# pgvector/pgvector

Measured on AMD Instinct MI355X. Metric: QPS @ recall@10 (IVFFlat, 1M x 1536d), higher is better.
Workload: dtype f32

## Files before the change

pgvector_amd/csrc/kernels_query.hip:

```cpp
#include "pgv_device.h"
#include "pgv_select.h"

#include <type_traits>

namespace pgv {

namespace {

constexpr int kQThreads = kSelThreads;
constexpr int kQWaves = kQThreads / kWave;
constexpr int kMaxBatchLists = 256;
constexpr int kHeadCap = 1024;

template <typename T, int METRIC, int NCH> struct WholeRows {
    Raw16 q[NCH];
    __device__ __forceinline__ void load_query(const char *qp, int lane) {
#pragma unroll
        for (int c = 0; c < NCH; c++) q[c] = load16(qp + ((size_t)c * kWave + lane) * sizeof(Raw16));
    }
    __device__ __forceinline__ float pair(const char *a, const char *b, int lane) const {
        Raw16 ra[NCH], rb[NCH];
#pragma unroll
        for (int c = 0; c < NCH; c++) ra[c] = load16(a + ((size_t)c * kWave + lane) * sizeof(Raw16));
#pragma unroll
        for (int c = 0; c < NCH; c++) rb[c] = load16(b + ((size_t)c * kWave + lane) * sizeof(Raw16));
        float sa = 0.f, sb = 0.f;
#pragma unroll
        for (int c = 0; c < NCH; c++) sa = accum_slice<T, METRIC>(sa, ra[c], q[c]);
#pragma unroll
        for (int c = 0; c < NCH; c++) sb = accum_slice<T, METRIC>(sb, rb[c], q[c]);
        return finish<METRIC>(wave_sum2(sa, sb));
    }
};

template <typename T, int METRIC>
__device__ __forceinline__ float group_distance(const char *row, const char *qp, int nvec, int lane_in, int lg) {
    const int lpr = 1 << lg;
    float acc0 = 0.f, acc1 = 0.f;
    int v = lane_in;
    for (; v + lpr < nvec; v += 2 * lpr) {
        const Raw16 a0 = load16(row + (size_t)v * sizeof(Raw16));
        const Raw16 a1 = load16(row + (size_t)(v + lpr) * sizeof(Raw16));
        acc0 = accum_slice<T, METRIC>(acc0, a0, load16(qp + (size_t)v * sizeof(Raw16)));
        acc1 = accum_slice<T, METRIC>(acc1, a1, load16(qp + (size_t)(v + lpr) * sizeof(Raw16)));
    }
    if (v < nvec) acc0 = accum_slice<T, METRIC>(acc0, load16(row + (size_t)v * sizeof(Raw16)), load16(qp + (size_t)v * sizeof(Raw16)));
    return finish<METRIC>(group_sum_to_last(acc0 + acc1, lg));
}

__device__ __forceinline__ float group_distance_dot(const char *row, const char *qp, int nvec, int lane_in, int lg, float *dot) {
    const int lpr = 1 << lg;
    float acc0 = 0.f, acc1 = 0.f, dot0 = 0.f, dot1 = 0.f;
    int v = lane_in;
    for (; v + lpr < nvec; v += 2 * lpr) {
        const Raw16 a0 = load16(row + (size_t)v * sizeof(Raw16));
        const Raw16 a1 = load16(row + (size_t)(v + lpr) * sizeof(Raw16));
        const Raw16 q0 = load16(qp + (size_t)v * sizeof(Raw16));
        const Raw16 q1 = load16(qp + (size_t)(v + lpr) * sizeof(Raw16));
        acc0 = accum_slice<float, 0>(acc0, a0, q0);
        acc1 = accum_slice<float, 0>(acc1, a1, q1);
        dot0 = accum_slice<float, 1>(dot0, a0, q0);
        dot1 = accum_slice<float, 1>(dot1, a1, q1);
    }
    if (v < nvec) {
        const Raw16 a0 = load16(row + (size_t)v * sizeof(Raw16)), q0 = load16(qp + (size_t)v * sizeof(Raw16));
        acc0 = accum_slice<float, 0>(acc0, a0, q0);
        dot0 = accum_slice<float, 1>(dot0, a0, q0);
    }
    *dot = group_sum_to_last(dot0 + dot1, lg);
    return finish<0>(group_sum_to_last(acc0 + acc1, lg));
}

template <typename RowPtr>
__device__ __forceinline__ void score_rows_dot(RowPtr row_ptr, int64_t first, int64_t end, const char *qp, int nvec, int lg,
                                               float *out, float *out_dot) {
    const int lane = threadIdx.x & (kWave - 1);
    const int wave = threadIdx.x >> 6;
    const int rpw = kWave >> lg;
    const int g = lane >> lg, lane_in = lane & ((1 << lg) - 1);
    for (int64_t j0 = first + (int64_t)wave * rpw; j0 < end; j0 += (int64_t)kQWaves * rpw) {
        const int64_t j = j0 + g;
        const bool valid = j < end;
        float dot;
        const float d = group_distance_dot(row_ptr(valid ? j : end - 1), qp, nvec, lane_in, lg, &dot);
        if (valid && lane_in == (1 << lg) - 1) {
            out[j] = d;
            out_dot[j] = dot;
        }
    }
}

__device__ __forceinline__ void fill_pair_terms(const char *vectors, size_t row_bytes, const char *qrow, int ld,
                                                const int32_t *slots_i32, const int64_t *slots_i64, int k,
                                                float *__restrict__ pair_t) {
    const int lane = threadIdx.x & (kWave - 1);
    for (int i = threadIdx.x >> 6; i < k; i += kQWaves) {
        const int64_t slot = slots_i32 ? (int64_t)__hip_atomic_load(slots_i32 + i, __ATOMIC_RELAXED, __HIP_MEMORY_SCOPE_AGENT)
                                       : __hip_atomic_load(slots_i64 + i, __ATOMIC_RELAXED, __HIP_MEMORY_SCOPE_AGENT);
        float a = 0.f;
        if (slot >= 0) {
            const float *x = reinterpret_cast<const float *>(qrow);
            const float *c = reinterpret_cast<const float *>(vectors + (size_t)slot * row_bytes);
            for (int e = lane; e < ld; e += kWave) a = fmaf(x[e], c[e], a);
            for (int o = 32; o > 0; o >>= 1) a += __shfl_xor(a, o);
        }
        if (lane == 0) pair_t[i] = -2.f * a;
    }
}

template <typename T, int METRIC, int NCH, typename RowPtr>
__device__ __forceinline__ void score_rows(RowPtr row_ptr, int64_t first, int64_t end, const char *qp, int nvec, int lg,
                                           float *out) {
    const int lane = threadIdx.x & (kWave - 1);
    const int wave = threadIdx.x >> 6;
    if constexpr (NCH > 0) {
        WholeRows<T, METRIC, NCH> w;
        w.load_query(qp, lane);
        for (int64_t j = first + 2 * wave; j < end; j += 2 * kQWaves) {
            const bool two = j + 1 < end;
            const float d = w.pair(row_ptr(j), row_ptr(two ? j + 1 : j), lane);
            if (lane == 0 || (lane == 1 && two)) out[j + lane] = d;
        }
    } else {
        const int rpw = kWave >> lg;
        const int g = lane >> lg, lane_in = lane & ((1 << lg) - 1);
        for (int64_t j0 = first + (int64_t)wave * rpw; j0 < end; j0 += (int64_t)kQWaves * rpw) {
            const int64_t j = j0 + g;
            const bool valid = j < end;
            const float d = group_distance<T, METRIC>(row_ptr(valid ? j : end - 1), qp, nvec, lane_in, lg);
            if (valid && lane_in == (1 << lg) - 1) out[j] = d;
        }
    }
}

template <typename T, int METRIC, int NCH>
__global__ __launch_bounds__(kQThreads) void query_rank_kernel(const char *__restrict__ centers, int nlists, int nvec,
                                                               int lg, const char *__restrict__ qp,
                                                               float *__restrict__ cdist, int per) {
    const size_t row_bytes = (size_t)nvec * sizeof(Raw16);
    for (int64_t first = (int64_t)blockIdx.x * per; first < nlists; first += (int64_t)gridDim.x * per) {
        const int64_t end = first + per < nlists ? first + per : nlists;
        score_rows<T, METRIC, NCH>([&](int64_t j) { return centers + (size_t)j * row_bytes; }, first, end, qp, nvec, lg,
                                   cdist);
    }
}

__global__ __launch_bounds__(kQThreads) void query_lists_kernel(const float *__restrict__ cdist, int nlists,
                                                                int max_probes, int kp, int32_t *__restrict__ out_lists) {
    extern __shared__ __attribute__((aligned(16))) char smem[];
    unsigned long long *ent = reinterpret_cast<unsigned long long *>(smem);
    SelShared *s = reinterpret_cast<SelShared *>(smem + (size_t)kHeadCap * 8);
    block_topk_auto(cdist, nlists, max_probes, kp, kHeadCap, ent, s);
    for (int i = threadIdx.x; i < max_probes; i += kQThreads) out_lists[i] = (int32_t)(unsigned)(ent[i] & 0xffffffffu);
}

struct QueryHead {
    long long total;
    int count;
    unsigned seq;
};

struct BatchMap {
    int64_t offs[kMaxBatchLists + 1];
    int64_t lbeg[kMaxBatchLists];
    __device__ void build(const int32_t *probe_lists, int nprobes, const int64_t *list_off) {
        if ((int)threadIdx.x < nprobes) {
            const int l = probe_lists[threadIdx.x];
            lbeg[threadIdx.x] = list_off[l];
            offs[threadIdx.x + 1] = list_off[l + 1] - list_off[l];
        }
        __syncthreads();
        if (threadIdx.x == 0) {
            offs[0] = 0;
            for (int p = 0; p < nprobes; p++) offs[p + 1] += offs[p];
        }
        __syncthreads();
    }
    __device__ __forceinline__ int64_t slot_of(int64_t j, int nprobes) const {
        int lo = 0, hi = nprobes - 1;
        while (lo < hi) {
            const int mid = (lo + hi + 1) >> 1;
            if (offs[mid] <= j)
                lo = mid;
            else
                hi = mid - 1;
        }
        return lbeg[lo] + (j - offs[lo]);
    }
};

template <typename T, int METRIC, int NCH>
__global__ __launch_bounds__(kQThreads) void query_scan_kernel(
    const char *__restrict__ vectors, const int64_t *__restrict__ list_off, const int32_t *__restrict__ probe_lists,
    int nprobes, int nvec, int lg, const char *__restrict__ qp, float *__restrict__ seg, int per) {
    __shared__ BatchMap map;
    const size_t row_bytes = (size_t)nvec * sizeof(Raw16);
    map.build(probe_lists, nprobes, list_off);
    const int64_t m = map.offs[nprobes];
    for (int64_t first = (int64_t)blockIdx.x * per; first < m; first += (int64_t)gridDim.x * per) {
        const int64_t end = first + per < m ? first + per : m;
        if (qp) {
            score_rows<T, METRIC, NCH>([&](int64_t j) { return vectors + (size_t)map.slot_of(j, nprobes) * row_bytes; },
                                       first, end, qp, nvec, lg, seg);
        } else {
            for (int64_t j = first + threadIdx.x; j < end; j += kQThreads) seg[j] = 0.f;
        }
    }
}

__global__ __launch_bounds__(kQThreads) void query_head_kernel(
    const float *__restrict__ seg, const int64_t *__restrict__ list_off, const uint64_t *__restrict__ tids,
    const int32_t *__restrict__ probe_lists, int nprobes, int skip, int count, int kp, QueryHead *__restrict__ hdr,
    float *__restrict__ head_dist, int64_t *__restrict__ head_slot, uint64_t *__restrict__ head_tid, unsigned seq) {
    extern __shared__ __attribute__((aligned(16))) char smem[];
    __shared__ BatchMap map;
    map.build(probe_lists, nprobes, list_off);
    const int64_t m = map.offs[nprobes];
    unsigned long long *ent = reinterpret_cast<unsigned long long *>(smem);
    SelShared *s = reinterpret_cast<SelShared *>(smem + (size_t)kHeadCap * 8);
    const int k = skip + count;
    block_topk_auto(seg, m, k, kp, kHeadCap, ent, s);
    const int have = (int)(m < k ? m : k) - skip;
    for (int i = threadIdx.x; i < have; i += kQThreads) {
        const unsigned long long e = ent[skip + i];
        const int64_t slot = map.slot_of((int64_t)(unsigned)(e & 0xffffffffu), nprobes);
        head_dist[i] = key_to_float((unsigned)(e >> 32));
        head_slot[i] = slot;
        head_tid[i] = tids ? tids[slot] : ~0ull;
    }
    asm volatile("s_waitcnt vmcnt(0)" ::: "memory");
    __syncthreads();
    if (threadIdx.x == 0) {
        hdr->total = m;
        hdr->count = have > 0 ? have : 0;
        __hip_atomic_store(&hdr->seq, seq, __ATOMIC_RELEASE, __HIP_MEMORY_SCOPE_SYSTEM);
    }
}

__global__ __launch_bounds__(1024) void query_stage_kernel(const Raw16 *__restrict__ src, Raw16 *__restrict__ dst, int nvec) {
    for (int i = threadIdx.x; i < nvec; i += 1024) dst[i] = src[i];
}

__global__ void query_iota_kernel(int32_t *__restrict__ out, int n) {
    const int i = blockIdx.x * blockDim.x + threadIdx.x;
    if (i < n) out[i] = i;
}

template <typename T, int METRIC, int NCH>
__global__ __launch_bounds__(kQThreads) void mq_rank_kernel(const char *__restrict__ centers, int nlists, int nvec, int lg,
                                                            const char *__restrict__ queries, float *__restrict__ cdist,
                                                            int64_t cd_stride, int per) {
    const size_t row_bytes = (size_t)nvec * sizeof(Raw16);
    const char *qp = queries + (size_t)blockIdx.y * row_bytes;
    float *cd = cdist + (size_t)blockIdx.y * cd_stride;
    for (int64_t first = (int64_t)blockIdx.x * per; first < nlists; first += (int64_t)gridDim.x * per) {
        const int64_t end = first + per < nlists ? first + per : nlists;
        score_rows<T, METRIC, NCH>([&](int64_t j) { return centers + (size_t)j * row_bytes; }, first, end, qp, nvec, lg, cd);
    }
}

__global__ __launch_bounds__(kQThreads) void mq_lists_kernel(const float *__restrict__ cdist, int64_t cd_stride, int nlists,
                                                             int max_probes, int kp, int32_t *__restrict__ out_lists,
                                                             float *__restrict__ out_dist) {
    extern __shared__ __attribute__((aligned(16))) char smem[];
    unsigned long long *ent = reinterpret_cast<unsigned long long *>(smem);
    SelShared *s = reinterpret_cast<SelShared *>(smem + (size_t)kHeadCap * 8);
    const int q = blockIdx.x;
    block_topk_auto(cdist + (size_t)q * cd_stride, nlists, max_probes, kp, kHeadCap, ent, s);
    for (int i = threadIdx.x; i < max_probes; i += kQThreads) {
        out_lists[(size_t)q * max_probes + i] = (int32_t)(unsigned)(ent[i] & 0xffffffffu);
        if (out_dist) out_dist[(size_t)q * max_probes + i] = key_to_float((unsigned)(ent[i] >> 32));
    }
}

template <typename T, int METRIC, int NCH>
__global__ __launch_bounds__(kQThreads) void mq_scan_kernel(
    const char *__restrict__ vectors, const int64_t *__restrict__ list_off, const int32_t *__restrict__ probe_lists,
    int nprobes, int nvec, int lg, const char *__restrict__ queries, float *__restrict__ seg, int64_t seg_stride, int per) {
    __shared__ BatchMap map;
    const size_t row_bytes = (size_t)nvec * sizeof(Raw16);
    const int q = blockIdx.y;
    map.build(probe_lists + (size_t)q * nprobes, nprobes, list_off);
    const int64_t m = map.offs[nprobes];
    const char *qp = queries + (size_t)q * row_bytes;
    float *sg = seg + (size_t)q * seg_stride;
    for (int64_t first = (int64_t)blockIdx.x * per; first < m; first += (int64_t)gridDim.x * per) {
        const int64_t end = first + per < m ? first + per : m;
        score_rows<T, METRIC, NCH>([&](int64_t j) { return vectors + (size_t)map.slot_of(j, nprobes) * row_bytes; },
                                   first, end, qp, nvec, lg, sg);
    }
}

__global__ __launch_bounds__(kQThreads) void mq_head_kernel(
    const float *__restrict__ seg, int64_t seg_stride, const int64_t *__restrict__ list_off,
    const uint64_t *__restrict__ tids, const int32_t *__restrict__ probe_lists, int nprobes, int k, int kp,
    float *__restrict__ out_dist, int64_t *__restrict__ out_slot, uint64_t *__restrict__ out_tid,
    double *__restrict__ stats) {
    extern __shared__ __attribute__((aligned(16))) char smem[];
    __shared__ BatchMap map;
    const int q = blockIdx.x;
    map.build(probe_lists + (size_t)q * nprobes, nprobes, list_off);
    const int64_t m = map.offs[nprobes];
    unsigned long long *ent = reinterpret_cast<unsigned long long *>(smem);
    SelShared *s = reinterpret_cast<SelShared *>(smem + (size_t)kHeadCap * 8);
    block_topk_auto(seg + (size_t)q * seg_stride, m, k, kp, kHeadCap, ent, s);
    const int have = (int)(m < k ? m : k);
    for (int i = threadIdx.x; i < k; i += kQThreads) {
        const size_t o = (size_t)q * k + i;
        if (i < have) {
            const unsigned long long e = ent[i];
            const int64_t slot = map.slot_of((int64_t)(unsigned)(e & 0xffffffffu), nprobes);
            out_dist[o] = key_to_float((unsigned)(e >> 32));
            if (out_slot) out_slot[o] = slot;
            if (out_tid) out_tid[o] = tids ? tids[slot] : ~0ull;
        } else {
            out_dist[o] = INFINITY;
            if (out_slot) out_slot[o] = -1;
            if (out_tid) out_tid[o] = ~0ull;
        }
    }
    if (stats && threadIdx.x == 0) {
        atomicAdd(&stats[0], (double)m);
        atomicAdd(&stats[1], (double)m);
        atomicAdd(&stats[5], (double)m);
    }
}

constexpr int kRecheckCap = 256;

template <typename T, bool DOT = false>
__global__ __launch_bounds__(kQThreads) void batch_recheck_kernel(
    const char *__restrict__ vectors, const uint64_t *__restrict__ tids, int nvec, int lg,
    const char *__restrict__ queries, int kprime, int k, const float *__restrict__ approx_val,
    const int64_t *__restrict__ cand_pos, const int64_t *__restrict__ cand_slot,
    const int64_t *__restrict__ list_off, const int32_t *__restrict__ probe_lists,
    const int64_t *__restrict__ probe_off, int probes,
    const int64_t *__restrict__ seg_start, int64_t fixed_len,
    const unsigned *__restrict__ row_norm_max, ScanBound bound, const float *__restrict__ eps_add, int nq,
    float *__restrict__ out_dist, int64_t *__restrict__ out_slot, uint64_t *__restrict__ out_tid,
    int32_t *__restrict__ out_i32, int32_t *__restrict__ flags, float *__restrict__ pair_t, PlanEmit emit) {
    static_assert(!DOT || std::is_same<T, float>::value, "pair terms: fp32 rows");
    __shared__ float exact[kRecheckCap];
    __shared__ float dots[DOT ? kRecheckCap : 1];
    __shared__ __attribute__((aligned(16))) unsigned long long ent[kRecheckCap];
    const int q = blockIdx.x;
    const size_t row_bytes = (size_t)nvec * sizeof(Raw16);
    const int64_t m = seg_start ? seg_start[q + 1] - seg_start[q] : fixed_len;
    const int ncand = (int)(m < kprime ? m : (int64_t)kprime);
    const int kk = ncand < k ? ncand : k;
    const float *av = approx_val + (size_t)q * kprime;
    __shared__ float qn_part[kQWaves];
    {
        const char *qrow = queries + (size_t)q * row_bytes;
        float a = 0.f;
        for (int v = threadIdx.x; v < nvec; v += kQThreads) {
            const Raw16 x = load16(qrow + (size_t)v * sizeof(Raw16));
            a = accum_slice<T, 1>(a, x, x);
        }
        for (int m2 = 32; m2 > 0; m2 >>= 1) a += __shfl_xor(a, m2);
        if ((threadIdx.x & (kWave - 1)) == 0) qn_part[threadIdx.x >> 6] = a;
    }
    __syncthreads();
    float qn = 0.f;
    for (int w = 0; w < kQWaves; w++) qn += qn_part[w];
    const float rn = __uint_as_float(*row_norm_max);
    const float cross = 2.f * sqrtf(qn * rn);
    const float eps = 1.001f * (bound.g_sq * (qn + rn + cross) + bound.g_dot * cross + bound.g_norm * rn +
                                (eps_add ? eps_add[q] : 0.f));
    unsigned band = 0u;
    if (kk > 0) {
        const float edge = av[kk - 1] + 2.f * eps;
        band = float_to_key(edge + bound.g_ref * fabsf(edge + qn));
    }
    const int cnt = __syncthreads_count((int)threadIdx.x < ncand && float_to_key(av[threadIdx.x]) <= band);
    __shared__ int64_t slots[kRecheckCap];
    if ((int)threadIdx.x < cnt) {
        const int64_t p = cand_pos[(size_t)q * kprime + threadIdx.x];
        int64_t slot = p;
        if (cand_slot) {
            slot = cand_slot[(size_t)q * kprime + threadIdx.x];
        } else {
            const int64_t *off = probe_off + (size_t)q * probes;
            int lo = 0, hi = probes - 1;
            while (lo < hi) {
                const int mid = (lo + hi + 1) >> 1;
                if (off[mid] <= p)
                    lo = mid;
                else
                    hi = mid - 1;
            }
            slot = list_off[probe_lists[(size_t)q * probes + lo]] + (p - off[lo]);
        }
        slots[threadIdx.x] = slot;
    }
    __syncthreads();
    if constexpr (DOT)
        score_rows_dot([&](int64_t j) { return vectors + (size_t)slots[j] * row_bytes; }, 0, cnt,
                       queries + (size_t)q * row_bytes, nvec, lg, exact, dots);
    else
        score_rows<T, 0, 0>([&](int64_t j) { return vectors + (size_t)slots[j] * row_bytes; }, 0, cnt,
                            queries + (size_t)q * row_bytes, nvec, lg, exact);
    __syncthreads();
    if ((int)threadIdx.x < kRecheckCap)
        ent[threadIdx.x] = (int)threadIdx.x < cnt
                               ? ((unsigned long long)float_to_key(exact[threadIdx.x]) << 32) |
                                     (unsigned)cand_pos[(size_t)q * kprime + threadIdx.x]
                               : ~0ull;
    __syncthreads();
    const unsigned long long mine = ent[threadIdx.x];
    const int64_t my_slot = (int)threadIdx.x < cnt ? slots[threadIdx.x] : -1;
    int rank = 0;
    {
        const ulonglong2 *e2 = reinterpret_cast<const ulonglong2 *>(ent);
        const int n2 = (cnt + 1) / 2;
#pragma unroll 8
        for (int j = 0; j < n2; j++) {
            const ulonglong2 o = e2[j];
            rank += o.x < mine ? 1 : 0;
            rank += o.y < mine ? 1 : 0;
        }
    }
    if ((int)threadIdx.x < cnt && rank < k) {
        const size_t o = (size_t)q * k + rank;
        out_dist[o] = key_to_float((unsigned)(mine >> 32));
        if (out_slot) out_slot[o] = my_slot;
        if (out_i32) out_i32[o] = (int32_t)my_slot;
        if (out_tid) out_tid[o] = tids ? tids[my_slot] : ~0ull;
        if constexpr (DOT) pair_t[o] = -2.f * dots[threadIdx.x];
    }
    if ((int)threadIdx.x >= kk && (int)threadIdx.x < k) {
        const size_t o = (size_t)q * k + threadIdx.x;
        out_dist[o] = INFINITY;
        if (out_slot) out_slot[o] = -1;
        if (out_i32) out_i32[o] = -1;
        if (out_tid) out_tid[o] = ~0ull;
        if constexpr (DOT) pair_t[o] = 0.f;
    }
    if constexpr (DOT) {
        if (emit.cnt) {
            __syncthreads();
            if ((int)threadIdx.x < cnt && rank < k) {
                atomicAdd(&emit.cnt[my_slot], 1);
                slots[rank] = emit.list_off[my_slot + 1] - emit.list_off[my_slot];
            }
            if ((int)threadIdx.x >= kk && (int)threadIdx.x < k) slots[threadIdx.x] = 0;
            __syncthreads();
            if ((int)threadIdx.x < k) {
                int64_t run = 0;
                for (int i = 0; i < (int)threadIdx.x; i++) run += slots[i];
                emit.probe_off[(size_t)q * k + threadIdx.x] = run;
                if ((int)threadIdx.x == k - 1) emit.seg_len[q] = run + slots[threadIdx.x];
            }
        }
    }
    if (threadIdx.x == 0) {
        const int32_t flag = (m > ncand && cnt == ncand) ? 1 : 0;
        flags[q] = flag;
        if (flag) flags[nq + 1 + atomicAdd(&flags[nq], 1)] = q;
    }
}

constexpr int kWide = kRecheckCap;

template <typename T>
__global__ __launch_bounds__(kQThreads) void batch_fix_kernel(
    const char *__restrict__ vectors, const int64_t *__restrict__ list_off, const uint64_t *__restrict__ tids, int nvec,
    int lg, const char *__restrict__ queries, const int32_t *__restrict__ probe_lists,
    const int64_t *__restrict__ probe_off, int probes, const int64_t *__restrict__ seg_start, int64_t fixed_len,
    const int32_t *__restrict__ flags, int nq, float *__restrict__ seg_vals, int k, int kp, int cap,
    const unsigned *__restrict__ row_norm_max, ScanBound bound, const float *__restrict__ eps_add, int widen,
    float *__restrict__ out_dist, int64_t *__restrict__ out_slot, uint64_t *__restrict__ out_tid,
    int32_t *__restrict__ out_i32, double *__restrict__ stats, float *__restrict__ pair_t, PlanEmit emit) {
    extern __shared__ __attribute__((aligned(16))) char smem[];
    unsigned long long *ent = reinterpret_cast<unsigned long long *>(smem);
    SelShared *sel = reinterpret_cast<SelShared *>(smem + (size_t)cap * 8);
    __shared__ float exact[kWide];
    __shared__ int64_t slots[kWide];
    __shared__ float qn_part[kQWaves];
    const int nflag = flags[nq];
    const size_t row_bytes = (size_t)nvec * sizeof(Raw16);
    for (int f = blockIdx.x; f < nflag; f += gridDim.x) {
        const int q = flags[nq + 1 + f];
        const int64_t base = probe_lists ? seg_start[q] : (int64_t)q * fixed_len;
        const int64_t m = probe_lists ? seg_start[q + 1] - base : fixed_len;
        const int64_t *off = probe_off + (size_t)q * probes;
        const int32_t *pl = probe_lists + (size_t)q * probes;
        auto slot_of = [&](int64_t j) -> int64_t {
            if (!probe_lists) return j;
            int lo = 0, hi = probes - 1;
            while (lo < hi) {
                const int mid = (lo + hi + 1) >> 1;
                if (off[mid] <= j)
                    lo = mid;
                else
                    hi = mid - 1;
            }
            return list_off[pl[lo]] + (j - off[lo]);
        };
        float *v = seg_vals + base;
        const char *qrow = queries + (size_t)q * row_bytes;
        auto pair_terms = [&]() {
            if constexpr (std::is_same<T, float>::value) {
                if (pair_t) {
                    __threadfence();
                    __syncthreads();
                    fill_pair_terms(vectors, row_bytes, qrow, nvec * 4, out_i32 ? out_i32 + (size_t)q * k : nullptr,
                                    out_slot ? out_slot + (size_t)q * k : nullptr, k, pair_t + (size_t)q * k);
                    if (emit.cnt) {
                        if ((int)threadIdx.x < k) {
                            const int l = __hip_atomic_load(out_i32 + (size_t)q * k + threadIdx.x, __ATOMIC_RELAXED,
                                                            __HIP_MEMORY_SCOPE_AGENT);
                            if (l >= 0) atomicAdd(&emit.cnt[l], 1);
                            slots[threadIdx.x] = l >= 0 ? emit.list_off[l + 1] - emit.list_off[l] : 0;
                        }
                        __syncthreads();
                        if ((int)threadIdx.x < k) {
                            int64_t run = 0;
                            for (int i = 0; i < (int)threadIdx.x; i++) run += slots[i];
                            emit.probe_off[(size_t)q * k + threadIdx.x] = run;
                            if ((int)threadIdx.x == k - 1) emit.seg_len[q] = run + slots[threadIdx.x];
                        }
                    }
                }
            }
        };
        if constexpr (std::is_same<T, float>::value) {
            if (pair_t && emit.cnt) {
                if ((int)threadIdx.x < k) {
                    const int l = out_i32[(size_t)q * k + threadIdx.x];
                    if (l >= 0) atomicSub(&emit.cnt[l], 1);
                }
                __syncthreads();
            }
        }
        bool settled = false;
        if (widen && k <= kWide / 2) {
            const int nw = (int)(m < kWide ? m : (int64_t)kWide);
            block_topk([v](int64_t i) { return v[i]; }, m, nw, kWide, cap, ent, sel);
            {
                float a = 0.f;
                for (int x = threadIdx.x; x < nvec; x += kQThreads) {
                    const Raw16 e = load16(qrow + (size_t)x * sizeof(Raw16));
                    a = accum_slice<T, 1>(a, e, e);
                }
                for (int m2 = 32; m2 > 0; m2 >>= 1) a += __shfl_xor(a, m2);
                if ((threadIdx.x & (kWave - 1)) == 0) qn_part[threadIdx.x >> 6] = a;
            }
            __syncthreads();
            float qn = 0.f;
            for (int w = 0; w < kQWaves; w++) qn += qn_part[w];
            const float rn = __uint_as_float(*row_norm_max);
            const float cross = 2.f * sqrtf(qn * rn);
            const float eps = 1.001f * (bound.g_sq * (qn + rn + cross) + bound.g_dot * cross + bound.g_norm * rn +
                                        (eps_add ? eps_add[q] : 0.f));
            const int kk = nw < k ? nw : k;
            unsigned band = 0u;
            if (kk > 0) {
                const float edge = key_to_float((unsigned)(ent[kk - 1] >> 32)) + 2.f * eps;
                band = float_to_key(edge + bound.g_ref * fabsf(edge + qn));
            }
            const int cnt = __syncthreads_count((int)threadIdx.x < nw && (unsigned)(ent[threadIdx.x] >> 32) <= band);
            settled = !(m > nw && cnt == nw);
            if (settled) {
                const unsigned my_pos = (int)threadIdx.x < cnt ? (unsigned)(ent[threadIdx.x] & 0xffffffffu) : 0u;
                if ((int)threadIdx.x < cnt) slots[threadIdx.x] = slot_of((int64_t)my_pos);
                __syncthreads();
                score_rows<T, 0, 0>([&](int64_t j) { return vectors + (size_t)slots[j] * row_bytes; }, 0, cnt, qrow, nvec, lg,
                                    exact);
                __syncthreads();
                if ((int)threadIdx.x < kWide)
                    ent[threadIdx.x] = (int)threadIdx.x < cnt
                                           ? ((unsigned long long)float_to_key(exact[threadIdx.x]) << 32) | my_pos
                                           : ~0ull;
                __syncthreads();
                const unsigned long long mine = ent[threadIdx.x];
                int rank = 0;
                for (int j = 0; j < cnt; j++) rank += ent[j] < mine ? 1 : 0;
                const int have = (int)(m < k ? m : (int64_t)k);
                if ((int)threadIdx.x < cnt && rank < k) {
                    const size_t o = (size_t)q * k + rank;
                    const int64_t slot = slots[threadIdx.x];
                    out_dist[o] = key_to_float((unsigned)(mine >> 32));
                    if (out_slot) out_slot[o] = slot;
                    if (out_i32) out_i32[o] = (int32_t)slot;
                    if (out_tid) out_tid[o] = tids ? tids[slot] : ~0ull;
                }
                if ((int)threadIdx.x >= have && (int)threadIdx.x < k) {
                    const size_t o = (size_t)q * k + threadIdx.x;
                    out_dist[o] = INFINITY;
                    if (out_slot) out_slot[o] = -1;
                    if (out_i32) out_i32[o] = -1;
                    if (out_tid) out_tid[o] = ~0ull;
                }
                if (stats && threadIdx.x == 0) atomicAdd(&stats[7], 1.0);
                pair_terms();
            }
            __syncthreads();
        }
        if (settled) continue;
        if (stats && threadIdx.x == 0) atomicAdd(&stats[6], 1.0);
        score_rows<T, 0, 0>([&](int64_t j) { return vectors + (size_t)slot_of(j) * row_bytes; }, 0, m, qrow, nvec, lg, v);
        __threadfence();
        __syncthreads();
        block_topk([v](int64_t i) { return __hip_atomic_load(v + i, __ATOMIC_RELAXED, __HIP_MEMORY_SCOPE_AGENT); }, m, k, kp,
                   cap, ent, sel);
        for (int i = threadIdx.x; i < k; i += kQThreads) {
            const unsigned long long e = ent[i];
            const bool have = e != ~0ull && (int64_t)i < (m < k ? m : (int64_t)k);
            const int64_t slot = have ? slot_of((int64_t)(unsigned)(e & 0xffffffffu)) : -1;
            out_dist[(size_t)q * k + i] = have ? key_to_float((unsigned)(e >> 32)) : INFINITY;
            if (out_slot) out_slot[(size_t)q * k + i] = slot;
            if (out_i32) out_i32[(size_t)q * k + i] = (int32_t)slot;
            if (out_tid) out_tid[(size_t)q * k + i] = (have && tids) ? tids[slot] : ~0ull;
        }
        pair_terms();
        __syncthreads();
    }
}

constexpr size_t kQueryLds = (size_t)kHeadCap * 8 + sizeof(SelShared);

void run_geometry(pgv_ctx *ctx, const RowGeom &g, int64_t nrows, int *per, int *grid) {
    const bool whole = g.lpr_log2 == 6 && g.nvec % kWave == 0;
    const int step = kQWaves * (whole ? 2 : (kWave >> g.lpr_log2));
    int64_t runs = (nrows + step - 1) / step;
    const int64_t cap = (int64_t)ctx->num_cus * 8;
    *per = step;
    *grid = (int)(runs < 1 ? 1 : (runs > cap ? cap : runs));
}

int pow2_at_least(int k) {
    int kp = 2;
    while (kp < k) kp <<= 1;
    return kp;
}

template <typename T, int METRIC, typename F> int dispatch_nch(const RowGeom &g, F f) {
    if (g.lpr_log2 == 6 && g.nvec % kWave == 0) {
        switch (g.nvec / kWave) {
            case 1: return f(std::integral_constant<int, 1>());
            case 2: return f(std::integral_constant<int, 2>());
            case 3: return f(std::integral_constant<int, 3>());
            case 4: return f(std::integral_constant<int, 4>());
            case 6: return f(std::integral_constant<int, 6>());
        }
    }
    return f(std::integral_constant<int, 0>());
}

}

int query_max_batch_lists() { return kMaxBatchLists; }
int query_head_cap() { return kHeadCap; }
size_t query_head_bytes(int head) { return sizeof(QueryHead) + (size_t)head * (4 + 8 + 8) + 64; }

int launch_query_stage(pgv_ctx *ctx, const void *src_pinned, void *dst_dev, int nvec) {
    hipLaunchKernelGGL(query_stage_kernel, dim3(1), dim3(1024), 0, ctx->stream, static_cast<const Raw16 *>(src_pinned),
                       static_cast<Raw16 *>(dst_dev), nvec);
    PGV_HIP(hipGetLastError());
    return PGV_OK;
}

int launch_query_iota(pgv_ctx *ctx, int32_t *out, int n) {
    hipLaunchKernelGGL(query_iota_kernel, dim3((n + 255) / 256), dim3(256), 0, ctx->stream, out, n);
    PGV_HIP(hipGetLastError());
    return PGV_OK;
}

int launch_one_query_rows(pgv_ctx *ctx, const RowsView &v, const void *q_dev, float *out) {
    if (v.n <= 0) return PGV_OK;
    if (v.bits()) PGV_FAIL(PGV_ERR_ARG, "one query over rows: fp32 / fp16 rows only");
    const RowGeom &g = v.geom;
    const void *rows = v.rows;
    const int n = (int)v.n;
    int per, grid;
    run_geometry(ctx, g, n, &per, &grid);
    return dispatch_metric(v.metric, v.dtype(), [&](auto *tp, auto mc) {
        using T = std::remove_pointer_t<decltype(tp)>;
        constexpr int M = decltype(mc)::value;
        return dispatch_nch<T, M>(g, [&](auto nc) {
            constexpr int NCH = decltype(nc)::value;
            hipLaunchKernelGGL((query_rank_kernel<T, M, NCH>), dim3(grid), dim3(kQThreads), 0, ctx->stream,
                               static_cast<const char *>(rows), n, g.nvec, g.lpr_log2, static_cast<const char *>(q_dev),
                               out, per);
            PGV_HIP(hipGetLastError());
            return PGV_OK;
        });
    });
}

int launch_query_rank(pgv_ctx *ctx, const pgv_index *ix, const void *q_dev, float *cdist, int max_probes,
                      int32_t *out_lists) {
    const RowGeom &g = ix->geom;
    int per, grid;
    run_geometry(ctx, g, ix->nlists, &per, &grid);
    const int kp = pow2_at_least(max_probes);
    PGV_TRY(dispatch_metric(ix->metric, ix->dtype, [&](auto *tp, auto mc) {
        using T = std::remove_pointer_t<decltype(tp)>;
        constexpr int M = decltype(mc)::value;
        return dispatch_nch<T, M>(g, [&](auto nc) {
            constexpr int NCH = decltype(nc)::value;
            hipLaunchKernelGGL((query_rank_kernel<T, M, NCH>), dim3(grid), dim3(kQThreads), 0, ctx->stream,
                               static_cast<const char *>(ix->centers), ix->nlists, g.nvec, g.lpr_log2,
                               static_cast<const char *>(q_dev), cdist, per);
            PGV_HIP(hipGetLastError());
            return PGV_OK;
        });
    }));
    hipLaunchKernelGGL(query_lists_kernel, dim3(1), dim3(kQThreads), kQueryLds, ctx->stream, cdist, ix->nlists,
                       max_probes, kp, out_lists);
    PGV_HIP(hipGetLastError());
    return PGV_OK;
}

int launch_query_scan(pgv_ctx *ctx, const pgv_index *ix, const void *q_dev, const int32_t *probe_lists, int nprobes,
                      int64_t rows_bound, float *seg) {
    const RowGeom &g = ix->geom;
    int per, grid;
    run_geometry(ctx, g, rows_bound, &per, &grid);
    return dispatch_metric(ix->metric, ix->dtype, [&](auto *tp, auto mc) {
        using T = std::remove_pointer_t<decltype(tp)>;
        constexpr int M = decltype(mc)::value;
        return dispatch_nch<T, M>(g, [&](auto nc) {
            constexpr int NCH = decltype(nc)::value;
            hipLaunchKernelGGL((query_scan_kernel<T, M, NCH>), dim3(grid), dim3(kQThreads), 0, ctx->stream,
                               static_cast<const char *>(ix->vectors), ix->list_offsets, probe_lists, nprobes, g.nvec,
                               g.lpr_log2, static_cast<const char *>(q_dev), seg, per);
            PGV_HIP(hipGetLastError());
            return PGV_OK;
        });
    });
}

int launch_query_head(pgv_ctx *ctx, const pgv_index *ix, const float *seg, const int32_t *probe_lists, int nprobes,
                      int skip, int count, void *head_rec, unsigned seq) {
    const int kp = pow2_at_least(skip + count);
    QueryHead *hdr = static_cast<QueryHead *>(head_rec);
    char *base = static_cast<char *>(head_rec) + 64;
    int64_t *h_slot = reinterpret_cast<int64_t *>(base);
    uint64_t *h_tid = reinterpret_cast<uint64_t *>(base + (size_t)count * 8);
    float *h_dist = reinterpret_cast<float *>(base + (size_t)count * 16);
    hipLaunchKernelGGL(query_head_kernel, dim3(1), dim3(kQThreads), kQueryLds, ctx->stream, seg, ix->list_offsets,
                       ix->tids, probe_lists, nprobes, skip, count, kp, hdr, h_dist, h_slot, h_tid, seq);
    PGV_HIP(hipGetLastError());
    return PGV_OK;
}

int launch_multi_rank(pgv_ctx *ctx, const pgv_index *ix, const void *q_dev, int nq, float *cdist, int64_t cd_stride,
                      int max_probes, int32_t *out_lists, float *out_dist) {
    const RowGeom &g = ix->geom;
    int per, grid;
    run_geometry(ctx, g, ix->nlists, &per, &grid);
    const int kp = pow2_at_least(max_probes);
    PGV_TRY(dispatch_metric(ix->metric, ix->dtype, [&](auto *tp, auto mc) {
        using T = std::remove_pointer_t<decltype(tp)>;
        constexpr int M = decltype(mc)::value;
        return dispatch_nch<T, M>(g, [&](auto nc) {
            constexpr int NCH = decltype(nc)::value;
            hipLaunchKernelGGL((mq_rank_kernel<T, M, NCH>), dim3(grid, nq), dim3(kQThreads), 0, ctx->stream,
                               static_cast<const char *>(ix->centers), ix->nlists, g.nvec, g.lpr_log2,
                               static_cast<const char *>(q_dev), cdist, cd_stride, per);
            PGV_HIP(hipGetLastError());
            return PGV_OK;
        });
    }));
    hipLaunchKernelGGL(mq_lists_kernel, dim3(nq), dim3(kQThreads), kQueryLds, ctx->stream, cdist, cd_stride, ix->nlists,
                       max_probes, kp, out_lists, out_dist);
    PGV_HIP(hipGetLastError());
    return PGV_OK;
}

int launch_multi_scan(pgv_ctx *ctx, const pgv_index *ix, const void *q_dev, int nq, const int32_t *probe_lists, int nprobes,
                      int64_t rows_bound, float *seg, int64_t seg_stride, int k, float *out_dist, int64_t *out_slot,
                      uint64_t *out_tid) {
    const RowGeom &g = ix->geom;
    int per, grid;
    run_geometry(ctx, g, rows_bound, &per, &grid);
    const int cap = (ctx->num_cus * 8 + nq - 1) / nq;
    if (grid > cap) grid = cap < 1 ? 1 : cap;
    PGV_TRY(dispatch_metric(ix->metric, ix->dtype, [&](auto *tp, auto mc) {
        using T = std::remove_pointer_t<decltype(tp)>;
        constexpr int M = decltype(mc)::value;
        return dispatch_nch<T, M>(g, [&](auto nc) {
            constexpr int NCH = decltype(nc)::value;
            hipLaunchKernelGGL((mq_scan_kernel<T, M, NCH>), dim3(grid, nq), dim3(kQThreads), 0, ctx->stream,
                               static_cast<const char *>(ix->vectors), ix->list_offsets, probe_lists, nprobes, g.nvec,
                               g.lpr_log2, static_cast<const char *>(q_dev), seg, seg_stride, per);
            PGV_HIP(hipGetLastError());
            return PGV_OK;
        });
    }));
    double *stats = (ctx->profiling && ctx->stats_dev.p) ? ctx->stats_dev.as<double>() : nullptr;
    hipLaunchKernelGGL(mq_head_kernel, dim3(nq), dim3(kQThreads), kQueryLds, ctx->stream, seg, seg_stride, ix->list_offsets,
                       ix->tids, probe_lists, nprobes, k, pow2_at_least(k), out_dist, out_slot, out_tid, stats);
    PGV_HIP(hipGetLastError());
    return PGV_OK;
}

namespace {
struct ApproxScratch {
    float *cand_val = nullptr;
    int64_t *cand_pos = nullptr;
    int32_t *flags = nullptr;
    int carve(DBuf &buf, int nq, int kprime) {
        const size_t nk = (size_t)nq * kprime;
        const size_t a1 = (sizeof(float) * nk + 15) & ~(size_t)15, a2 = a1 + sizeof(int64_t) * nk;
        PGV_TRY(buf.ensure(a2 + sizeof(int32_t) * (2 * (size_t)nq + 1)));
        cand_val = buf.as<float>();
        cand_pos = reinterpret_cast<int64_t *>(buf.as<char>() + a1);
        flags = reinterpret_cast<int32_t *>(buf.as<char>() + a2);
        return PGV_OK;
    }
};
}

int launch_exact_tail(pgv_ctx *ctx, const ExactTail &t, DBuf &scratch) {
    if (t.nq <= 0) return PGV_OK;
    const ExactRows &xr = t.rows;
    const bool dense = t.dense();
    if (dense ? (t.fixed_len <= 0 || t.probe_off || t.seg_start || t.probes != 0)
              : (t.fixed_len != 0 || !t.probe_off || !t.seg_start || t.probes < 1))
        PGV_FAIL(PGV_ERR_ARG, "exact tail: a list plan or one dense run");
    if (t.kprime > kRecheckCap || t.k > t.kprime)
        PGV_FAIL(PGV_ERR_ARG, "exact tail: k' = %d outside k..%d", t.kprime, kRecheckCap);
    if (t.pair_t && xr.dtype != PGV_F32) PGV_FAIL(PGV_ERR_ARG, "exact tail: pair terms are for fp32 rows");
    static_assert(kWide >= kRecheckCap, "k <= k' <= kWide: batch_fix_kernel's emit");
    if (t.emit.cnt && !(dense && t.pair_t && t.out_i32 && t.emit.probe_off && t.emit.seg_len && t.emit.list_off))
        PGV_FAIL(PGV_ERR_ARG, "exact tail: the plan is counted where the pair terms are written");
    ApproxScratch sc;
    PGV_TRY(sc.carve(scratch, t.nq, t.kprime));
    const int64_t *cand_slot = dense ? sc.cand_pos : nullptr;
    const int64_t *seg_start = dense ? nullptr : t.seg_start;
    const int64_t fixed_len = dense ? t.fixed_len : 0;
    PGV_TRY(launch_topk_segments(ctx, t.approx, seg_start, t.nq, fixed_len, t.kprime, sc.cand_val, sc.cand_pos,
                                 sc.flags + t.nq, t.emit.cnt, t.emit.cnt ? 2 * (int)fixed_len : 0,
                                 dense ? 0 : t.seg_bound));
#define PGV_RECHECK(T, DOT)                                                                                          \
    hipLaunchKernelGGL((batch_recheck_kernel<T, DOT>), dim3(t.nq), dim3(kQThreads), 0, ctx->stream,                   \
                       static_cast<const char *>(xr.vectors), xr.tids, xr.geom.nvec, xr.geom.lpr_log2,                \
                       static_cast<const char *>(t.queries), t.kprime, t.k, sc.cand_val, sc.cand_pos, cand_slot,      \
                       xr.list_offsets, t.probe_lists, t.probe_off, t.probes, seg_start, fixed_len, xr.norm_max,      \
                       t.bound, t.eps_add, t.nq, t.out_dist, t.out_slot, t.out_tid, t.out_i32, sc.flags, t.pair_t,    \
                       t.emit)
    if (t.pair_t)
        PGV_RECHECK(float, true);
    else if (xr.dtype == PGV_F32)
        PGV_RECHECK(float, false);
    else
        PGV_RECHECK(__half, false);
#undef PGV_RECHECK
    PGV_HIP(hipGetLastError());
    double *stats = (ctx->profiling && ctx->stats_dev.p) ? ctx->stats_dev.as<double>() : nullptr;
    int kp = 2;
    while (kp < t.k) kp <<= 1;
    const int cap = kp > kFastCap ? kp : kFastCap;
    const size_t lds = (size_t)cap * 8 + sizeof(SelShared);
    const int grid = t.nq < ctx->num_cus ? t.nq : ctx->num_cus;
#define PGV_FIX(T)                                                                                                    \
    hipLaunchKernelGGL(batch_fix_kernel<T>, dim3(grid), dim3(kQThreads), lds, ctx->stream,                            \
                       static_cast<const char *>(xr.vectors), xr.list_offsets, xr.tids, xr.geom.nvec,                 \
                       xr.geom.lpr_log2, static_cast<const char *>(t.queries), t.probe_lists, t.probe_off, t.probes,  \
                       seg_start, fixed_len, sc.flags, t.nq, t.approx, t.k, kp, cap, xr.norm_max, t.bound, t.eps_add, \
                       ctx->no_widen ? 0 : 1, t.out_dist, t.out_slot, t.out_tid, t.out_i32, stats, t.pair_t, t.emit)
    if (xr.dtype == PGV_F32)
        PGV_FIX(float);
    else
        PGV_FIX(__half);
#undef PGV_FIX
    PGV_HIP(hipGetLastError());
    return PGV_OK;
}

}
```

pgvector_amd/csrc/kernels_shadow.hip:

```cpp
#include "pgv_device.h"

#include <cfloat>

namespace pgv {

namespace {

__device__ __forceinline__ int list_of_row(const int64_t *__restrict__ list_off, int nlists, int64_t r) {
    int lo = 0, hi = nlists - 1;
    while (lo < hi) {
        const int mid = (lo + hi + 1) >> 1;
        if (list_off[mid] <= r)
            lo = mid;
        else
            hi = mid - 1;
    }
    return lo;
}

__device__ __forceinline__ int scale_for(float m) {
    if (!(m > 0.f) || !isfinite(m)) return 0;
    int e;
    (void)frexpf(m, &e);
    return e - 14;
}

__global__ __launch_bounds__(256) void shadow_absmax_kernel(const float *__restrict__ rows, const float *__restrict__ centers,
                                                            const int64_t *__restrict__ list_off, int nlists, int64_t n,
                                                            int ld, unsigned *__restrict__ max_bits) {
    const int64_t r = (int64_t)blockIdx.x * 4 + (threadIdx.x >> 6);
    if (r >= n) return;
    const int lane = threadIdx.x & (kWave - 1);
    const float *x = rows + (size_t)r * ld;
    const float *c = centers ? centers + (size_t)list_of_row(list_off, nlists, r) * ld : nullptr;
    float m = 0.f;
    for (int i = lane; i < ld; i += kWave) {
        const float d = fabsf(c ? x[i] - c[i] : x[i]);
        m = (d > m || d != d) ? d : m;
    }
    for (int o = 32; o > 0; o >>= 1) {
        const float v = __shfl_xor(m, o);
        m = (v > m || v != v) ? v : m;
    }
    if (lane == 0 && __float_as_uint(m) > __hip_atomic_load(max_bits, __ATOMIC_RELAXED, __HIP_MEMORY_SCOPE_AGENT))
        atomicMax(max_bits, __float_as_uint(m));
}

__global__ __launch_bounds__(256) void shadow_build_kernel(const float *__restrict__ rows, const float *__restrict__ centers,
                                                           const int64_t *__restrict__ list_off, int nlists, int64_t n,
                                                           int ld, int ld16, const unsigned *__restrict__ max_bits,
                                                           __half *__restrict__ shadow,
                                                           unsigned long long *__restrict__ ep_bits) {
    const int64_t r = (int64_t)blockIdx.x * 4 + (threadIdx.x >> 6);
    if (r >= n) return;
    const int lane = threadIdx.x & (kWave - 1);
    const int s = scale_for(__uint_as_float(*max_bits));
    const float *x = rows + (size_t)r * ld;
    const float *c = centers ? centers + (size_t)list_of_row(list_off, nlists, r) * ld : nullptr;
    __half *h = shadow + (size_t)r * ld16;
    const double up = ldexp(1.0, s);
    double e2 = 0.0, p2 = 0.0;
    for (int i = lane; i < ld16; i += kWave) {
        __half v = __float2half(0.f);
        if (i < ld) {
            const float ci = c ? c[i] : 0.f;
            v = __float2half(ldexpf(x[i] - ci, -s));
            const double back = (double)__half2float(v) * up;
            const double d = ((double)x[i] - (double)ci) - back;
            e2 = fma(d, d, e2);
            p2 = fma(back, back, p2);
        }
        h[i] = v;
    }
    for (int o = 32; o > 0; o >>= 1) {
        e2 += __shfl_xor(e2, o);
        p2 += __shfl_xor(p2, o);
    }
    if (lane == 0) {
        const unsigned long long eb = (unsigned long long)__double_as_longlong(e2 != e2 ? INFINITY : e2),
                                 pb = (unsigned long long)__double_as_longlong(p2 != p2 ? INFINITY : p2);
        if (eb > __hip_atomic_load(&ep_bits[0], __ATOMIC_RELAXED, __HIP_MEMORY_SCOPE_AGENT)) atomicMax(&ep_bits[0], eb);
        if (pb > __hip_atomic_load(&ep_bits[1], __ATOMIC_RELAXED, __HIP_MEMORY_SCOPE_AGENT)) atomicMax(&ep_bits[1], pb);
    }
}

constexpr int kCastChunks = 4;

struct CastChunk {
    float4 a, b;
};

__device__ __forceinline__ float absmax_keep_nan(float m, float v) {
    const float a = fabsf(v);
    return (a > m || a != a) ? a : m;
}

__device__ __forceinline__ CastChunk cast_chunk_load(const float *__restrict__ x, int c, int ld) {
    CastChunk r;
    const float4 zero = make_float4(0.f, 0.f, 0.f, 0.f);
    r.a = 8 * c < ld ? *reinterpret_cast<const float4 *>(x + 8 * c) : zero;
    r.b = 8 * c + 4 < ld ? *reinterpret_cast<const float4 *>(x + 8 * c + 4) : zero;
    return r;
}

__device__ __forceinline__ float cast_chunk_max(const CastChunk &r, float m) {
    m = absmax_keep_nan(m, r.a.x);
    m = absmax_keep_nan(m, r.a.y);
    m = absmax_keep_nan(m, r.a.z);
    m = absmax_keep_nan(m, r.a.w);
    m = absmax_keep_nan(m, r.b.x);
    m = absmax_keep_nan(m, r.b.y);
    m = absmax_keep_nan(m, r.b.z);
    m = absmax_keep_nan(m, r.b.w);
    return m;
}

__device__ __forceinline__ void cast_chunk_store(const CastChunk &r, int c, int ld, int sq, double up, __half *__restrict__ h,
                                                 double (&qq)[4], double (&dd)[4], double (&hh)[4]) {
    const float xs[8] = {r.a.x, r.a.y, r.a.z, r.a.w, r.b.x, r.b.y, r.b.z, r.b.w};
    union {
        __half v[8];
        uint4 w;
    } out;
#pragma unroll
    for (int e = 0; e < 8; e++) {
        __half v = __float2half(0.f);
        if (8 * c + e < ld) {
            v = __float2half(ldexpf(xs[e], -sq));
            const double back = (double)__half2float(v) * up, xi = (double)xs[e];
            qq[e & 3] = fma(xi, xi, qq[e & 3]);
            dd[e & 3] = fma(xi - back, xi - back, dd[e & 3]);
            hh[e & 3] = fma(back, back, hh[e & 3]);
        }
        out.v[e] = v;
    }
    *reinterpret_cast<uint4 *>(h + 8 * c) = out.w;
}

__global__ __launch_bounds__(256) void shadow_query_kernel(const float *__restrict__ queries, int nq, int ld, int ld16,
                                                           ShadowTerms st, RankShadowTerms rt,
                                                           const float *__restrict__ center_norm_max,
                                                           const float *__restrict__ row_norm_max,
                                                           __half *__restrict__ qcast, float *__restrict__ qscale,
                                                           float *__restrict__ qeps, float *__restrict__ cscale,
                                                           float *__restrict__ ceps) {
    const int q = (int)(blockIdx.x * 4 + (threadIdx.x >> 6));
    if (q >= nq) return;
    const int lane = threadIdx.x & (kWave - 1);
    const float *x = queries + (size_t)q * ld;
    __half *h = qcast + (size_t)q * ld16;
    const int nchunks = ld16 / 8;
    const bool in_regs = nchunks <= kWave * kCastChunks;
    CastChunk reg[kCastChunks];
    float m = 0.f;
    if (in_regs) {
#pragma unroll
        for (int j = 0; j < kCastChunks; j++) {
            const int c = lane + j * kWave;
            reg[j] = cast_chunk_load(x, c < nchunks ? c : nchunks, ld);
        }
#pragma unroll
        for (int j = 0; j < kCastChunks; j++) m = cast_chunk_max(reg[j], m);
    } else {
        for (int c = lane; c < nchunks; c += kWave) m = cast_chunk_max(cast_chunk_load(x, c, ld), m);
    }
    for (int o = 32; o > 0; o >>= 1) {
        const float v = __shfl_xor(m, o);
        m = (v > m || v != v) ? v : m;
    }
    const int sq = scale_for(m);
    const double up = ldexp(1.0, sq);
    double qq4[4] = {0.0, 0.0, 0.0, 0.0}, dd4[4] = {0.0, 0.0, 0.0, 0.0}, hh4[4] = {0.0, 0.0, 0.0, 0.0};
    if (in_regs) {
#pragma unroll
        for (int j = 0; j < kCastChunks; j++) {
            const int c = lane + j * kWave;
            if (c < nchunks) cast_chunk_store(reg[j], c, ld, sq, up, h, qq4, dd4, hh4);
        }
    } else {
        for (int c = lane; c < nchunks; c += kWave) cast_chunk_store(cast_chunk_load(x, c, ld), c, ld, sq, up, h, qq4, dd4, hh4);
    }
    double qq = (qq4[0] + qq4[1]) + (qq4[2] + qq4[3]);
    double dd = (dd4[0] + dd4[1]) + (dd4[2] + dd4[3]);
    double hh = (hh4[0] + hh4[1]) + (hh4[2] + hh4[3]);
    for (int o = 32; o > 0; o >>= 1) {
        qq += __shfl_xor(qq, o);
        dd += __shfl_xor(dd, o);
        hh += __shfl_xor(hh, o);
    }
    const double u = 5.9604644775390625e-8;
    if (lane == 0 && ceps) {
        const int e = 1 + rt.s + sq;
        const double qn = sqrt(qq), dq = sqrt(dd), qh = sqrt(hh);
        const double cn = (double)*center_norm_max * (1.0 + rt.g_cn);
        double eps = 2.0 * (qn * rt.E + dq * rt.P)
                     + rt.g_dot * 2.0 * qh * rt.P
                     + 4.0 * u * (cn + 2.0 * qh * rt.P * (1.0 + rt.g_dot));
        eps = eps * (1.0 + 1.0 / 1048576.0) + 4.0 * (double)FLT_MIN;
        if (e < -125 || e > 125 || !(eps < 1e30)) eps = INFINITY;
        cscale[q] = ldexpf(1.f, e < -125 ? 0 : (e > 125 ? 0 : e));
        ceps[q] = (float)eps;
    }
    if (lane == 0 && qeps) {
        const int e = 1 + st.s + sq;
        const double qn = sqrt(qq), dq = sqrt(dd), qh = sqrt(hh);
        const double cmax = sqrt((double)*center_norm_max * (1.0 + st.g_cn)), rn = (double)*row_norm_max * (1.0 + st.g_cn);
        const double tmax = 2.0 * qn * cmax;
        double eps = 2.0 * (qn * st.E + dq * st.P)
                     + st.g_dot * 2.0 * qh * st.P
                     + st.g_pair * tmax
                     + 4.0 * u * (rn + tmax * (1.0 + st.g_pair) + 2.0 * qh * st.P * (1.0 + st.g_dot));
        eps = eps * (1.0 + 1.0 / 1048576.0) + 4.0 * (double)FLT_MIN;
        if (e < -125 || e > 125 || !(eps < 1e30)) eps = INFINITY;
        qscale[q] = ldexpf(1.f, e < -125 ? 0 : (e > 125 ? 0 : e));
        qeps[q] = (float)eps;
    }
}

__global__ __launch_bounds__(256) void shadow_pair_kernel(const float *__restrict__ queries, const float *__restrict__ centers,
                                                          const int64_t *__restrict__ pair_start, int nlists, int64_t npairs,
                                                          int ld, ScanPair *__restrict__ pairs) {
    const int64_t pos = (int64_t)blockIdx.x * 4 + (threadIdx.x >> 6);
    if (pos >= npairs) return;
    const int lane = threadIdx.x & (kWave - 1);
    int lo = 0, hi = nlists - 1;
    while (lo < hi) {
        const int mid = (lo + hi + 1) >> 1;
        if (pair_start[mid] <= pos)
            lo = mid;
        else
            hi = mid - 1;
    }
    const int q = pairs[pos].query;
    const float *x = queries + (size_t)q * ld;
    const float *c = centers + (size_t)lo * ld;
    float a = 0.f;
    for (int i = lane; i < ld; i += kWave) a = fmaf(x[i], c[i], a);
    for (int o = 32; o > 0; o >>= 1) a += __shfl_xor(a, o);
    if (lane == 0) pairs[pos].pad = (int32_t)__float_as_uint(-2.f * a);
}

}

int launch_shadow_build(pgv_ctx *ctx, const RowGeom &g32, const RowGeom &g16, const void *rows, const void *centers,
                        const int64_t *list_off, int nlists, int64_t n, void *shadow, void *words) {
    if (n <= 0) return PGV_OK;
    PGV_HIP(hipMemsetAsync(words, 0, 24, ctx->stream));
    unsigned *max_bits = static_cast<unsigned *>(words);
    unsigned long long *ep = reinterpret_cast<unsigned long long *>(static_cast<char *>(words) + 8);
    const dim3 grid((unsigned)((n + 3) / 4));
    hipLaunchKernelGGL(shadow_absmax_kernel, grid, dim3(256), 0, ctx->stream, static_cast<const float *>(rows),
                       static_cast<const float *>(centers), list_off, nlists, n, g32.ld, max_bits);
    hipLaunchKernelGGL(shadow_build_kernel, grid, dim3(256), 0, ctx->stream, static_cast<const float *>(rows),
                       static_cast<const float *>(centers), list_off, nlists, n, g32.ld, g16.ld, max_bits, static_cast<__half *>(shadow), ep);
    PGV_HIP(hipGetLastError());
    return PGV_OK;
}

int shadow_scale_of(float max_abs) {
    if (!(max_abs > 0.f) || !std::isfinite(max_abs)) return 0;
    int e;
    (void)std::frexp(max_abs, &e);
    return e - 14;
}

int launch_shadow_query(pgv_ctx *ctx, const RowGeom &g32, const RowGeom &g16, const void *queries, int nq,
                        const ShadowTerms &st, const RankShadowTerms &rt, const float *center_norm_max,
                        const float *row_norm_max, void *qcast, float *qscale, float *qeps, float *cscale, float *ceps) {
    if (nq <= 0) return PGV_OK;
    hipLaunchKernelGGL(shadow_query_kernel, dim3((unsigned)((nq + 3) / 4)), dim3(256), 0, ctx->stream,
                       static_cast<const float *>(queries), nq, g32.ld, g16.ld, st, rt, center_norm_max, row_norm_max,
                       static_cast<__half *>(qcast), qscale, qeps, cscale, ceps);
    PGV_HIP(hipGetLastError());
    return PGV_OK;
}

int launch_shadow_pairs(pgv_ctx *ctx, const RowGeom &g32, const void *queries, const void *centers,
                        const int64_t *pair_start, int nlists, int64_t npairs, ScanPair *pairs) {
    if (npairs <= 0) return PGV_OK;
    hipLaunchKernelGGL(shadow_pair_kernel, dim3((unsigned)((npairs + 3) / 4)), dim3(256), 0, ctx->stream,
                       static_cast<const float *>(queries), static_cast<const float *>(centers), pair_start, nlists, npairs,
                       g32.ld, pairs);
    PGV_HIP(hipGetLastError());
    return PGV_OK;
}

}
```

pgvector_amd/csrc/pgv_abi_ivf.hip:

```cpp
#include "pgv_abi_common.h"

extern "C" {


namespace {
struct IndexLayout {
    size_t centers, vectors, offsets, tids, row_norms, center_norms, bytes;
    bool has_tids, has_norms;
};
IndexLayout index_layout(int nlists, int64_t n, size_t row_bytes, bool has_tids, bool l2) {
    auto up = [](size_t v) { return (v + 255) & ~(size_t)255; };
    IndexLayout L{};
    size_t at = 0;
    L.centers = at; at = up(at + (size_t)nlists * row_bytes);
    L.vectors = at; at = up(at + (size_t)(n > 0 ? n : 1) * row_bytes);
    L.offsets = at; at = up(at + sizeof(int64_t) * ((size_t)nlists + 1));
    L.has_tids = has_tids;
    L.tids = at; if (has_tids) at = up(at + sizeof(uint64_t) * (size_t)n);
    L.has_norms = l2;
    L.row_norms = at; if (l2 && n > 0) at = up(at + sizeof(float) * ((size_t)n + 1));
    L.center_norms = at; if (l2) at = up(at + sizeof(float) * ((size_t)nlists + 1));
    L.bytes = at;
    return L;
}
void index_carve(pgv_index *ix, const IndexLayout &L) {
    char *b = static_cast<char *>(ix->arena);
    ix->centers = b + L.centers;
    ix->vectors = b + L.vectors;
    ix->list_offsets = reinterpret_cast<int64_t *>(b + L.offsets);
    ix->tids = L.has_tids ? reinterpret_cast<uint64_t *>(b + L.tids) : nullptr;
    ix->row_norms = L.has_norms && ix->nrows > 0 ? reinterpret_cast<float *>(b + L.row_norms) : nullptr;
    ix->center_norms = L.has_norms ? reinterpret_cast<float *>(b + L.center_norms) : nullptr;
}
void index_host_tables(pgv_index *ix) {
    const int nlists = ix->nlists;
    std::vector<int64_t> lens((size_t)nlists);
    int64_t maxlen = 0;
    for (int l = 0; l < nlists; l++) {
        lens[l] = ix->h_offsets[l + 1] - ix->h_offsets[l];
        if (lens[l] > maxlen) maxlen = lens[l];
    }
    ix->max_list_len = maxlen;
    std::sort(lens.begin(), lens.end(), [](int64_t a, int64_t b) { return a > b; });
    ix->len_prefix.assign((size_t)nlists + 1, 0);
    for (int l = 0; l < nlists; l++) ix->len_prefix[l + 1] = ix->len_prefix[l] + lens[l];
}
}

extern "C++" {
namespace {

int shadow_env() {
    const char *e = getenv("PGV_SCAN_SHADOW");
    return e ? atoi(e) : -1;
}

int rank_shadow_env() {
    const char *e = getenv("PGV_RANK_SHADOW");
    return e ? atoi(e) : 1;
}

int shadow_create(pgv_ctx *ctx, pgv_index *ix) {
    const int env = shadow_env();
    if (env == 0 || ix->metric != PGV_L2SQ || ix->dtype != PGV_F32 || ix->nrows <= 0 || !ix->row_norms || !ix->center_norms)
        return PGV_OK;
    if (env < 0 && !rows_stream_past_caches(ivf_rows(ix))) return PGV_OK;
    const RowGeom g16 = row_geom(ix->dim, PGV_F16);
    const size_t bytes = ((size_t)ix->nrows * g16.ld * sizeof(uint16_t) + 255) & ~(size_t)255;
    const size_t cbytes = ((size_t)ix->nlists * g16.ld * sizeof(uint16_t) + 255) & ~(size_t)255;
    void *sh = nullptr;
    if (hipMalloc(&sh, bytes + 256 + cbytes) != hipSuccess) {
        (void)hipGetLastError();
        return PGV_OK;
    }
    void *words = static_cast<char *>(sh) + bytes;
    void *csh = static_cast<char *>(sh) + bytes + 256;
    int rc = launch_shadow_build(ctx, ix->geom, g16, ix->vectors, ix->centers, ix->list_offsets, ix->nlists, ix->nrows, sh,
                                 words);
    if (rc == PGV_OK)
        rc = launch_shadow_build(ctx, ix->geom, g16, ix->centers, nullptr, nullptr, 0, ix->nlists, csh,
                                 static_cast<char *>(words) + 32);
    unsigned char h[56];
    if (rc == PGV_OK && (hipStreamSynchronize(ctx->stream) != hipSuccess ||
                         hipMemcpy(h, words, sizeof(h), hipMemcpyDeviceToHost) != hipSuccess)) {
        set_error("shadow build failed: %s", hipGetErrorString(hipGetLastError()));
        rc = PGV_ERR_DEVICE;
    }
    if (rc != PGV_OK) {
        (void)hipFree(sh);
        return rc;
    }
    float max_abs;
    double e2, p2;
    memcpy(&max_abs, h, 4);
    memcpy(&e2, h + 8, 8);
    memcpy(&p2, h + 16, 8);
    const double P = std::sqrt(p2), E = std::sqrt(e2);
    if (!std::isfinite(E) || !std::isfinite(P) || !std::isfinite(max_abs)) {
        (void)hipFree(sh);
        return PGV_OK;
    }
    ix->shadow = sh;
    ix->shadow_geom = g16;
    ix->shadow_s = shadow_scale_of(max_abs);
    ix->shadow_E = (E + 1e-12 * (P + E)) * (1.0 + 1e-9);
    ix->shadow_P = P * (1.0 + 1e-9);
    float cmax_abs;
    double ce2, cp2;
    memcpy(&cmax_abs, h + 32, 4);
    memcpy(&ce2, h + 40, 8);
    memcpy(&cp2, h + 48, 8);
    const double Pc = std::sqrt(cp2), Ec = std::sqrt(ce2);
    if (std::isfinite(Ec) && std::isfinite(Pc) && std::isfinite(cmax_abs)) {
        ix->cshadow = csh;
        ix->cshadow_s = shadow_scale_of(cmax_abs);
        ix->cshadow_E = (Ec + 1e-12 * (Pc + Ec)) * (1.0 + 1e-9);
        ix->cshadow_P = Pc * (1.0 + 1e-9);
    }
    return PGV_OK;
}

struct ShadowBatch {
    void *qcast = nullptr;
    float *qscale = nullptr, *qeps = nullptr;
    float *cscale = nullptr, *ceps = nullptr;
    float *pair_t = nullptr;
    bool scan_follows = false;
    bool cast_for_scan = false;
    bool pairs_done = false;
};

int shadow_batch_cast(pgv_index *ix, const void *q_dev, int nq, int probes, bool for_rank, bool for_scan, ShadowBatch *sb) {
    pgv_ctx *ctx = ix->ctx;
    const RowGeom &g16 = ix->shadow_geom;
    const size_t qb = ((size_t)nq * g16.ld * sizeof(uint16_t) + 255) & ~(size_t)255;
    PGV_TRY(ctx->sh_q.ensure(qb + sizeof(float) * (size_t)nq * (4 + (size_t)probes)));
    sb->qcast = ctx->sh_q.p;
    sb->qscale = reinterpret_cast<float *>(ctx->sh_q.as<char>() + qb);
    sb->qeps = sb->qscale + nq;
    sb->cscale = sb->qeps + nq;
    sb->ceps = sb->cscale + nq;
    sb->pair_t = sb->ceps + nq;
    constexpr double u = 5.9604644775390625e-8;
    ShadowTerms st{};
    st.s = ix->shadow_s;
    st.E = ix->shadow_E;
    st.P = ix->shadow_P;
    st.g_dot = gamma_n(shadow_chain_length(g16) + 4.0, u);
    st.g_pair = gamma_n((double)pair_chain_length(ix->geom), u);
    st.g_cn = shadow_band(ix->geom.ld, 0.f, u).g_norm;
    RankShadowTerms rt{};
    rt.s = ix->cshadow_s;
    rt.E = ix->cshadow_E;
    rt.P = ix->cshadow_P;
    rt.g_dot = st.g_dot;
    rt.g_cn = st.g_cn;
    PGV_TRY(launch_shadow_query(ctx, ix->geom, g16, q_dev, nq, st, rt, ix->center_norms + ix->nlists,
                                ix->row_norms + ix->nrows, sb->qcast, for_scan ? sb->qscale : nullptr,
                                for_scan ? sb->qeps : nullptr, for_rank ? sb->cscale : nullptr,
                                for_rank ? sb->ceps : nullptr));
    sb->cast_for_scan = for_scan;
    return PGV_OK;
}

struct IndexElem {
    pgv_metric metric;
    pgv_dtype dtype;
    int dim, nbits;
    static IndexElem bits(int nbits) { return {PGV_L1, PGV_F32, nbits, nbits}; }
    size_t tight_bytes() const { return nbits > 0 ? (size_t)(nbits + 7) / 8 : (size_t)dim * elem_size(dtype); }
};

template <typename Fill>
int index_create(pgv_ctx *ctx, const IndexElem &el, int nlists, const std::vector<int64_t> &off, bool has_tids, Fill fill,
                 pgv_index **out) {
    const pgv_metric metric = el.metric;
    const int nbits = el.nbits;
    const int64_t n = off[nlists];
    pgv_index *ix = new (std::nothrow) pgv_index();
    if (!ix) PGV_FAIL(PGV_ERR_NOMEM, "out of host memory");
    ix->ctx = ctx;
    ix->refs = new (std::nothrow) int(1);
    if (!ix->refs) {
        delete ix;
        PGV_FAIL(PGV_ERR_NOMEM, "out of host memory");
    }
    ix->metric = metric;
    ix->dtype = el.dtype;
    ix->dim = el.dim;
    ix->nlists = nlists;
    ix->nrows = n;
    ix->nbits = nbits;
    ix->geom = nbits > 0 ? bit_row_geom(nbits) : row_geom(el.dim, el.dtype);
    ix->h_offsets = off;
    index_host_tables(ix);

    auto fail = [&](int rc) {
        pgv_index_free(ix);
        return rc;
    };
    IndexLayout lay = index_layout(nlists, n, ivf_rows(ix).row_bytes(), has_tids && n > 0, metric == PGV_L2SQ && nbits == 0);
    if (malloc_exportable(&ix->arena, lay.bytes) != hipSuccess) {
        (void)hipGetLastError();
        set_error("hipMalloc(%zu) for the index mirror failed", lay.bytes);
        return fail(PGV_ERR_NOMEM);
    }
    ix->arena_bytes = lay.bytes;
    index_carve(ix, lay);
    int rc;
    if ((rc = fill(ix)) != PGV_OK) return fail(rc);
    if (hipMemcpyAsync(ix->list_offsets, ix->h_offsets.data(), sizeof(int64_t) * off.size(),
                       hipMemcpyHostToDevice, ctx->stream) != hipSuccess)
        return fail((set_error("copy of list_offsets failed"), PGV_ERR_DEVICE));
    if (ix->row_norms) {
        if (hipMemsetAsync(ix->row_norms + n, 0, sizeof(float), ctx->stream) != hipSuccess)
            return fail((set_error("memset of row_norms failed"), PGV_ERR_DEVICE));
        if ((rc = launch_row_norms(ctx, ivf_rows(ix), ix->row_norms, reinterpret_cast<unsigned *>(ix->row_norms + n))) != PGV_OK)
            return fail(rc);
    }
    if (ix->center_norms) {
        if (hipMemsetAsync(ix->center_norms + nlists, 0, sizeof(float), ctx->stream) != hipSuccess)
            return fail((set_error("memset of center_norms failed"), PGV_ERR_DEVICE));
        if ((rc = launch_row_norms(ctx, ivf_centers(ix), ix->center_norms,
                                   reinterpret_cast<unsigned *>(ix->center_norms + nlists))) != PGV_OK)
            return fail(rc);
    }
    if (nbits == 0 && (rc = shadow_create(ctx, ix)) != PGV_OK) return fail(rc);
    if (hipStreamSynchronize(ctx->stream) != hipSuccess)
        return fail((set_error("index upload failed: %s", hipGetErrorString(hipGetLastError())), PGV_ERR_DEVICE));
    *out = ix;
    return PGV_OK;
}

int index_upload(pgv_ctx *ctx, const IndexElem &el, int nlists, const void *centers, const int64_t *list_offsets,
                 const void *rows, const char *rows_name, const uint64_t *tids, pgv_index **out) {
    if (nlists < 1 || nlists > 32768) PGV_FAIL(PGV_ERR_ARG, "lists %d outside 1..32768", nlists);
    if (!centers || !list_offsets) PGV_FAIL(PGV_ERR_ARG, "centers/list_offsets is NULL");
    PGV_HIP(hipSetDevice(ctx->device));
    std::vector<int64_t> off((size_t)nlists + 1);
    if (is_device_ptr(list_offsets)) {
        PGV_HIP(hipMemcpy(off.data(), list_offsets, sizeof(int64_t) * off.size(), hipMemcpyDeviceToHost));
    } else {
        memcpy(off.data(), list_offsets, sizeof(int64_t) * off.size());
    }
    if (off[0] != 0) PGV_FAIL(PGV_ERR_ARG, "list_offsets[0] must be 0");
    for (int l = 0; l < nlists; l++)
        if (off[l + 1] < off[l]) PGV_FAIL(PGV_ERR_ARG, "list_offsets not ascending at list %d", l);
    const int64_t n = off[nlists];
    if (n > 0 && !rows) PGV_FAIL(PGV_ERR_ARG, "%s is NULL", rows_name);
    return index_create(ctx, el, nlists, off, tids != nullptr, [&](pgv_index *ix) -> int {
        const size_t padded = ivf_rows(ix).row_bytes();
        PGV_TRY(put_padded_rows(ctx->stream, ix->centers, padded, centers, el.tight_bytes(), nlists));
        PGV_TRY(put_padded_rows(ctx->stream, ix->vectors, padded, rows, el.tight_bytes(), n));
        if (ix->tids)
            PGV_HIP(hipMemcpyAsync(ix->tids, tids, sizeof(uint64_t) * (size_t)n,
                                   is_device_ptr(tids) ? hipMemcpyDeviceToDevice : hipMemcpyHostToDevice, ctx->stream));
        return PGV_OK;
    }, out);
}

}
}

int pgv_index_upload(pgv_ctx *ctx, pgv_metric metric, pgv_dtype dtype, int dim, int nlists,
                     const void *centers, const int64_t *list_offsets, const void *vectors,
                     const uint64_t *tids, pgv_index **out) {
    if (!ctx || !out) PGV_FAIL(PGV_ERR_ARG, "pgv_index_upload: ctx/out is NULL");
    *out = nullptr;
    PGV_TRY(check_common(dtype, dim));
    PGV_TRY(check_metric(metric));
    return index_upload(ctx, IndexElem{metric, dtype, dim, 0}, nlists, centers, list_offsets, vectors, "vectors", tids, out);
}

int pgv_index_upload_bits(pgv_ctx *ctx, int nbits, int nlists, const void *centers, const int64_t *list_offsets,
                          const void *rows, const uint64_t *tids, pgv_index **out) {
    if (!ctx || !out) PGV_FAIL(PGV_ERR_ARG, "pgv_index_upload_bits: ctx/out is NULL");
    *out = nullptr;
    if (nbits < 1 || nbits > kIvfMaxBits) PGV_FAIL(PGV_ERR_DIMS, "bit length %d outside 1..%d", nbits, kIvfMaxBits);
    return index_upload(ctx, IndexElem::bits(nbits), nlists, centers, list_offsets, rows, "rows", tids, out);
}

int pgv_index_nbits(const pgv_index *ix) { return ix ? ix->nbits : -1; }

#define PGV_NO_BIT_INDEX(ix, who)                                                                                 \
    do {                                                                                                          \
        if ((ix)->nbits > 0) PGV_FAIL(PGV_ERR_ARG, "%s: not served on a bit index (pgv_index_upload_bits)", who); \
    } while (0)

static int stage_queries(pgv_index *ix, const void *queries, int nq, const void **q_dev) {
    if (ix->nbits > 0)
        return stage_rows(ix->ctx, queries, nq, (size_t)(ix->nbits + 7) / 8, (size_t)bit_query_bytes(ix->nbits), ix->ctx->q_stage,
                          q_dev);
    return stage_rows(ix->ctx, queries, nq, ix->dim, ix->dtype, ix->geom, ix->ctx->q_stage, q_dev);
}

struct pgv_builder {
    pgv_ctx *ctx = nullptr;
    pgv_metric metric = PGV_L2SQ;
    pgv_dtype dtype = PGV_F32;
    int dim = 0, nlists = 0;
    RowGeom geom{};
    DBuf centers;
    DBuf rows;
    DBuf tids;
    DBuf lists;
    int64_t n = 0, cap = 0;
    int64_t assigned = 0;
    bool has_tids = true;
    bool deferred = false;
    hipStream_t copy_stream = nullptr;
    hipStream_t stream() const { return deferred ? copy_stream : ctx->stream; }
    RowsView view() const { return {rows.p, n, geom, row_kind(dtype), metric}; }
    size_t row_bytes() const { return view().row_bytes(); }
    int put(hipStream_t to, void *dst, const void *src, int64_t cnt) const {
        return put_padded_rows(to, dst, row_bytes(), src, (size_t)dim * elem_size(dtype), cnt);
    }
};

static int builder_reserve(pgv_builder *b, int64_t want) {
    if (want <= b->cap) return PGV_OK;
    int64_t cap = b->cap ? b->cap + b->cap / 2 : want;
    if (cap < want) cap = want;
    const size_t row_bytes = b->row_bytes();
    DBuf rows, tids, lists;
    PGV_TRY(rows.ensure(row_bytes * (size_t)cap));
    int rc = tids.ensure(sizeof(uint64_t) * (size_t)cap);
    if (rc == PGV_OK) rc = lists.ensure(sizeof(int32_t) * (size_t)cap);
    if (rc == PGV_OK && b->n > 0) {
        hipError_t e = hipMemcpyAsync(rows.p, b->rows.p, row_bytes * (size_t)b->n, hipMemcpyDeviceToDevice, b->stream());
        if (e == hipSuccess) e = hipMemcpyAsync(tids.p, b->tids.p, sizeof(uint64_t) * (size_t)b->n, hipMemcpyDeviceToDevice, b->stream());
        if (e == hipSuccess) e = hipMemcpyAsync(lists.p, b->lists.p, sizeof(int32_t) * (size_t)b->n, hipMemcpyDeviceToDevice, b->stream());
        if (e == hipSuccess) e = hipStreamSynchronize(b->stream());
        if (e != hipSuccess) {
            set_error("growing the builder failed: %s", hipGetErrorString(e));
            rc = PGV_ERR_DEVICE;
        }
    }
    if (rc != PGV_OK) {
        rows.release();
        tids.release();
        lists.release();
        return rc;
    }
    b->rows.release();
    b->tids.release();
    b->lists.release();
    b->rows = rows;
    b->tids = tids;
    b->lists = lists;
    b->cap = cap;
    return PGV_OK;
}

static int builder_assign_pending(pgv_builder *b) {
    if (b->assigned >= b->n) return PGV_OK;
    PGV_TRY(launch_argmin(b->ctx, b->metric, b->dtype, b->geom, b->rows.as<char>() + (size_t)b->assigned * b->row_bytes(),
                          b->n - b->assigned, b->centers.p, b->nlists, b->lists.as<int32_t>() + b->assigned, nullptr));
    b->assigned = b->n;
    return PGV_OK;
}

int pgv_builder_begin(pgv_ctx *ctx, pgv_metric metric, pgv_dtype dtype, int dim, int nlists, const void *centers,
                      int64_t expected_rows, pgv_builder **out) {
    if (!ctx || !out) PGV_FAIL(PGV_ERR_ARG, "pgv_builder_begin: ctx/out is NULL");
    *out = nullptr;
    PGV_TRY(check_common(dtype, dim));
    PGV_TRY(check_metric(metric));
    if (nlists < 1 || nlists > 32768) PGV_FAIL(PGV_ERR_ARG, "lists %d outside 1..32768", nlists);
    if (expected_rows < 0) PGV_FAIL(PGV_ERR_ARG, "expected_rows < 0");
    PGV_HIP(hipSetDevice(ctx->device));
    pgv_builder *b = new (std::nothrow) pgv_builder();
    if (!b) PGV_FAIL(PGV_ERR_NOMEM, "out of host memory");
    b->ctx = ctx;
    b->metric = metric;
    b->dtype = dtype;
    b->dim = dim;
    b->nlists = nlists;
    b->geom = row_geom(dim, dtype);
    int rc = b->centers.ensure(b->row_bytes() * (size_t)nlists);
    if (rc == PGV_OK && centers) {
        rc = b->put(ctx->stream, b->centers.p, centers, nlists);
        if (rc == PGV_OK && hipStreamSynchronize(ctx->stream) != hipSuccess) rc = PGV_ERR_DEVICE;
    } else if (rc == PGV_OK) {
        b->deferred = true;
        if (hipStreamCreateWithFlags(&b->copy_stream, hipStreamNonBlocking) != hipSuccess) {
            set_error("pgv_builder_begin: no stream for the upload");
            rc = PGV_ERR_DEVICE;
        }
    }
    if (rc == PGV_OK && expected_rows > 0) rc = builder_reserve(b, expected_rows);
    if (rc != PGV_OK) {
        pgv_builder_free(b);
        return rc;
    }
    *out = b;
    return PGV_OK;
}

void pgv_builder_free(pgv_builder *b) {
    if (!b) return;
    if (b->copy_stream) {
        (void)hipStreamSynchronize(b->copy_stream);
        (void)hipStreamDestroy(b->copy_stream);
    }
    if (b->ctx) (void)hipStreamSynchronize(b->ctx->stream);
    b->centers.release();
    b->rows.release();
    b->tids.release();
    b->lists.release();
    delete b;
}

int64_t pgv_builder_rows(const pgv_builder *b) { return b ? b->n : -1; }

int pgv_builder_add(pgv_builder *b, const void *rows, const uint64_t *tids, int64_t n) {
    if (!b) PGV_FAIL(PGV_ERR_ARG, "pgv_builder_add: builder is NULL");
    if (n < 0) PGV_FAIL(PGV_ERR_ARG, "n < 0");
    if (n == 0) return PGV_OK;
    if (!rows) PGV_FAIL(PGV_ERR_ARG, "rows is NULL");
    if (b->n + n > 0xffffffffll) PGV_FAIL(PGV_ERR_ARG, "pgv_builder_add: more than 2^32 rows");
    if (b->n > 0 && (tids != nullptr) != b->has_tids) PGV_FAIL(PGV_ERR_ARG, "pgv_builder_add: tids given for some batches only");
    pgv_ctx *ctx = b->ctx;
    PGV_HIP(hipSetDevice(ctx->device));
    PGV_TRY(builder_reserve(b, b->n + n));
    b->has_tids = tids != nullptr;
    hipStream_t stream = b->stream();
    PGV_TRY(b->put(stream, b->rows.as<char>() + (size_t)b->n * b->row_bytes(), rows, n));
    if (tids)
        PGV_HIP(hipMemcpyAsync(b->tids.as<uint64_t>() + b->n, tids, sizeof(uint64_t) * (size_t)n,
                               is_device_ptr(tids) ? hipMemcpyDeviceToDevice : hipMemcpyHostToDevice, stream));
    b->n += n;
    if (!b->deferred) PGV_TRY(builder_assign_pending(b));
    if (b->deferred || !is_device_ptr(rows) || (tids && !is_device_ptr(tids))) PGV_HIP(hipStreamSynchronize(stream));
    return PGV_OK;
}

int pgv_builder_set_centers(pgv_builder *b, const void *centers) {
    if (!b || !centers) PGV_FAIL(PGV_ERR_ARG, "pgv_builder_set_centers: builder/centers is NULL");
    if (!b->deferred) PGV_FAIL(PGV_ERR_STATE, "pgv_builder_set_centers: the builder has its centers");
    pgv_ctx *ctx = b->ctx;
    PGV_HIP(hipSetDevice(ctx->device));
    PGV_HIP(hipStreamSynchronize(b->copy_stream));
    b->deferred = false;
    PGV_TRY(b->put(ctx->stream, b->centers.p, centers, b->nlists));
    PGV_HIP(hipStreamSynchronize(ctx->stream));
    return PGV_OK;
}

int pgv_builder_finish(pgv_builder *b, pgv_index **out_index, int64_t *out_offsets, int32_t *out_lists) {
    if (!b || !out_index) PGV_FAIL(PGV_ERR_ARG, "pgv_builder_finish: builder/out_index is NULL");
    *out_index = nullptr;
    pgv_ctx *ctx = b->ctx;
    PGV_HIP(hipSetDevice(ctx->device));
    if (b->deferred) PGV_FAIL(PGV_ERR_STATE, "pgv_builder_finish: no centers (pgv_builder_set_centers)");
    PGV_TRY(builder_assign_pending(b));
    const int64_t n = b->n;
    const int nlists = b->nlists;
    int list_bits = 1;
    while ((1 << list_bits) < nlists) list_bits++;
    const size_t sort_bytes = n > 0 ? build_sort_scratch_bytes(n, 32 + list_bits) : 0;
    const size_t kb = sizeof(unsigned long long) * (size_t)(n > 0 ? n : 1), cb = sizeof(unsigned long long) * (size_t)nlists,
                 ob = sizeof(int64_t) * ((size_t)nlists + 1);
    auto up = [](size_t x) { return (x + 255) & ~(size_t)255; };
    const size_t o_sorted = up(kb), o_counts = o_sorted + up(kb), o_off = o_counts + up(cb), o_bad = o_off + up(ob),
                 o_sort = o_bad + 256;
    DBuf scratch;
    PGV_TRY(scratch.ensure(o_sort + sort_bytes + 256));
    char *sp = scratch.as<char>();
    auto *keys_tmp = reinterpret_cast<unsigned long long *>(sp);
    auto *keys_sorted = reinterpret_cast<unsigned long long *>(sp + o_sorted);
    auto *counts = reinterpret_cast<unsigned long long *>(sp + o_counts);
    auto *offsets_dev = reinterpret_cast<int64_t *>(sp + o_off);
    int *bad = reinterpret_cast<int *>(sp + o_bad);
    int rc = launch_build_order(ctx, b->lists.as<int32_t>(), n, nlists, keys_tmp, keys_sorted, counts, offsets_dev, bad,
                                sp + o_sort, sort_bytes);
    std::vector<int64_t> off((size_t)nlists + 1);
    int bad_h = 0;
    if (rc == PGV_OK) {
        hipError_t e = hipMemcpyAsync(off.data(), offsets_dev, ob, hipMemcpyDeviceToHost, ctx->stream);
        if (e == hipSuccess) e = hipMemcpyAsync(&bad_h, bad, sizeof(int), hipMemcpyDeviceToHost, ctx->stream);
        if (e == hipSuccess && out_lists && n > 0)
            e = hipMemcpyAsync(out_lists, b->lists.p, sizeof(int32_t) * (size_t)n,
                               is_device_ptr(out_lists) ? hipMemcpyDeviceToDevice : hipMemcpyDeviceToHost, ctx->stream);
        if (e == hipSuccess) e = hipStreamSynchronize(ctx->stream);
        if (e != hipSuccess) {
            set_error("pgv_builder_finish: %s", hipGetErrorString(e));
            rc = PGV_ERR_DEVICE;
        }
    }
    if (rc == PGV_OK && (bad_h || off[nlists] != n)) {
        set_error("pgv_builder_finish: assignment produced a list id outside 0..%d", nlists - 1);
        rc = PGV_ERR_STATE;
    }
    if (rc == PGV_OK)
        rc = index_create(ctx, IndexElem{b->metric, b->dtype, b->dim, 0}, nlists, off, true, [&](pgv_index *ix) -> int {
            PGV_HIP(hipMemcpyAsync(ix->centers, b->centers.p, b->row_bytes() * (size_t)nlists, hipMemcpyDeviceToDevice,
                                   ctx->stream));
            return launch_build_gather(ctx, b->rows.p, keys_sorted, n, b->geom.nvec, ix->vectors,
                                       b->has_tids ? b->tids.as<uint64_t>() : nullptr, ix->tids);
        }, out_index);
    scratch.release();
    if (rc != PGV_OK) return rc;
    if (out_offsets) memcpy(out_offsets, off.data(), ob);
    b->rows.release();
    b->tids.release();
    b->lists.release();
    b->n = b->cap = b->assigned = 0;
    return PGV_OK;
}

int pgv_index_drain(pgv_index *ix, int64_t chunk_rows, pgv_rows_sink sink, void *arg) {
    if (!ix || !sink) PGV_FAIL(PGV_ERR_ARG, "pgv_index_drain: index/sink is NULL");
    PGV_NO_BIT_INDEX(ix, "pgv_index_drain");
    pgv_ctx *ctx = ix->ctx;
    PGV_HIP(hipSetDevice(ctx->device));
    const int64_t n = ix->nrows;
    if (n == 0) return PGV_OK;
    const size_t tight = (size_t)ix->dim * elem_size(ix->dtype), padded = ivf_rows(ix).row_bytes();
    if (chunk_rows <= 0) chunk_rows = (int64_t)std::max<size_t>(1, ((size_t)64 << 20) / tight);
    if (chunk_rows > n) chunk_rows = n;
    void *buf[2] = {nullptr, nullptr};
    hipEvent_t ev[2] = {nullptr, nullptr};
    const size_t piece = tight * (size_t)chunk_rows + sizeof(uint64_t) * (size_t)chunk_rows;
    int rc = PGV_OK;
    for (int i = 0; i < 2 && rc == PGV_OK; i++) {
        if (hipHostMalloc(&buf[i], piece, hipHostMallocDefault) != hipSuccess) rc = PGV_ERR_NOMEM;
        if (rc == PGV_OK && hipEventCreateWithFlags(&ev[i], hipEventDisableTiming) != hipSuccess) rc = PGV_ERR_DEVICE;
    }
    auto issue = [&](int64_t c, int slot) -> int {
        const int64_t r0 = c * chunk_rows, cnt = std::min(chunk_rows, n - r0);
        char *dst = static_cast<char *>(buf[slot]);
        const char *src = static_cast<const char *>(ix->vectors) + (size_t)r0 * padded;
        if (padded == tight)
            PGV_HIP(hipMemcpyAsync(dst, src, tight * (size_t)cnt, hipMemcpyDeviceToHost, ctx->stream));
        else
            PGV_HIP(hipMemcpy2DAsync(dst, tight, src, padded, tight, (size_t)cnt, hipMemcpyDeviceToHost, ctx->stream));
        if (ix->tids)
            PGV_HIP(hipMemcpyAsync(dst + tight * (size_t)chunk_rows, ix->tids + r0, sizeof(uint64_t) * (size_t)cnt,
                                   hipMemcpyDeviceToHost, ctx->stream));
        PGV_HIP(hipEventRecord(ev[slot], ctx->stream));
        return PGV_OK;
    };
    const int64_t nchunks = (n + chunk_rows - 1) / chunk_rows;
    if (rc == PGV_OK) rc = issue(0, 0);
    for (int64_t c = 0; c < nchunks && rc == PGV_OK; c++) {
        const int slot = (int)(c & 1);
        if (c + 1 < nchunks) rc = issue(c + 1, slot ^ 1);
        if (rc != PGV_OK) break;
        if (hipEventSynchronize(ev[slot]) != hipSuccess) {
            set_error("pgv_index_drain: copy failed");
            rc = PGV_ERR_DEVICE;
            break;
        }
        const int64_t r0 = c * chunk_rows, cnt = std::min(chunk_rows, n - r0);
        const char *p = static_cast<const char *>(buf[slot]);
        const int src = sink(arg, r0, cnt, p, ix->tids ? reinterpret_cast<const uint64_t *>(p + tight * (size_t)chunk_rows) : nullptr);
        if (src != 0) {
            set_error("pgv_index_drain: the sink returned %d", src);
            rc = PGV_ERR_STATE;
        }
    }
    (void)hipStreamSynchronize(ctx->stream);
    for (int i = 0; i < 2; i++) {
        if (ev[i]) (void)hipEventDestroy(ev[i]);
        if (buf[i]) (void)hipHostFree(buf[i]);
    }
    if (rc == PGV_ERR_NOMEM) set_error("pgv_index_drain: pinned buffers (2 x %zu bytes) could not be allocated", piece);
    return rc;
}

static void index_drop_lanes(pgv_index *ix);

int pgv_index_set_overlap(pgv_index *ix, int lanes) {
    if (!ix) PGV_FAIL(PGV_ERR_ARG, "pgv_index_set_overlap: index is NULL");
    PGV_NO_BIT_INDEX(ix, "pgv_index_set_overlap");
    if (lanes < 1 || lanes > 4) PGV_FAIL(PGV_ERR_ARG, "pgv_index_set_overlap: lanes %d outside 1..4", lanes);
    PGV_HIP(hipSetDevice(ix->ctx->device));
    PGV_TRY(pgv_ctx_sync(ix->ctx));
    index_drop_lanes(ix);
    if (lanes == 1) return PGV_OK;
    PGV_HIP(hipEventCreateWithFlags(&ix->lane_event, hipEventDisableTiming));
    PGV_HIP(hipEventCreateWithFlags(&ix->lane_scan_done, hipEventDisableTiming));
    for (int i = 0; i < lanes; i++) {
        pgv_ctx *lc = nullptr;
        pgv_index *v = nullptr;
        int rc = pgv_ctx_create(ix->ctx->device, nullptr, &lc);
        if (rc == PGV_OK) rc = pgv_index_share(ix, lc, &v);
        if (rc != PGV_OK) {
            if (lc) pgv_ctx_destroy(lc);
            index_drop_lanes(ix);
            return rc;
        }
        lc->no_mfma_scan = ix->ctx->no_mfma_scan;
        lc->bound_mode = ix->ctx->bound_mode;
        lc->assign_bound_mode = ix->ctx->assign_bound_mode;
        if (ix->ctx->profiling) (void)pgv_ctx_set_profiling(lc, 1);
        lc->scan_gate = ix->lane_scan_done;
        ix->lanes.push_back(v);
        ix->ctx->children.push_back(lc);
    }
    return PGV_OK;
}

int pgv_index_share(pgv_index *ix, pgv_ctx *ctx, pgv_index **out) {
    if (!ix || !ctx || !out) PGV_FAIL(PGV_ERR_ARG, "pgv_index_share: index/ctx/out is NULL");
    *out = nullptr;
    if (ctx->device != ix->ctx->device)
        PGV_FAIL(PGV_ERR_ARG, "pgv_index_share: the index lives on device %d, the context on %d", ix->ctx->device, ctx->device);
    pgv_index *v = new (std::nothrow) pgv_index(*ix);
    if (!v) PGV_FAIL(PGV_ERR_NOMEM, "out of host memory");
    v->ctx = ctx;
    v->lanes.clear();
    v->lane_next = 0;
    v->lane_event = nullptr;
    v->lane_scan_done = nullptr;
    __atomic_add_fetch(ix->refs, 1, __ATOMIC_RELAXED);
    *out = v;
    return PGV_OK;
}

struct IndexHandleWire {
    uint64_t magic;
    uint32_t abi, pid;
    int32_t device, metric, dtype, dim, nlists, has_tids;
    int64_t nrows;
    uint64_t arena_bytes;
    hipIpcMemHandle_t mem;
};
static_assert(sizeof(IndexHandleWire) <= PGV_INDEX_HANDLE_BYTES, "pgv_index_handle too small");
static constexpr uint64_t kIndexHandleMagic = 0x7067765f69786831ull;

int pgv_index_export(pgv_index *ix, pgv_index_handle *out) {
    if (!ix || !out) PGV_FAIL(PGV_ERR_ARG, "pgv_index_export: index/out is NULL");
    PGV_NO_BIT_INDEX(ix, "pgv_index_export");
    if (!ix->arena) PGV_FAIL(PGV_ERR_STATE, "pgv_index_export: the index has no device arrays");
    if (ix->imported) PGV_FAIL(PGV_ERR_STATE, "pgv_index_export: export from the process that uploaded the index");
    PGV_HIP(hipSetDevice(ix->ctx->device));
    IndexHandleWire w;
    memset(&w, 0, sizeof(w));
    w.magic = kIndexHandleMagic;
    w.abi = PGV_ABI_VERSION;
    w.pid = (uint32_t)getpid();
    w.device = ix->ctx->device;
    w.metric = ix->metric;
    w.dtype = ix->dtype;
    w.dim = ix->dim;
    w.nlists = ix->nlists;
    w.has_tids = ix->tids != nullptr;
    w.nrows = ix->nrows;
    w.arena_bytes = ix->arena_bytes;
    hipError_t e = hipIpcGetMemHandle(&w.mem, ix->arena);
    if (e != hipSuccess) {
        (void)hipGetLastError();
        PGV_FAIL(PGV_ERR_DEVICE,
                 "hipIpcGetMemHandle failed: %s (the driver here shares memory by dmabuf: HSA_ENABLE_IPC_MODE_LEGACY=0 "
                 "must be in the environment of every process)", hipGetErrorString(e));
    }
    memset(out, 0, sizeof(*out));
    memcpy(out->bytes, &w, sizeof(w));
    return PGV_OK;
}

int pgv_index_import(pgv_ctx *ctx, const pgv_index_handle *handle, pgv_index **out) {
    if (!ctx || !handle || !out) PGV_FAIL(PGV_ERR_ARG, "pgv_index_import: ctx/handle/out is NULL");
    *out = nullptr;
    IndexHandleWire w;
    memcpy(&w, handle->bytes, sizeof(w));
    if (w.magic != kIndexHandleMagic || w.abi != PGV_ABI_VERSION)
        PGV_FAIL(PGV_ERR_ARG, "pgv_index_import: not a handle of this library version");
    if (w.pid == (uint32_t)getpid())
        PGV_FAIL(PGV_ERR_STATE, "pgv_index_import: the handle was exported by this process (use pgv_index_share)");
    if (w.device != ctx->device)
        PGV_FAIL(PGV_ERR_ARG, "pgv_index_import: the index lives on device %d, the context on %d", w.device, ctx->device);
    PGV_TRY(check_common((pgv_dtype)w.dtype, w.dim));
    PGV_TRY(check_metric((pgv_metric)w.metric));
    if (w.nlists < 1 || w.nlists > 32768 || w.nrows < 0) PGV_FAIL(PGV_ERR_ARG, "pgv_index_import: corrupt handle");
    PGV_HIP(hipSetDevice(ctx->device));
    pgv_index *ix = new (std::nothrow) pgv_index();
    if (!ix) PGV_FAIL(PGV_ERR_NOMEM, "out of host memory");
    ix->refs = new (std::nothrow) int(1);
    if (!ix->refs) {
        delete ix;
        PGV_FAIL(PGV_ERR_NOMEM, "out of host memory");
    }
    ix->ctx = ctx;
    ix->metric = (pgv_metric)w.metric;
    ix->dtype = (pgv_dtype)w.dtype;
    ix->dim = w.dim;
    ix->nlists = w.nlists;
    ix->nrows = w.nrows;
    ix->geom = row_geom(w.dim, ix->dtype);
    ix->imported = true;
    IndexLayout lay = index_layout(w.nlists, w.nrows, ivf_rows(ix).row_bytes(), w.has_tids != 0, ix->metric == PGV_L2SQ);
    if (lay.bytes != w.arena_bytes) {
        pgv_index_free(ix);
        PGV_FAIL(PGV_ERR_ARG, "pgv_index_import: handle describes %llu bytes, this library lays the mirror out in %zu",
                 (unsigned long long)w.arena_bytes, lay.bytes);
    }
    hipError_t e = hipIpcOpenMemHandle(&ix->arena, w.mem, hipIpcMemLazyEnablePeerAccess);
    if (e != hipSuccess) {
        (void)hipGetLastError();
        ix->arena = nullptr;
        pgv_index_free(ix);
        PGV_FAIL(PGV_ERR_DEVICE, "hipIpcOpenMemHandle failed: %s (is the exporting process alive, and "
                 "HSA_ENABLE_IPC_MODE_LEGACY=0 set in both?)", hipGetErrorString(e));
    }
    ix->arena_bytes = lay.bytes;
    index_carve(ix, lay);
    ix->h_offsets.assign((size_t)w.nlists + 1, 0);
    if (hipMemcpy(ix->h_offsets.data(), ix->list_offsets, sizeof(int64_t) * ix->h_offsets.size(),
                  hipMemcpyDeviceToHost) != hipSuccess) {
        set_error("pgv_index_import: reading list_offsets failed: %s", hipGetErrorString(hipGetLastError()));
        pgv_index_free(ix);
        return PGV_ERR_DEVICE;
    }
    if (ix->h_offsets[0] != 0 || ix->h_offsets[w.nlists] != w.nrows) {
        pgv_index_free(ix);
        PGV_FAIL(PGV_ERR_DATA, "pgv_index_import: the shared mirror does not match its handle");
    }
    index_host_tables(ix);
    *out = ix;
    return PGV_OK;
}

static void index_drop_lanes(pgv_index *ix) {
    for (pgv_index *v : ix->lanes) {
        pgv_ctx *lc = v->ctx;
        if (ix->ctx) {
            auto &ch = ix->ctx->children;
            ch.erase(std::remove(ch.begin(), ch.end(), lc), ch.end());
        }
        pgv_index_free(v);
        pgv_ctx_destroy(lc);
    }
    ix->lanes.clear();
    if (ix->lane_event) (void)hipEventDestroy(ix->lane_event);
    ix->lane_event = nullptr;
    if (ix->lane_scan_done) (void)hipEventDestroy(ix->lane_scan_done);
    ix->lane_scan_done = nullptr;
}

void pgv_index_free(pgv_index *ix) {
    if (!ix) return;
    if (!ix->lanes.empty()) index_drop_lanes(ix);
    if (ix->ctx) (void)hipStreamSynchronize(ix->ctx->stream);
    if (ix->refs && __atomic_sub_fetch(ix->refs, 1, __ATOMIC_ACQ_REL) > 0) {
        delete ix;
        return;
    }
    if (ix->arena) {
        if (ix->imported)
            (void)hipIpcCloseMemHandle(ix->arena);
        else
            (void)hipFree(ix->arena);
    }
    if (ix->shadow) (void)hipFree(ix->shadow);
    delete ix->refs;
    delete ix;
}

int pgv_index_tids(pgv_index *ix, const int64_t *slots, int64_t n, uint64_t *out) {
    if (!ix || !out || (n > 0 && !slots)) PGV_FAIL(PGV_ERR_ARG, "pgv_index_tids: index/slots/out is NULL");
    if (!ix->tids) PGV_FAIL(PGV_ERR_STATE, "pgv_index_tids: the index was uploaded without tids");
    if (is_device_ptr(slots) || is_device_ptr(out)) PGV_FAIL(PGV_ERR_ARG, "pgv_index_tids: host arrays only");
    PGV_HIP(hipSetDevice(ix->ctx->device));
    int64_t i = 0;
    while (i < n) {
        if (slots[i] < 0 || slots[i] >= ix->nrows) PGV_FAIL(PGV_ERR_ARG, "pgv_index_tids: slot %lld out of range", (long long)slots[i]);
        int64_t j = i + 1;
        while (j < n && slots[j] == slots[j - 1] + 1) j++;
        if (slots[j - 1] >= ix->nrows) PGV_FAIL(PGV_ERR_ARG, "pgv_index_tids: slot %lld out of range", (long long)slots[j - 1]);
        PGV_HIP(hipMemcpyAsync(out + i, ix->tids + slots[i], sizeof(uint64_t) * (size_t)(j - i), hipMemcpyDeviceToHost,
                               ix->ctx->stream));
        i = j;
    }
    PGV_HIP(hipStreamSynchronize(ix->ctx->stream));
    return PGV_OK;
}

int64_t pgv_index_rows(const pgv_index *ix) { return ix ? ix->nrows : -1; }
int pgv_index_lists(const pgv_index *ix) { return ix ? ix->nlists : -1; }

static int rank_lists_impl(pgv_index *ix, const void *q_dev, int nq, int maxprobes,
                           int32_t *out_lists_dev, float *out_dist_dev, ShadowBatch *sb) {
    pgv_ctx *ctx = ix->ctx;
    PGV_TRY(ctx->dist_mat.ensure(sizeof(float) * (size_t)nq * ix->nlists));
    float *mat = ctx->dist_mat.as<float>();
    PGV_TRY(ctx->sel_a.ensure(sizeof(int64_t) * (size_t)nq * maxprobes));
    float *dist = out_dist_dev;
    if (!dist) {
        PGV_TRY(ctx->sel_b.ensure(sizeof(float) * (size_t)nq * maxprobes));
        dist = ctx->sel_b.as<float>();
    }
    int64_t *pos = ctx->sel_a.as<int64_t>();
    if (ix->nbits > 0) {
        ScanTimer timer{ctx};
        PGV_TRY(timer.begin((double)ix->nlists * nq, (double)ix->nlists * ((nq + 31) / 32), true));
        PGV_TRY(launch_hamming_tiles(ctx, ivf_centers(ix), q_dev, bit_query_bytes(ix->nbits), nq, mat));
        PGV_TRY(timer.end());
        PGV_TRY(launch_topk_segments(ctx, mat, nullptr, nq, ix->nlists, maxprobes, dist, pos));
        return launch_cast_pos_to_i32(ctx, pos, (int64_t)nq * maxprobes, out_lists_dev);
    }
    if (nq <= 24 && maxprobes <= query_head_cap()) {
        const int64_t cd_stride = ((int64_t)ix->nlists + 7) / 4 * 4;
        PGV_TRY(ctx->dist_mat.ensure(sizeof(float) * (size_t)nq * cd_stride));
        return launch_multi_rank(ctx, ix, q_dev, nq, ctx->dist_mat.as<float>(), cd_stride, maxprobes, out_lists_dev,
                                 out_dist_dev);
    }
    int cand = maxprobes + 16 < ix->nlists ? maxprobes + 16 : ix->nlists;
    const int rank_env = rank_shadow_env();
    const bool rank_sh = ix->metric == PGV_L2SQ && ix->cshadow && ix->dtype == PGV_F32 && rank_env != 0 && shadow_env() != 0;
    if (rank_sh && maxprobes + 54 <= 256) cand = maxprobes + 54 < ix->nlists ? maxprobes + 54 : ix->nlists;
    const bool mfma = nq >= 128 && ix->nlists >= 64 && !ctx->no_mfma_scan &&
                      (ix->metric == PGV_NEG_IP || (ix->metric == PGV_L2SQ && ix->center_norms && cand <= 256));
    if (mfma && ix->metric == PGV_L2SQ) {
        ShadowBatch own;
        if (!sb) sb = &own;
        const bool scan_follows = sb->scan_follows;
        if (rank_sh) {
            PGV_TRY(shadow_batch_cast(ix, q_dev, nq, maxprobes, true, scan_follows, sb));
            PGV_TRY(dense_scan(ctx, ivf_shadow_centers(ix), sb->qcast, nq, ix->nlists, mat, true, ix->center_norms, nullptr,
                               sb->cscale));
        } else {
            PGV_TRY(dense_scan(ctx, ivf_centers(ix), q_dev, nq, ix->nlists, mat, true, ix->center_norms, nullptr));
        }
        ExactTail tail;
        tail.pair_t = (rank_sh && rank_env == 1 && scan_follows) ? sb->pair_t : nullptr;
        PlanBuffers pbuf;
        if (tail.pair_t) {
            PGV_TRY(plan_batch_reserve(ctx, ix->nlists, nq, maxprobes, &pbuf));
            tail.emit = {pbuf.cnt, pbuf.probe_off, pbuf.seg_len, ix->list_offsets};
        }
        tail.rows = {ix->centers, nullptr, nullptr, ix->geom, ix->dtype,
                     reinterpret_cast<const unsigned *>(ix->center_norms + ix->nlists)};
        tail.queries = q_dev;
        tail.nq = nq;
        tail.kprime = cand;
        tail.k = maxprobes;
        tail.approx = mat;
        tail.fixed_len = ix->nlists;
        tail.bound = scan_bound_chain(ctx, ix->geom.ld, scan_chain_length(ix->geom, ix->dtype, false));
        if (rank_sh) tail.bound = shadow_band(ix->geom.ld, tail.bound.g_ref);
        tail.eps_add = rank_sh ? sb->ceps : nullptr;
        tail.out_dist = dist;
        tail.out_i32 = out_lists_dev;
        PGV_TRY(launch_exact_tail(ctx, tail, ctx->ms_b));
        sb->pairs_done = tail.pair_t != nullptr;
        return PGV_OK;
    } else {
        PGV_TRY(dense_scan(ctx, ivf_centers(ix), q_dev, nq, ix->nlists, mat, mfma, nullptr, nullptr));
        PGV_TRY(launch_topk_segments(ctx, mat, nullptr, nq, ix->nlists, maxprobes, dist, pos));
    }
    PGV_TRY(launch_cast_pos_to_i32(ctx, pos, (int64_t)nq * maxprobes, out_lists_dev));
    return PGV_OK;
}

int rank_lists_dev(pgv_index *ix, const void *q_dev, int nq, int maxprobes, int32_t *out_lists_dev, float *out_dist_dev) {
    return rank_lists_impl(ix, q_dev, nq, maxprobes, out_lists_dev, out_dist_dev, nullptr);
}

int pgv_rank_lists(pgv_index *ix, const void *queries, int nq, int maxprobes, int32_t *out_lists,
                   float *out_dist) {
    if (!ix || !out_lists) PGV_FAIL(PGV_ERR_ARG, "pgv_rank_lists: index/out_lists is NULL");
    if (nq < 0) PGV_FAIL(PGV_ERR_ARG, "nq < 0");
    if (maxprobes < 1 || maxprobes > ix->nlists)
        PGV_FAIL(PGV_ERR_ARG, "maxprobes %d outside 1..lists (%d)", maxprobes, ix->nlists);
    if (nq == 0) return PGV_OK;
    if (!queries) PGV_FAIL(PGV_ERR_ARG, "queries is NULL");
    pgv_ctx *ctx = ix->ctx;
    PGV_HIP(hipSetDevice(ctx->device));
    const void *q_dev;
    PGV_TRY(stage_queries(ix, queries, nq, &q_dev));
    OutArg ol, od;
    PGV_TRY(ol.init(out_lists, sizeof(int32_t) * (size_t)nq * maxprobes, ctx->out_stage));
    PGV_TRY(od.init(out_dist, sizeof(float) * (size_t)nq * maxprobes, ctx->out_stage2));
    PGV_TRY(rank_lists_dev(ix, q_dev, nq, maxprobes, ol.as<int32_t>(), od.as<float>()));
    bool need = false;
    PGV_TRY(ol.finish(ctx, &need));
    PGV_TRY(od.finish(ctx, &need));
    return sync_if(ctx, need);
}

static int scan_turn_begin(pgv_ctx *ctx) {
    if (ctx->scan_gate) PGV_HIP(hipStreamWaitEvent(ctx->stream, ctx->scan_gate, 0));
    return PGV_OK;
}
static int scan_turn_end(pgv_ctx *ctx) {
    if (ctx->scan_gate) PGV_HIP(hipEventRecord(ctx->scan_gate, ctx->stream));
    return PGV_OK;
}

struct ScanPath {
    bool bits = false;
    bool per_query = false;
    bool use_mfma = false;
    bool use_tile = false;
    bool wide = false;
    int qt = 0, rows_per_task = 0;
    bool approx = false;
    bool shadow = false;
};
static ScanPath scan_path(const pgv_index *ix, int nq, int probes, int k) {
    ScanPath p;
    const double share = (double)nq * probes / (double)ix->nlists;
    if (ix->nbits > 0) {
        p.bits = true;
        p.qt = hamming_list_group_size(share);
        p.rows_per_task = hamming_list_rows_per_task();
        return p;
    }
    p.per_query = (share <= 0.4 || nq <= 4) && nq <= 1024 && probes <= query_max_batch_lists() && k <= query_head_cap();
    if (p.per_query) return p;
    p.use_mfma = share > 3.0 && k <= 192 && !ix->ctx->no_mfma_scan &&
                 (ix->metric == PGV_NEG_IP || (ix->metric == PGV_L2SQ && ix->row_norms));
    p.use_tile = !p.use_mfma && tile_scan_supported(ix->geom) && share > 8.0;
    static const int wide_env = [] {
        const char *e = getenv("PGV_SCAN_WIDE");
        return e ? atoi(e) : -1;
    }();
    p.wide = p.use_mfma && (wide_env < 0 ? share > 12.0 : wide_env != 0);
    p.qt = p.use_mfma ? (p.wide ? mfma_scan_queries_per_task_wide() : mfma_scan_queries_per_task())
                      : (p.use_tile ? tile_scan_queries_per_task()
                                    : scan_group_size(ix->geom, ix->dtype, (int)std::ceil(share)));
    constexpr int rpt_tiles = 20;
    p.rows_per_task = p.use_mfma ? mfma_scan_rows_per_task()
                                 : (p.use_tile ? rpt_tiles * tile_scan_tile_rows(ix->geom)
                                               : (p.qt >= 16 ? 256 : (p.qt >= 4 ? 128 : 64)));
    p.approx = p.use_mfma && ix->metric == PGV_L2SQ;
    p.shadow = p.approx && ix->shadow && shadow_env() != 0;
    return p;
}

static int list_scan_step(pgv_index *ix, const ScanPath &path, const ScanWork &work, const void *queries, const float *qscale,
                          double counted, float *out) {
    pgv_ctx *ctx = ix->ctx;
    const RowsView v = path.shadow ? ivf_shadow_rows(ix) : ivf_rows(ix);
    PGV_TRY(scan_turn_begin(ctx));
    ScanTimer timer{ctx};
    PGV_TRY(timer.begin(counted, counted));
    if (path.bits)
        PGV_TRY(launch_hamming_lists(ctx, v, queries, bit_query_bytes(ix->nbits), work, path.qt, out));
    else if (path.use_mfma)
        PGV_TRY(launch_mfma_scan(ctx, v, queries, work, ix->row_norms, nullptr, out, rows_stream_past_caches(v), path.qt,
                                 path.shadow ? qscale : nullptr));
    else if (path.use_tile)
        PGV_TRY(launch_tile_scan(ctx, v, queries, work, out));
    else
        PGV_TRY(launch_scan(ctx, v, queries, work, path.qt, out));
    PGV_TRY(timer.end());
    return scan_turn_end(ctx);
}

static int scan_batch_impl(pgv_index *ix, const void *q_dev, int nq, const int32_t *probe_lists, int probes,
                           int k, float *out_dist, int64_t *out_slot, uint64_t *out_tid, ShadowBatch *sb) {
    pgv_ctx *ctx = ix->ctx;
    const ScanPath path = scan_path(ix, nq, probes, k);
    if (path.per_query) {
        const int64_t bound = ix->len_prefix[probes];
        const int64_t seg_stride = (bound + 7) / 4 * 4;
        PGV_TRY(ctx->plan_d.ensure(sizeof(float) * (size_t)nq * seg_stride));
        OutArg od, os, ot;
        PGV_TRY(od.init(out_dist, sizeof(float) * (size_t)nq * k, ctx->out_stage));
        PGV_TRY(os.init(out_slot, sizeof(int64_t) * (size_t)nq * k, ctx->out_stage2));
        PGV_TRY(ot.init(out_tid, sizeof(uint64_t) * (size_t)nq * k, ctx->sel_b));
        PGV_TRY(scan_turn_begin(ctx));
        ScanTimer timer{ctx};
        PGV_TRY(timer.begin(0.0, 0.0));
        PGV_TRY(launch_multi_scan(ctx, ix, q_dev, nq, probe_lists, probes, bound, ctx->plan_d.as<float>(), seg_stride, k,
                                  od.as<float>(), os.as<int64_t>(), ot.as<uint64_t>()));
        PGV_TRY(timer.end());
        PGV_TRY(scan_turn_end(ctx));
        bool need = false;
        PGV_TRY(od.finish(ctx, &need));
        PGV_TRY(os.finish(ctx, &need));
        PGV_TRY(ot.finish(ctx, &need));
        return sync_if(ctx, need);
    }
    ShadowBatch own;
    if (!sb) sb = &own;
    if (path.shadow && !sb->cast_for_scan) PGV_TRY(shadow_batch_cast(ix, q_dev, nq, probes, false, true, sb));
    const float *pair_t = (path.shadow && sb->pairs_done) ? sb->pair_t : nullptr;
    PlanResult plan;
    PGV_TRY(launch_plan_batch(ctx, ix, probe_lists, nq, probes, path.qt, path.rows_per_task, ctx->profiling, &plan, pair_t,
                              pair_t != nullptr));
    if (path.shadow) {
        if (!pair_t)
            PGV_TRY(launch_shadow_pairs(ctx, ix->geom, q_dev, ix->centers, plan.pair_start, ix->nlists, (int64_t)nq * probes,
                                        plan.pairs));
        ctx->scan_shadow_queries += nq;
    }

    PGV_TRY(ctx->plan_d.ensure(sizeof(float) * (size_t)(plan.out_bound > 0 ? plan.out_bound : 1)));
    float *seg_vals = ctx->plan_d.as<float>();
    if (plan.ntasks_bound > 0)
        PGV_TRY(list_scan_step(ix, path, plan.work(), path.shadow ? sb->qcast : q_dev, sb->qscale, 0.0, seg_vals));

    OutArg od, os, ot;
    PGV_TRY(od.init(out_dist, sizeof(float) * (size_t)nq * k, ctx->out_stage));
    PGV_TRY(os.init(out_slot, sizeof(int64_t) * (size_t)nq * k, ctx->out_stage2));
    PGV_TRY(ot.init(out_tid, sizeof(uint64_t) * (size_t)nq * k, ctx->sel_b));
    PGV_TRY(ctx->sel_a.ensure(sizeof(int64_t) * (size_t)nq * k));
    int64_t *pos = ctx->sel_a.as<int64_t>();
    if (path.approx) {
        ExactTail tail;
        tail.rows = {ix->vectors, ix->tids, ix->list_offsets, ix->geom, ix->dtype,
                     reinterpret_cast<const unsigned *>(ix->row_norms + ix->nrows)};
        tail.queries = q_dev;
        tail.nq = nq;
        tail.kprime = approx_candidates(k);
        tail.k = k;
        tail.approx = seg_vals;
        tail.probe_lists = probe_lists;
        tail.probe_off = plan.probe_off;
        tail.probes = probes;
        tail.seg_start = plan.seg_start;
        tail.seg_bound = ix->len_prefix[probes];
        tail.bound = scan_bound_chain(ctx, ix->geom.ld, scan_chain_length(ix->geom, ix->dtype, path.wide));
        if (path.shadow) tail.bound = shadow_band(ix->geom.ld, tail.bound.g_ref);
        tail.eps_add = path.shadow ? sb->qeps : nullptr;
        tail.out_dist = od.as<float>();
        tail.out_slot = os.as<int64_t>();
        tail.out_tid = ot.as<uint64_t>();
        PGV_TRY(launch_exact_tail(ctx, tail, ctx->ms_a));
    } else {
        PGV_TRY(launch_topk_segments(ctx, seg_vals, plan.seg_start, nq, 0, k, od.as<float>(), pos, nullptr, nullptr, 0,
                                     ix->len_prefix[probes]));
        PGV_TRY(launch_positions_to_slots(ctx, ix, probe_lists, plan.probe_off, nq, probes, k, pos,
                                          os.as<int64_t>(), ot.as<uint64_t>()));
    }
    bool need = false;
    PGV_TRY(od.finish(ctx, &need));
    PGV_TRY(os.finish(ctx, &need));
    PGV_TRY(ot.finish(ctx, &need));
    return sync_if(ctx, need);
}

int scan_batch_dev(pgv_index *ix, const void *q_dev, int nq, const int32_t *probe_lists, int probes, int k, float *out_dist,
                   int64_t *out_slot, uint64_t *out_tid) {
    return scan_batch_impl(ix, q_dev, nq, probe_lists, probes, k, out_dist, out_slot, out_tid, nullptr);
}

int pgv_scan_lists(pgv_index *ix, const void *query, const int32_t *lists, int nlists,
                   float *out_dist, int64_t *out_slot, int64_t capacity, int64_t *out_count) {
    if (!ix || !out_count) PGV_FAIL(PGV_ERR_ARG, "pgv_scan_lists: index/out_count is NULL");
    if (nlists < 0 || (nlists > 0 && !lists)) PGV_FAIL(PGV_ERR_ARG, "bad list array");
    pgv_ctx *ctx = ix->ctx;
    PGV_HIP(hipSetDevice(ctx->device));

    std::vector<int32_t> hl((size_t)nlists);
    if (nlists) {
        if (is_device_ptr(lists))
            PGV_HIP(hipMemcpy(hl.data(), lists, sizeof(int32_t) * (size_t)nlists, hipMemcpyDeviceToHost));
        else
            memcpy(hl.data(), lists, sizeof(int32_t) * (size_t)nlists);
    }
    int64_t m = 0;
    for (int p = 0; p < nlists; p++) {
        if (hl[p] < 0 || hl[p] >= ix->nlists) PGV_FAIL(PGV_ERR_ARG, "list id %d out of range", hl[p]);
        m += ix->h_offsets[hl[p] + 1] - ix->h_offsets[hl[p]];
    }
    *out_count = m;
    if (m > capacity) PGV_FAIL(PGV_ERR_ARG, "output capacity %lld < %lld tuples", (long long)capacity, (long long)m);
    if (m == 0) return PGV_OK;
    if (!out_dist || !out_slot) PGV_FAIL(PGV_ERR_ARG, "out_dist/out_slot is NULL");

    OutArg od, os;
    PGV_TRY(od.init(out_dist, sizeof(float) * (size_t)m, ctx->out_stage));
    PGV_TRY(os.init(out_slot, sizeof(int64_t) * (size_t)m, ctx->out_stage2));

    ScanPath path;
    path.bits = ix->nbits > 0;
    path.qt = path.bits ? hamming_list_group_size(1.0) : 1;
    path.rows_per_task = path.bits ? hamming_list_rows_per_task() : rows_per_task_for(ctx, m, 1);
    const int ch = path.rows_per_task;
    int64_t ntasks = 0;
    for (int p = 0; p < nlists; p++) {
        int64_t len = ix->h_offsets[hl[p] + 1] - ix->h_offsets[hl[p]];
        ntasks += (len + ch - 1) / ch;
    }
    const size_t tb = sizeof(ScanTask) * (size_t)ntasks, pb = sizeof(ScanPair) * (size_t)nlists,
                 ob = sizeof(int64_t) * (size_t)nlists, lb = sizeof(int32_t) * (size_t)nlists;
    PGV_TRY(staging_acquire(ctx));
    PGV_TRY(ctx->h_a.ensure(tb + pb + ob + lb + 16));
    char *hb = ctx->h_a.as<char>();
    ScanTask *ht = reinterpret_cast<ScanTask *>(hb);
    ScanPair *hp = reinterpret_cast<ScanPair *>(hb + tb);
    int64_t *hoff = reinterpret_cast<int64_t *>(hb + tb + pb);
    int32_t *hlist = reinterpret_cast<int32_t *>(hb + tb + pb + ob);
    int *hn = reinterpret_cast<int *>(hb + tb + pb + ob + lb);
    int64_t t = 0, run = 0;
    for (int p = 0; p < nlists; p++) {
        const int64_t beg = ix->h_offsets[hl[p]], len = ix->h_offsets[hl[p] + 1] - beg;
        hp[p].out_rel = run - beg;
        hp[p].query = 0;
        hp[p].pad = 0;
        hoff[p] = run;
        hlist[p] = hl[p];
        for (int64_t c = 0; c * ch < len; c++) {
            ht[t].row0 = beg + c * ch;
            int64_t left = len - c * ch;
            ht[t].nrows = (int)(left < ch ? left : ch);
            ht[t].pair0 = p;
            ht[t].npairs = 1;
            ht[t].pad = 0;
            t++;
        }
        run += len;
    }
    *hn = (int)ntasks;
    const size_t total = tb + pb + ob + lb + 16;
    PGV_TRY(ctx->tasks.ensure(total));
    PGV_HIP(hipMemcpyAsync(ctx->tasks.p, hb, total, hipMemcpyHostToDevice, ctx->stream));
    char *db = ctx->tasks.as<char>();

    PGV_TRY(launch_iota_slots(ctx, ix, reinterpret_cast<int32_t *>(db + tb + pb + ob), nlists,
                              reinterpret_cast<int64_t *>(db + tb + pb), os.as<int64_t>()));
    if (query == nullptr) {
        PGV_HIP(hipMemsetAsync(od.dev, 0, sizeof(float) * (size_t)m, ctx->stream));
    } else {
        const void *q_dev;
        PGV_TRY(stage_queries(ix, query, 1, &q_dev));
        const ScanWork work{reinterpret_cast<ScanTask *>(db), reinterpret_cast<int *>(db + tb + pb + ob + lb), (int)ntasks,
                            reinterpret_cast<ScanPair *>(db + tb)};
        PGV_TRY(list_scan_step(ix, path, work, q_dev, nullptr, (double)m, od.as<float>()));
    }
    bool need = true;
    PGV_TRY(od.finish(ctx, &need));
    PGV_TRY(os.finish(ctx, &need));
    return sync_if(ctx, need);
}

int check_batch_args(pgv_index *ix, const void *queries, int nq, int probes, int k, float *out_dist,
                            uint64_t *out_tid, const char *who) {
    if (!ix) PGV_FAIL(PGV_ERR_ARG, "%s: index is NULL", who);
    if (nq < 0 || k < 1) PGV_FAIL(PGV_ERR_ARG, "bad nq/k");
    if (probes < 1 || probes > ix->nlists)
        PGV_FAIL(PGV_ERR_ARG, "probes %d outside 1..lists (%d)", probes, ix->nlists);
    if (out_tid && !ix->tids) PGV_FAIL(PGV_ERR_STATE, "index was uploaded without tids");
    if (nq > 0 && (!queries || !out_dist)) PGV_FAIL(PGV_ERR_ARG, "queries/out_dist is NULL");
    return PGV_OK;
}

int pgv_search_batch(pgv_index *ix, const void *queries, int nq, int probes, int k, float *out_dist,
                     int64_t *out_slot, uint64_t *out_tid) {
    PGV_TRY(check_batch_args(ix, queries, nq, probes, k, out_dist, out_tid, "pgv_search_batch"));
    if (nq == 0) return PGV_OK;
    if (!ix->lanes.empty()) {
        pgv_index *lane = ix->lanes[ix->lane_next++ % ix->lanes.size()];
        PGV_HIP(hipSetDevice(ix->ctx->device));
        PGV_HIP(hipEventRecord(ix->lane_event, ix->ctx->stream));
        PGV_HIP(hipStreamWaitEvent(lane->ctx->stream, ix->lane_event, 0));
        return pgv_search_batch(lane, queries, nq, probes, k, out_dist, out_slot, out_tid);
    }
    pgv_ctx *ctx = ix->ctx;
    PGV_HIP(hipSetDevice(ctx->device));
    const void *q_dev;
    PGV_TRY(stage_queries(ix, queries, nq, &q_dev));
    PGV_TRY(ctx->idx_stage.ensure(sizeof(int32_t) * (size_t)nq * probes));
    int32_t *probe_lists = ctx->idx_stage.as<int32_t>();
    ShadowBatch sb;
    sb.scan_follows = scan_path(ix, nq, probes, k).shadow;
    PGV_TRY(rank_lists_impl(ix, q_dev, nq, probes, probe_lists, nullptr, &sb));
    return scan_batch_impl(ix, q_dev, nq, probe_lists, probes, k, out_dist, out_slot, out_tid, &sb);
}

int pgv_scan_batch(pgv_index *ix, const void *queries, int nq, const int32_t *probe_lists, int probes, int k,
                   float *out_dist, int64_t *out_slot, uint64_t *out_tid) {
    PGV_TRY(check_batch_args(ix, queries, nq, probes, k, out_dist, out_tid, "pgv_scan_batch"));
    if (nq == 0) return PGV_OK;
    if (!probe_lists) PGV_FAIL(PGV_ERR_ARG, "probe_lists is NULL");
    pgv_ctx *ctx = ix->ctx;
    PGV_HIP(hipSetDevice(ctx->device));
    if (!is_device_ptr(probe_lists)) {
        for (size_t i = 0; i < (size_t)nq * probes; i++)
            if (probe_lists[i] < 0 || probe_lists[i] >= ix->nlists)
                PGV_FAIL(PGV_ERR_ARG, "probe list id %d out of range 0..%d", probe_lists[i], ix->nlists - 1);
    }
    const void *q_dev, *pl_dev;
    PGV_TRY(stage_queries(ix, queries, nq, &q_dev));
    PGV_TRY(stage_flat(ctx, probe_lists, sizeof(int32_t) * (size_t)nq * probes, ctx->idx_stage, &pl_dev));
    return scan_batch_dev(ix, q_dev, nq, static_cast<const int32_t *>(pl_dev), probes, k, out_dist, out_slot,
                          out_tid);
}

int pgv_index_shadow_cast(pgv_index *ix, const void *queries, int nq, void *out_qcast, float *out_qscale, float *out_qeps,
                          float *out_cscale, float *out_ceps) {
    if (!ix || !queries || nq < 1) PGV_FAIL(PGV_ERR_ARG, "pgv_index_shadow_cast: index/queries is NULL or nq < 1");
    PGV_NO_BIT_INDEX(ix, "pgv_index_shadow_cast");
    if (!ix->shadow || !ix->cshadow) PGV_FAIL(PGV_ERR_STATE, "pgv_index_shadow_cast: the index has no fp16 shadow");
    pgv_ctx *ctx = ix->ctx;
    PGV_HIP(hipSetDevice(ctx->device));
    const void *q_dev;
    PGV_TRY(stage_rows(ctx, queries, nq, ix->dim, ix->dtype, ix->geom, ctx->q_stage, &q_dev));
    ShadowBatch sb;
    PGV_TRY(shadow_batch_cast(ix, q_dev, nq, 1, true, true, &sb));
    const struct {
        void *dst;
        const void *src;
        size_t bytes;
    } parts[] = {{out_qcast, sb.qcast, (size_t)nq * ix->shadow_geom.ld * sizeof(uint16_t)},
                 {out_qscale, sb.qscale, sizeof(float) * (size_t)nq},
                 {out_qeps, sb.qeps, sizeof(float) * (size_t)nq},
                 {out_cscale, sb.cscale, sizeof(float) * (size_t)nq},
                 {out_ceps, sb.ceps, sizeof(float) * (size_t)nq}};
    for (const auto &p : parts)
        if (p.dst) PGV_HIP(hipMemcpyAsync(p.dst, p.src, p.bytes, hipMemcpyDefault, ctx->stream));
    PGV_HIP(hipStreamSynchronize(ctx->stream));
    return PGV_OK;
}

namespace {

struct QueryHeadHost {
    long long total;
    int count;
    unsigned seq;
};

static int g_scan_gate_width = -1;
static PgvGate g_scan_gate;
static void scan_gate_enter() {
    if (g_scan_gate_width < 0) {
        const char *e = getenv("PGV_MAX_INFLIGHT_SCANS");
        __atomic_store_n(&g_scan_gate_width, e ? atoi(e) : 16, __ATOMIC_RELAXED);
    }
    g_scan_gate.enter(g_scan_gate_width);
}
static void scan_gate_leave() { g_scan_gate.leave(g_scan_gate_width); }
struct ScanGate {
    ScanGate() { scan_gate_enter(); }
    ~ScanGate() { scan_gate_leave(); }
};

int wait_head(pgv_ctx *ctx, pgv_query *q, unsigned seq) {
    volatile QueryHeadHost *h = static_cast<volatile QueryHeadHost *>(q->head_pinned);
    for (int spin = 0; spin < 200000; spin++) {
        if (__atomic_load_n(&h->seq, __ATOMIC_ACQUIRE) == seq) return PGV_OK;
        __builtin_ia32_pause();
    }
    PGV_HIP(hipStreamSynchronize(ctx->stream));
    if (__atomic_load_n(&h->seq, __ATOMIC_ACQUIRE) != seq) PGV_FAIL(PGV_ERR_DEVICE, "query kernel did not report");
    return PGV_OK;
}

void copy_head(pgv_query *q, int stride, int n, float *out_dist, int64_t *out_slot, uint64_t *out_tid) {
    const char *base = static_cast<const char *>(q->head_pinned) + 64;
    if (out_slot) memcpy(out_slot, base, sizeof(int64_t) * (size_t)n);
    if (out_tid) memcpy(out_tid, base + (size_t)stride * 8, sizeof(uint64_t) * (size_t)n);
    if (out_dist) memcpy(out_dist, base + (size_t)stride * 16, sizeof(float) * (size_t)n);
}

}

static bool query_direct_enabled() {
    static const bool on = [] {
        const char *e = getenv("PGV_QUERY_DIRECT");
        return !(e && e[0] == '0');
    }();
    return on;
}

int pgv_query_begin(pgv_index *ix, pgv_query **out) {
    if (!ix || !out) PGV_FAIL(PGV_ERR_ARG, "pgv_query_begin: index/out is NULL");
    *out = nullptr;
    PGV_NO_BIT_INDEX(ix, "pgv_query_begin");
    pgv_ctx *ctx = ix->ctx;
    PGV_HIP(hipSetDevice(ctx->device));
    pgv_query *q = new (std::nothrow) pgv_query();
    if (!q) PGV_FAIL(PGV_ERR_NOMEM, "out of host memory");
    q->ix = ix;
    const int cap = query_head_cap();
    const size_t state_bytes = sizeof(int32_t) * (size_t)cap + sizeof(float) * ((size_t)ix->nlists + 4);
    const size_t row_bytes = ivf_rows(ix).row_bytes();
    q->head_bytes = query_head_bytes(cap);
    int rc = q->state.ensure(state_bytes);
    if (rc == PGV_OK) rc = q->q_dev.ensure(row_bytes);
    if (rc == PGV_OK && hipHostMalloc(&q->q_pinned, row_bytes, hipHostMallocDefault) != hipSuccess) rc = PGV_ERR_NOMEM;
    if (rc == PGV_OK && hipHostMalloc(&q->head_pinned, q->head_bytes, hipHostMallocDefault) != hipSuccess)
        rc = PGV_ERR_NOMEM;
    if (rc == PGV_OK && hipMemsetAsync(q->state.p, 0, state_bytes, ctx->stream) != hipSuccess) rc = PGV_ERR_DEVICE;
    int large_bar = 0;
    if (rc == PGV_OK && query_direct_enabled() &&
        hipDeviceGetAttribute(&large_bar, hipDeviceAttributeIsLargeBar, ctx->device) == hipSuccess && large_bar) {
        if (hipExtMallocWithFlags(&q->q_direct, row_bytes, hipDeviceMallocFinegrained) != hipSuccess) {
            (void)hipGetLastError();
            q->q_direct = nullptr;
        }
    }
    if (rc != PGV_OK) {
        set_error("pgv_query_begin: allocation failed");
        pgv_query_end(q);
        return rc;
    }
    memset(q->head_pinned, 0, q->head_bytes);
    q->lists = q->state.as<int32_t>();
    q->cdist = reinterpret_cast<float *>(q->lists + cap);
    *out = q;
    return PGV_OK;
}

void pgv_query_end(pgv_query *q) {
    if (!q) return;
    if (q->ix && q->ix->ctx) (void)hipStreamSynchronize(q->ix->ctx->stream);
    q->state.release();
    q->seg.release();
    q->q_dev.release();
    if (q->q_pinned) (void)hipHostFree(q->q_pinned);
    if (q->q_direct) (void)hipFree(q->q_direct);
    if (q->head_pinned) (void)hipHostFree(q->head_pinned);
    delete q;
}

int pgv_query_rank(pgv_query *q, const void *query, int max_probes) {
    if (!q) PGV_FAIL(PGV_ERR_ARG, "pgv_query_rank: q is NULL");
    pgv_index *ix = q->ix;
    pgv_ctx *ctx = ix->ctx;
    if (max_probes < 1 || max_probes > ix->nlists)
        PGV_FAIL(PGV_ERR_ARG, "maxprobes %d outside 1..lists (%d)", max_probes, ix->nlists);
    if (max_probes > query_head_cap())
        PGV_FAIL(PGV_ERR_ARG, "pgv_query_rank handles up to %d probes; use pgv_rank_lists", query_head_cap());
    PGV_HIP(hipSetDevice(ctx->device));
    q->max_probes = max_probes;
    q->is_null = query == nullptr;
    q->cur_n = 0;
    if (q->is_null) return launch_query_iota(ctx, q->lists, max_probes);
    const size_t tight = (size_t)ix->dim * elem_size(ix->dtype), row_bytes = ivf_rows(ix).row_bytes();
    if (is_device_ptr(query)) {
        PGV_HIP(hipMemsetAsync(q->q_dev.p, 0, row_bytes, ctx->stream));
        PGV_HIP(hipMemcpyAsync(q->q_dev.p, query, tight, hipMemcpyDeviceToDevice, ctx->stream));
        q->q_row = q->q_dev.p;
    } else {
        if (q->rank_pending) PGV_HIP(hipStreamSynchronize(ctx->stream));
        void *dst = q->q_direct ? q->q_direct : q->q_pinned;
        memcpy(dst, query, tight);
        if (row_bytes > tight) memset(static_cast<char *>(dst) + tight, 0, row_bytes - tight);
        if (q->q_direct) {
            __builtin_ia32_sfence();
            q->q_row = q->q_direct;
        } else {
            PGV_TRY(launch_query_stage(ctx, q->q_pinned, q->q_dev.p, ix->geom.nvec));
            q->q_row = q->q_dev.p;
        }
    }
    q->rank_pending = true;
    return launch_query_rank(ctx, ix, q->q_row, q->cdist, max_probes, q->lists);
}

int pgv_query_scan(pgv_query *q, int first, int nprobes, int head, float *out_dist, int64_t *out_slot,
                   uint64_t *out_tid, int *out_count, int64_t *out_total) {
    if (!q || !out_count) PGV_FAIL(PGV_ERR_ARG, "pgv_query_scan: q/out_count is NULL");
    pgv_index *ix = q->ix;
    pgv_ctx *ctx = ix->ctx;
    if (q->max_probes <= 0) PGV_FAIL(PGV_ERR_STATE, "pgv_query_scan before pgv_query_rank");
    if (first < 0 || nprobes < 1 || first + nprobes > q->max_probes)
        PGV_FAIL(PGV_ERR_ARG, "lists [%d, %d) outside the %d ranked", first, first + nprobes, q->max_probes);
    if (nprobes > query_max_batch_lists())
        PGV_FAIL(PGV_ERR_ARG, "pgv_query_scan handles up to %d lists per batch; use pgv_scan_lists", query_max_batch_lists());
    if (head < 1 || head > query_head_cap()) PGV_FAIL(PGV_ERR_ARG, "head %d outside 1..%d", head, query_head_cap());
    if (out_tid && !ix->tids) PGV_FAIL(PGV_ERR_STATE, "index was uploaded without tids");
    PGV_HIP(hipSetDevice(ctx->device));
    const int64_t bound = ix->len_prefix[nprobes];
    PGV_TRY(q->seg.ensure(sizeof(float) * (size_t)(bound + 4)));
    const unsigned seq = ++q->seq ? q->seq : ++q->seq;
    ScanGate gate;
    PGV_TRY(launch_query_scan(ctx, ix, q->is_null ? nullptr : q->q_row, q->lists + first, nprobes, bound,
                              q->seg.as<float>()));
    PGV_TRY(launch_query_head(ctx, ix, q->seg.as<float>(), q->lists + first, nprobes, 0, head, q->head_pinned, seq));
    q->cur_first = first;
    q->cur_n = nprobes;
    PGV_TRY(wait_head(ctx, q, seq));
    q->rank_pending = false;
    const QueryHeadHost *h = static_cast<const QueryHeadHost *>(q->head_pinned);
    *out_count = h->count;
    if (out_total) *out_total = h->total;
    copy_head(q, head, h->count, out_dist, out_slot, out_tid);
    return PGV_OK;
}

int pgv_query_more(pgv_query *q, int skip, int count, float *out_dist, int64_t *out_slot, uint64_t *out_tid,
                   int *out_count) {
    if (!q || !out_count) PGV_FAIL(PGV_ERR_ARG, "pgv_query_more: q/out_count is NULL");
    pgv_index *ix = q->ix;
    pgv_ctx *ctx = ix->ctx;
    if (q->cur_n <= 0) PGV_FAIL(PGV_ERR_STATE, "pgv_query_more before pgv_query_scan");
    if (skip < 0 || count < 1 || skip + count > query_head_cap())
        PGV_FAIL(PGV_ERR_ARG, "skip + count = %d exceeds %d; fetch the batch with pgv_scan_lists", skip + count,
                 query_head_cap());
    if (out_tid && !ix->tids) PGV_FAIL(PGV_ERR_STATE, "index was uploaded without tids");
    PGV_HIP(hipSetDevice(ctx->device));
    const unsigned seq = ++q->seq ? q->seq : ++q->seq;
    PGV_TRY(launch_query_head(ctx, ix, q->seg.as<float>(), q->lists + q->cur_first, q->cur_n, skip, count,
                              q->head_pinned, seq));
    PGV_TRY(wait_head(ctx, q, seq));
    const QueryHeadHost *h = static_cast<const QueryHeadHost *>(q->head_pinned);
    *out_count = h->count;
    copy_head(q, count, h->count, out_dist, out_slot, out_tid);
    return PGV_OK;
}

int pgv_query_lists(pgv_query *q, int32_t *out_lists, int n) {
    if (!q || !out_lists) PGV_FAIL(PGV_ERR_ARG, "pgv_query_lists: NULL argument");
    if (n < 0 || n > q->max_probes) PGV_FAIL(PGV_ERR_ARG, "%d lists asked, %d ranked", n, q->max_probes);
    pgv_ctx *ctx = q->ix->ctx;
    PGV_HIP(hipSetDevice(ctx->device));
    PGV_HIP(hipMemcpyAsync(out_lists, q->lists, sizeof(int32_t) * (size_t)n,
                           is_device_ptr(out_lists) ? hipMemcpyDeviceToDevice : hipMemcpyDeviceToHost, ctx->stream));
    PGV_HIP(hipStreamSynchronize(ctx->stream));
    q->rank_pending = false;
    return PGV_OK;
}

}
```

pgvector_amd/csrc/pgv_internal.h:

```cpp
#pragma once

#include <hip/hip_runtime.h>

#include <cstdint>
#include <cstdio>
#include <cstdlib>
#include <cstring>
#include <cmath>
#include <vector>

#include "../../include/pgv_hip.h"

namespace pgv {

void set_error(const char *fmt, ...) __attribute__((format(printf, 1, 2)));

#define PGV_FAIL(code, ...)            \
    do {                               \
        ::pgv::set_error(__VA_ARGS__); \
        return (code);                 \
    } while (0)

#define PGV_HIP(call)                                                                  \
    do {                                                                               \
        hipError_t e__ = (call);                                                       \
        if (e__ != hipSuccess) {                                                       \
            ::pgv::set_error("%s failed: %s (%s:%d)", #call, hipGetErrorString(e__),   \
                             __FILE__, __LINE__);                                      \
            return e__ == hipErrorOutOfMemory ? PGV_ERR_NOMEM : PGV_ERR_DEVICE;        \
        }                                                                              \
    } while (0)

#define PGV_TRY(call)          \
    do {                       \
        int rc__ = (call);     \
        if (rc__ != PGV_OK)    \
            return rc__;       \
    } while (0)

struct DBuf {
    void *p = nullptr;
    size_t cap = 0;
    int ensure(size_t bytes);
    void release();
    template <typename T> T *as() const { return static_cast<T *>(p); }
};

struct HBuf {
    void *p = nullptr;
    size_t cap = 0;
    int ensure(size_t bytes);
    void release();
    template <typename T> T *as() const { return static_cast<T *>(p); }
};

bool is_device_ptr(const void *p);

constexpr int kVecBytes = 16;

constexpr int kHnswMaxBits = 64000;
constexpr int kIvfMaxBits = 64000;

inline int elem_size(pgv_dtype t) { return t == PGV_F32 ? 4 : 2; }
inline int padded_dim(int dim, pgv_dtype t) {
    int per = kVecBytes / elem_size(t);
    return (dim + per - 1) / per * per;
}

struct RowGeom {
    int ld;
    int nvec;
    int lpr_log2;
    int nchunks;
};
RowGeom row_geom(int dim, pgv_dtype t);
RowGeom bit_row_geom(int nbits);

enum class RowKind { F32, F16, Bits };
struct RowsView {
    const void *rows;
    int64_t n;
    RowGeom geom;
    RowKind kind;
    pgv_metric metric;
    bool bits() const { return kind == RowKind::Bits; }
    pgv_dtype dtype() const { return kind == RowKind::F16 ? PGV_F16 : PGV_F32; }
    size_t row_bytes() const { return bits() ? (size_t)geom.ld : (size_t)geom.ld * elem_size(dtype()); }
};
inline RowKind row_kind(pgv_dtype t) { return t == PGV_F16 ? RowKind::F16 : RowKind::F32; }

struct HnswGraph {
    void *mem = nullptr;
    size_t bytes = 0;
    const int32_t *levels = nullptr;
    const int64_t *nbr_start = nullptr;
    int32_t *nbr = nullptr;
    int64_t nbr_total = 0;
    int m = 0;
    int32_t entry = -1;
};

struct ScanTask {
    int64_t row0;
    int32_t nrows;
    int32_t pair0;
    int32_t npairs;
    int32_t pad;
};
struct ScanPair {
    int64_t out_rel;
    int32_t query;
    int32_t pad;
};
struct ScanWork {
    const ScanTask *tasks;
    const int *ntasks_dev;
    int ntasks_bound;
    const ScanPair *pairs;
};

}

struct pgv_ctx {
    int device = 0;
    hipStream_t stream = nullptr;
    bool own_stream = false;
    int num_cus = 256;
    hipEvent_t ev0 = nullptr, ev1 = nullptr;
    pgv::DBuf q_stage, rows_stage, centers_stage, out_stage, out_stage2, idx_stage;
    pgv::DBuf tasks, pairs, counters, plan_a, plan_b, plan_c, plan_d, dist_mat, sel_a, sel_b;
    pgv::DBuf km_a, km_b, km_c, km_d, km_e, km_f, km_g;
    pgv::DBuf ms_b;
    pgv::DBuf dense_plan;
    int64_t dense_plan_rows = -1, dense_plan_stride = -1;
    int dense_plan_nq = -1, dense_plan_kind = -1;
    bool counters_clean = false;
    pgv::DBuf ms_a;
    pgv::DBuf sh_q;
    pgv::DBuf mf_d;
    pgv::DBuf mf_a, mf_b, mf_c, zeros;
    pgv::DBuf stats_dev;
    pgv::HBuf h_a, h_b, h_c;
    hipEvent_t h_a_busy = nullptr;
    bool h_a_pending = false;
    bool profiling = false;
    bool no_mfma_scan = false;
    bool no_widen = false;
    int bound_mode = 1;
    int assign_bound_mode = 1;
    pgv::DBuf xt_norms;
    std::vector<hipEvent_t> ev_pool;
    size_t ev_used = 0;
    double scan_ms = 0.0;
    int64_t scan_launches = 0;
    double scan_pairs = 0.0;
    double scan_rows = 0.0;
    std::vector<char> ev_is_aux;
    double aux_ms = 0.0;
    int64_t aux_launches = 0;
    double aux_pairs = 0.0;
    double scan_shadow_queries = 0.0;
    std::vector<pgv_ctx *> children;
    hipEvent_t scan_gate = nullptr;
};

struct pgv_index {
    pgv_ctx *ctx = nullptr;
    pgv_metric metric = PGV_L2SQ;
    pgv_dtype dtype = PGV_F32;
    int dim = 0;
    int nbits = 0;
    int nlists = 0;
    int64_t nrows = 0;
    pgv::RowGeom geom{};
    void *centers = nullptr;
    void *vectors = nullptr;
    int64_t *list_offsets = nullptr;
    uint64_t *tids = nullptr;
    float *row_norms = nullptr;
    float *center_norms = nullptr;
    int *refs = nullptr;
    void *arena = nullptr;
    size_t arena_bytes = 0;
    bool imported = false;
    void *shadow = nullptr;
    pgv::RowGeom shadow_geom{};
    int shadow_s = 0;
    double shadow_E = 0.0;
    double shadow_P = 0.0;
    void *cshadow = nullptr;
    int cshadow_s = 0;
    double cshadow_E = 0.0;
    double cshadow_P = 0.0;
    std::vector<int64_t> h_offsets;
    std::vector<int64_t> len_prefix;
    int64_t max_list_len = 0;
    std::vector<pgv_index *> lanes;
    unsigned lane_next = 0;
    hipEvent_t lane_event = nullptr;
    hipEvent_t lane_scan_done = nullptr;
};

struct pgv_query {
    pgv_index *ix = nullptr;
    pgv::DBuf state;
    pgv::DBuf seg;
    pgv::DBuf q_dev;
    void *q_pinned = nullptr;
    const void *q_row = nullptr;
    void *q_direct = nullptr;
    void *head_pinned = nullptr;
    size_t head_bytes = 0;
    int32_t *lists = nullptr;
    float *cdist = nullptr;
    int max_probes = 0;
    bool is_null = false;
    bool rank_pending = false;
    int cur_first = 0, cur_n = 0;
    unsigned seq = 0;
};

struct HnswElements {
    pgv_metric metric = PGV_L2SQ;
    pgv_dtype dtype = PGV_F32;
    int dim = 0;
    int nbits = 0;
    int64_t n = 0;
    pgv::RowGeom geom{};
    void *elements = nullptr;
    char *payload = nullptr;
    int payload_bytes = 0;
};

struct pgv_hnsw : HnswElements {
    pgv_ctx *ctx = nullptr;
    pgv::HnswGraph graph;
    pgv::DBuf bitmaps;
    bool imported = false;
    pgv_hnsw *view_of = nullptr;
    hipEvent_t graph_ev = nullptr;
    bool graph_ev_set = false;
    struct HnswLinkState *link = nullptr;
};

namespace pgv {
inline RowsView hnsw_rows(const pgv_hnsw *h) {
    return {h->elements, h->n, h->geom, h->nbits > 0 ? RowKind::Bits : row_kind(h->dtype), h->metric};
}
inline RowsView ivf_rows(const pgv_index *ix) {
    return {ix->vectors, ix->nrows, ix->geom, ix->nbits > 0 ? RowKind::Bits : row_kind(ix->dtype), ix->metric};
}
inline RowsView ivf_centers(const pgv_index *ix) {
    RowsView v = ivf_rows(ix);
    v.rows = ix->centers;
    v.n = ix->nlists;
    return v;
}
inline RowsView ivf_shadow_rows(const pgv_index *ix) { return {ix->shadow, ix->nrows, ix->shadow_geom, RowKind::F16, ix->metric}; }
inline RowsView ivf_shadow_centers(const pgv_index *ix) {
    return {ix->cshadow, ix->nlists, ix->shadow_geom, RowKind::F16, ix->metric};
}
}

struct HnswLinkState {
    float *nb_dist = nullptr;
    uint8_t *nb_flag = nullptr;
    int *list_count = nullptr;
    int *list_rec = nullptr;
    size_t nlists = 0;
    int64_t *stats_dev = nullptr, *stats_host = nullptr;
    pgv::DBuf rec, links, ids, pa, pb, tri, mm, loc, sel;
    int nrec = 0, nq = 0, lcap = 0;
    int64_t npairs = 0;
    bool prepared = false;
    int32_t *rec_owner = nullptr, *rec_lc = nullptr, *rec_nstart = nullptr, *rec_from = nullptr, *rec_wait = nullptr,
            *rec_list = nullptr;
    int64_t *rec_off = nullptr, *rec_pos = nullptr, *ids_start = nullptr, *pair_start = nullptr, *mm_start = nullptr,
            *totals = nullptr;
    int *rec_fill = nullptr, *blocked = nullptr, *nrec_dev = nullptr;
    int32_t *d_link_elem = nullptr;
    float *d_link_dist = nullptr;
    int32_t *d_sel_ids = nullptr, *d_sel_cnt = nullptr, *d_elems = nullptr;
    float *d_sel_dist = nullptr;
    uint8_t *d_sel_closer = nullptr, *d_linked = nullptr;
    struct Kept {
        pgv::DBuf ids, dist, cnt, elems;
        int nq = 0, ef = 0, lcap = 0;
    } kept[2];
};

namespace pgv {

struct ScanBound {
    float g_sq, g_dot, g_norm, g_ref;
};
struct ShadowTerms {
    int s;
    double E, P;
    double g_dot, g_pair, g_cn;
};
struct RankShadowTerms {
    int s;
    double E, P;
    double g_dot, g_cn;
};
inline float gamma_n(double n, double v) { return (float)(n * v / (1.0 - n * v)); }
inline int pair_chain_length(const RowGeom &g32) {
    const int by_pair_kernel = (g32.ld + 63) / 64 + 6;
    const int per_lane = (g32.nvec + (1 << g32.lpr_log2) - 1) >> g32.lpr_log2;
    const int by_recheck = 4 * ((per_lane + 1) / 2) + 1 + g32.lpr_log2;
    return by_pair_kernel > by_recheck ? by_pair_kernel : by_recheck;
}
inline ScanBound scan_bound(const pgv_ctx *ctx, int dim) {
    if (ctx->bound_mode == 0) return {8.f * std::sqrt((float)dim + 4.f) * 5.9604645e-8f, 0.f, 0.f, 0.f};
    constexpr double v = 5.9604645e-8;
    return {0.f, gamma_n(dim / 4.0 + 4.0, v), gamma_n(dim / 64.0 + 10.0, v), 2.f * gamma_n(dim + 2.0, v)};
}
inline ScanBound scan_bound_chain(const pgv_ctx *ctx, int dim, int chain) {
    ScanBound b = scan_bound(ctx, dim);
    if (ctx->bound_mode != 0) b.g_dot = gamma_n(chain + 4.0, 5.9604645e-8);
    return b;
}
inline ScanBound shadow_band(int ld, float g_ref, double u = 5.9604645e-8) {
    return {0.f, 0.f, gamma_n(ld / 64.0 + 10.0, u), g_ref};
}
struct ExpansionBound {
    float gamma;
    float gamma_exact;
};
inline ExpansionBound argmin_bound(const pgv_ctx *ctx, int dim) {
    constexpr float u = 5.9604645e-8f;
    if (ctx->assign_bound_mode == 0) return {8.f * std::sqrt((float)dim + 4.f) * u, 0.f};
    const float n1 = (float)(dim + 1) * u, n2 = (float)(dim + 2) * u;
    return {n1 / (1.f - n1), n2 / (1.f - n2)};
}

int launch_scan(pgv_ctx *ctx, const RowsView &v, const void *queries, const ScanWork &w, int qt, float *out);
int scan_group_size(const RowGeom &g, pgv_dtype dtype, int wanted);
int launch_score_gather(pgv_ctx *ctx, const RowsView &v, const void *queries, const int32_t *slot, const int32_t *query_of,
                        int64_t npairs, float *out);
int launch_score_groups(pgv_ctx *ctx, const RowsView &v, const int32_t *ids, const int64_t *ids_at, int64_t ids_stride,
                        const int32_t *n_arr, const int32_t *from_arr, const int64_t *pair_at, int ngroups, float *out);
int launch_expand_groups(pgv_ctx *ctx, const int32_t *ids, const int64_t *ids_at, int64_t ids_stride, const int32_t *n_arr,
                         const int32_t *from_arr, const int64_t *pair_at, int ngroups, int32_t *a, int32_t *b);

int launch_cosine(pgv_ctx *ctx, pgv_dtype dtype, const RowGeom &g, const void *rows, const void *query, int64_t n,
                  double *out);
int launch_bit_distance(pgv_ctx *ctx, int mode, const RowGeom &g, const void *rows, const void *query, int64_t n,
                        double *out);

int bit_topk_slice_bytes();
inline int bit_query_bytes(int nbits) {
    const int slice = bit_topk_slice_bytes();
    return ((nbits + 7) / 8 + slice - 1) / slice * slice;
}
int launch_hamming_tiles(pgv_ctx *ctx, const RowsView &v, const void *queries, int qbytes, int nq, float *out);
int hamming_list_group_size(double queries_per_list);
int hamming_list_rows_per_task();
int launch_hamming_lists(pgv_ctx *ctx, const RowsView &v, const void *queries, int qbytes, const ScanWork &w, int qt,
                         float *out);
int launch_bit_closest(pgv_ctx *ctx, const float *mat, int k, const float *best_val, const int64_t *best_pos, int n,
                       bool sticky, int32_t *closest_io, float *out_dist, int32_t *counts, unsigned long long *changes);
int launch_bit_sums(pgv_ctx *ctx, const void *samples, int ld, int nbits, int n, const int32_t *closest, int32_t *sums);
int launch_bit_centers(pgv_ctx *ctx, const int32_t *sums, const int32_t *counts, int k, int nbits, int ld,
                       const int32_t *refill_row, const uint8_t *refill, void *centers);
int launch_binary_quantize(pgv_ctx *ctx, pgv_dtype dtype, int dim, const void *rows, int64_t n, void *out_bits);
int launch_rerank_pairs(pgv_ctx *ctx, const int64_t *cand, int64_t total, int kc, int32_t *slot, int32_t *query_of);
int launch_rerank_mask(pgv_ctx *ctx, const int64_t *cand, int64_t total, float *vals);
int launch_rerank_map(pgv_ctx *ctx, const int64_t *cand, int nq, int kc, int k, const int64_t *pos, int64_t *out_idx);

struct SparseCsr {
    const int64_t *ptr;
    const int32_t *idx;
    const float *val;
    int64_t n;
};
struct SparseTile {
    int64_t elem0;
    int32_t q0, nq, nnz, pad;
};
int sparse_tile_nnz();
int sparse_tile_queries();
int sparse_reg_row_nnz();
void sparse_plan_tiles(const int64_t *q_ptr, int nq, std::vector<SparseTile> *tiles, int *max_q_nnz);
int launch_sparse_tiles(pgv_ctx *ctx, int mode, const SparseTile *tiles_dev, int ntiles, int max_tile_nnz, int max_tile_nq,
                        int max_q_nnz, const SparseCsr &q, const SparseCsr &r, void *out, int64_t out_stride);

int hnsw_search_grid(pgv_ctx *ctx, int nq, int64_t n, int *words_out);
struct HnswSearchArgs {
    const void *queries = nullptr;
    const int32_t *qids = nullptr;
    const int32_t *qlevels = nullptr;
    int nq = 0, ef = 0, k = 0;
    int64_t *out_elem = nullptr;
    float *out_dist = nullptr;
    int64_t *out_scored = nullptr;
    int32_t *lw_ids = nullptr;
    float *lw_dist = nullptr;
    int32_t *lw_cnt = nullptr;
    int lcap = 0;
};
int launch_hnsw_search(pgv_ctx *ctx, const RowsView &v, const HnswGraph &graph, const HnswSearchArgs &a, uint32_t *bitmaps,
                       int words, int grid, int *counter);
int launch_hnsw_patch(pgv_ctx *ctx, const HnswGraph &graph, int64_t n, const int32_t *ids, const int64_t *packed_off,
                      const int32_t *packed, int nupd);

bool tile_scan_supported(const RowGeom &g);
int tile_scan_queries_per_task();
int tile_scan_tile_rows(const RowGeom &g);
int launch_tile_scan(pgv_ctx *ctx, const RowsView &v, const void *queries, const ScanWork &w, float *out);

int launch_argmin(pgv_ctx *ctx, pgv_metric metric, pgv_dtype dtype, const RowGeom &g,
                  const void *rows, int64_t n, const void *centers, int k, int32_t *out_idx,
                  float *out_val);
int launch_argmin_mode(pgv_ctx *ctx, int mode, pgv_dtype dtype, const RowGeom &g,
                       const void *rows, int64_t n, const void *centers, int k,
                       int32_t *out_idx, float *out_val);

int launch_argmin_listed(pgv_ctx *ctx, int mode, pgv_dtype dtype, const RowGeom &g, const void *rows, int64_t n,
                         const void *centers, int k, const int32_t *row_list, const int *row_count,
                         unsigned long long *packed);
int launch_hnsw_select_plan(pgv_ctx *ctx, const int32_t *cnt, int ngroups, int lcap, int m, int64_t *pair_start);
int launch_hnsw_select(pgv_ctx *ctx, const int32_t *lw_ids, const float *lw_dist, const int32_t *cnt, const int32_t *qlevels,
                       const int64_t *pair_start, const float *tri, int ngroups, int lcap, int ef, int m, int stride,
                       int32_t *out_ids, float *out_dist, uint8_t *out_closer, int32_t *out_cnt);
int launch_hnsw_link_group(pgv_ctx *ctx, int step, const HnswGraph &graph, const int32_t *elems, const uint8_t *linked, int nq,
                           int lcap, const int32_t *sel_ids, const float *sel_dist, const int32_t *sel_cnt, int *list_count,
                           int *list_rec, int *nrec, int32_t *rec_owner, int32_t *rec_lc, int32_t *rec_list,
                           const int64_t *rec_off, int *rec_fill, int32_t *link_elem, float *link_dist);
int launch_hnsw_link_size(pgv_ctx *ctx, const HnswGraph &graph, const uint8_t *nb_flag, const int32_t *rec_owner,
                          const int32_t *rec_lc, const int32_t *rec_list, const int *list_count, int64_t *rec_off, int nrec,
                          int pass, int64_t *rec_pos, int32_t *rec_nstart, int32_t *rec_from, const int32_t *rec_wait,
                          int64_t *size_ids, int64_t *size_pairs);
int launch_hnsw_link_scan(pgv_ctx *ctx, int64_t *a, int64_t *b, int64_t *c, int n, int64_t *totals);
int launch_hnsw_link_stats(pgv_ctx *ctx, const int *blocked, const int64_t *totals, int64_t *stats);
int launch_hnsw_link_pairs(pgv_ctx *ctx, const int32_t *nbr, const int64_t *rec_pos, const int32_t *rec_nstart,
                           const int32_t *rec_from, const int64_t *rec_off, int32_t *link_elem, float *link_dist,
                           const int32_t *rec_list, int *list_count, int nrec, int pass,
                           const int64_t *ids_start, int32_t *ids, const int64_t *pair_start, int32_t *a, int32_t *b);
int launch_hnsw_link_replay(pgv_ctx *ctx, const HnswGraph &graph, float *nb_dist, uint8_t *nb_flag, int nrec, int pass,
                            const int32_t *rec_lc, const int64_t *rec_off, const float *link_dist, const int64_t *rec_pos,
                            const int32_t *rec_nstart, const int32_t *rec_from, const int64_t *ids_start, const int32_t *ids,
                            const int64_t *pair_start, const float *tri, const int64_t *mm_start, const float *mm,
                            int32_t *rec_wait, int16_t *loc_save, int *blocked);
int launch_hnsw_link_new(pgv_ctx *ctx, const HnswGraph &graph, float *nb_dist, uint8_t *nb_flag, const int32_t *elems,
                         const uint8_t *linked, int nq, int lcap, const int32_t *sel_ids, const float *sel_dist,
                         const uint8_t *sel_closer, const int32_t *sel_cnt);
bool mfma_argmin_supported(int mode, int64_t n, int k);
int launch_argmin_mfma(pgv_ctx *ctx, int mode, pgv_dtype dtype, const RowGeom &g, const void *rows, int64_t n,
                       const void *centers, int k, int32_t *out_idx, float *out_val);

int mfma_scan_rows_per_task();
int mfma_scan_queries_per_task();
int launch_mfma_dense(pgv_ctx *ctx, pgv_metric metric, pgv_dtype dtype, const RowGeom &g, const void *rows, int64_t n,
                      const void *queries, int nq, const float *row_norms, float *out, int64_t out_stride);
int dense_chain_length(const RowGeom &g, pgv_dtype dtype);
int launch_row_norms(pgv_ctx *ctx, const RowsView &v, float *out, unsigned *max_bits);
int launch_mfma_scan(pgv_ctx *ctx, const RowsView &v, const void *queries, const ScanWork &w, const float *row_norms,
                     const float *query_norms, float *out, bool stream_rows, int queries_per_task = 32,
                     const float *shadow_scale = nullptr);
int launch_shadow_build(pgv_ctx *ctx, const RowGeom &g32, const RowGeom &g16, const void *rows, const void *centers,
                        const int64_t *list_off, int nlists, int64_t n, void *shadow, void *words);
int shadow_scale_of(float max_abs);
int shadow_chain_length(const RowGeom &g16);
int scan_chain_length(const RowGeom &g, pgv_dtype dtype, bool wide);
int launch_shadow_query(pgv_ctx *ctx, const RowGeom &g32, const RowGeom &g16, const void *queries, int nq,
                        const ShadowTerms &st, const RankShadowTerms &rt, const float *center_norm_max,
                        const float *row_norm_max, void *qcast, float *qscale, float *qeps, float *cscale, float *ceps);
int launch_shadow_pairs(pgv_ctx *ctx, const RowGeom &g32, const void *queries, const void *centers,
                        const int64_t *pair_start, int nlists, int64_t npairs, ScanPair *pairs);
int mfma_scan_queries_per_task_wide();

int launch_gather_words(pgv_ctx *ctx, const void *src, int words_per_row, int64_t nrows, const int64_t *idx, int n,
                        uint32_t *out);
size_t build_sort_scratch_bytes(int64_t n, int key_bits);
int launch_build_order(pgv_ctx *ctx, const int32_t *lists, int64_t n, int nlists, unsigned long long *keys_tmp,
                       unsigned long long *keys_sorted, unsigned long long *counts, int64_t *offsets, int *bad,
                       void *sort_scratch, size_t sort_scratch_bytes);
int launch_build_gather(pgv_ctx *ctx, const void *src_rows, const unsigned long long *keys_sorted, int64_t n, int nvec,
                        void *dst_rows, const uint64_t *src_tids, uint64_t *dst_tids);

struct PlanResult {
    ScanTask *tasks = nullptr;
    ScanPair *pairs = nullptr;
    int *ntasks_dev = nullptr;
    int64_t ntasks = 0;
    int64_t total_out = 0;
    int64_t ntasks_bound = 0;
    int64_t out_bound = 0;
    int64_t *seg_start = nullptr;
    int64_t *probe_off = nullptr;
    int64_t *pair_start = nullptr;
    ScanWork work() const { return {tasks, ntasks_dev, (int)ntasks_bound, pairs}; }
};
struct PlanBuffers {
    int *cnt = nullptr, *fill = nullptr;
    int64_t *probe_off = nullptr, *seg_len = nullptr;
    int64_t *seg_start = nullptr, *pair_start = nullptr, *task_start = nullptr, *totals = nullptr;
};
int plan_batch_reserve(pgv_ctx *ctx, int nlists, int nq, int probes, PlanBuffers *pb);
struct PlanEmit {
    int *cnt = nullptr;
    int64_t *probe_off = nullptr, *seg_len = nullptr;
    const int64_t *list_off = nullptr;
};
int launch_plan_batch(pgv_ctx *ctx, const pgv_index *ix, const int32_t *probe_lists, int nq,
                      int probes, int qt, int rows_per_task, bool read_totals, PlanResult *res,
                      const float *pair_t = nullptr, bool counted = false);
int launch_topk_segments(pgv_ctx *ctx, const float *vals, const int64_t *seg_start, int nseg,
                         int64_t fixed_len, int k, float *out_val, int64_t *out_pos, int32_t *zero_word = nullptr,
                         int32_t *zero_range = nullptr, int zero_n = 0, int64_t len_bound = 0);
int launch_positions_to_slots(pgv_ctx *ctx, const pgv_index *ix, const int32_t *probe_lists,
                              const int64_t *probe_off, int nq, int probes, int k,
                              const int64_t *pos, int64_t *out_slot, uint64_t *out_tid);
struct ExactRows {
    const void *vectors;
    const uint64_t *tids;
    const int64_t *list_offsets;
    pgv::RowGeom geom;
    pgv_dtype dtype;
    const unsigned *norm_max;
};
struct ExactTail {
    ExactRows rows;
    const void *queries = nullptr;
    int nq = 0;
    int kprime = 0;
    int k = 0;
    float *approx = nullptr;
    const int32_t *probe_lists = nullptr;
    const int64_t *probe_off = nullptr;
    int probes = 0;
    const int64_t *seg_start = nullptr;
    int64_t seg_bound = 0;
    int64_t fixed_len = 0;
    ScanBound bound{};
    const float *eps_add = nullptr;
    float *out_dist = nullptr;
    int64_t *out_slot = nullptr;
    uint64_t *out_tid = nullptr;
    int32_t *out_i32 = nullptr;
    float *pair_t = nullptr;
    PlanEmit emit;
    bool dense() const { return probe_lists == nullptr; }
};
int launch_exact_tail(pgv_ctx *ctx, const ExactTail &t, DBuf &scratch);
int launch_iota_slots(pgv_ctx *ctx, const pgv_index *ix, const int32_t *lists_dev, int nlists,
                      const int64_t *probe_off, int64_t *out_slot);

int query_max_batch_lists();
int query_head_cap();
size_t query_head_bytes(int head);
int launch_query_stage(pgv_ctx *ctx, const void *src_pinned, void *dst_dev, int nvec);
int launch_multi_rank(pgv_ctx *ctx, const pgv_index *ix, const void *q_dev, int nq, float *cdist, int64_t cd_stride,
                      int max_probes, int32_t *out_lists, float *out_dist);
int launch_multi_scan(pgv_ctx *ctx, const pgv_index *ix, const void *q_dev, int nq, const int32_t *probe_lists, int nprobes,
                      int64_t rows_bound, float *seg, int64_t seg_stride, int k, float *out_dist, int64_t *out_slot,
                      uint64_t *out_tid);
int launch_query_iota(pgv_ctx *ctx, int32_t *out, int n);
int launch_one_query_rows(pgv_ctx *ctx, const RowsView &v, const void *q_dev, float *out);
int launch_query_rank(pgv_ctx *ctx, const pgv_index *ix, const void *q_dev, float *cdist, int max_probes,
                      int32_t *out_lists);
int launch_query_scan(pgv_ctx *ctx, const pgv_index *ix, const void *q_dev, const int32_t *probe_lists, int nprobes,
                      int64_t rows_bound, float *seg);
int launch_query_head(pgv_ctx *ctx, const pgv_index *ix, const float *seg, const int32_t *probe_lists, int nprobes,
                      int skip, int count, void *head_rec, unsigned seq);

int launch_merge_heads(pgv_ctx *ctx, const float *dist_all, const uint64_t *tid_all, int nranks, int nq, int k,
                       float *out_dist, uint64_t *out_tid);

int launch_cast_pos_to_i32(pgv_ctx *ctx, const int64_t *pos, int64_t n, int32_t *out);

int kmpp_block_count(int n);
int launch_kmpp_update(pgv_ctx *ctx, const float *raw, float *weight, int n, int spherical,
                       double *block_sums);
int launch_kmpp_pick(pgv_ctx *ctx, const RowGeom &g, const void *samples, int n,
                     const float *weight, const double *block_sums, const double *draws,
                     int round, void *centers, int32_t *picked);
int launch_kmpp_total(pgv_ctx *ctx, const double *block_sums, int nblocks, double *out);
int launch_kmpp_pick_sharded(pgv_ctx *ctx, const RowGeom &g, const void *samples, int n, const float *weight,
                             const double *block_sums, const double *totals, const int64_t *counts, int nranks, int rank,
                             const double *draws, int round, void *send_row, int32_t *owner_out);
int launch_kmpp_take_row(pgv_ctx *ctx, const RowGeom &g, const void *gathered, const int32_t *owner, void *centers,
                         int round);
int launch_lloyd_pack(pgv_ctx *ctx, const int32_t *counts, const unsigned long long *changes, int k, float *tail);
int launch_lloyd_unpack(pgv_ctx *ctx, const float *tail, int k, int32_t *counts, unsigned long long *changes,
                        long long *host_rec, long long seq);
int launch_changes_hist(pgv_ctx *ctx, const int32_t *closest_new, int32_t *closest_io, int n,
                        int32_t *counts, unsigned long long *changes);
int launch_members(pgv_ctx *ctx, const int32_t *closest, int n, int k, const int32_t *counts,
                   int32_t *offsets, int32_t *members);
int launch_center_sums(pgv_ctx *ctx, pgv_dtype dtype, const RowGeom &g, const void *samples,
                       const int32_t *offsets, const int32_t *members, int k, float *sums);
int launch_finish_centers(pgv_ctx *ctx, pgv_dtype dtype, const RowGeom &g, int k, int dim,
                          const float *sums, const int32_t *counts, const float *refill,
                          const int32_t *refill_row, void *centers);
int launch_normalize_rows(pgv_ctx *ctx, pgv_dtype dtype, const RowGeom &g, void *rows, int64_t n,
                          int dim, int32_t *flag);
int launch_check_centers(pgv_ctx *ctx, pgv_dtype dtype, const RowGeom &g, const void *centers,
                         int k, int dim, int check_zero_norm, int32_t *flag);

}
```

Measured before the change: 1.506 million.

## Fuse fallback fix pass into recheck kernel and reuse precomputed query norms

Merges the separate batch_fix kernel into batch_recheck, so queries whose candidate band overflows redo their work in the same block instead of being flagged and handled by a second launch. The query squared norm is now computed in the shadow query kernel and passed in, which removes a per-block reduction over the query row. Per-query probe offsets and list bases are staged into LDS for the slot binary search, and tids are prefetched. Merging the launches drops one kernel and the flags round trip, but the recheck kernel now needs dynamic shared memory and can run the heavy fallback path inside one block, which may unbalance work across blocks.

```diff
diff --git a/pgvector_amd/csrc/kernels_query.hip b/pgvector_amd/csrc/kernels_query.hip
--- a/pgvector_amd/csrc/kernels_query.hip
+++ b/pgvector_amd/csrc/kernels_query.hip
@@ -91,12 +91,10 @@
 }
 
 __device__ __forceinline__ void fill_pair_terms(const char *vectors, size_t row_bytes, const char *qrow, int ld,
-                                                const int32_t *slots_i32, const int64_t *slots_i64, int k,
-                                                float *__restrict__ pair_t) {
+                                                const int64_t *row_slots, int k, float *__restrict__ pair_t) {
     const int lane = threadIdx.x & (kWave - 1);
     for (int i = threadIdx.x >> 6; i < k; i += kQWaves) {
-        const int64_t slot = slots_i32 ? (int64_t)__hip_atomic_load(slots_i32 + i, __ATOMIC_RELAXED, __HIP_MEMORY_SCOPE_AGENT)
-                                       : __hip_atomic_load(slots_i64 + i, __ATOMIC_RELAXED, __HIP_MEMORY_SCOPE_AGENT);
+        const int64_t slot = row_slots[i];
         float a = 0.f;
         if (slot >= 0) {
             const float *x = reinterpret_cast<const float *>(qrow);
@@ -327,31 +325,184 @@
 }
 
 constexpr int kRecheckCap = 256;
+constexpr int kWide = kRecheckCap;
+
+constexpr int kSlotTab = 64;
+struct SlotMap {
+    int64_t off[kSlotTab];
+    int64_t beg[kSlotTab];
+};
+
+struct SlotOf {
+    const SlotMap *map;
+    const int64_t *off;
+    const int32_t *pl;
+    const int64_t *list_off;
+    int probes;
+    __device__ __forceinline__ int64_t operator()(int64_t j) const {
+        if (!pl) return j;
+        int lo = 0, hi = probes - 1;
+        if (map) {
+            while (lo < hi) {
+                const int mid = (lo + hi + 1) >> 1;
+                if (map->off[mid] <= j)
+                    lo = mid;
+                else
+                    hi = mid - 1;
+            }
+            return map->beg[lo] + (j - map->off[lo]);
+        }
+        while (lo < hi) {
+            const int mid = (lo + hi + 1) >> 1;
+            if (off[mid] <= j)
+                lo = mid;
+            else
+                hi = mid - 1;
+        }
+        return list_off[pl[lo]] + (j - off[lo]);
+    }
+};
+
+template <typename T, bool DOT>
+__device__ __forceinline__ void redo_query(
+    const char *__restrict__ vectors, const uint64_t *__restrict__ tids, int nvec, int lg, const char *qrow, int q,
+    const SlotOf slot_of, int64_t m, float *v, int k, int kp, int cap, float eps, float qn, float g_ref, int widen,
+    float *__restrict__ out_dist, int64_t *__restrict__ out_slot, uint64_t *__restrict__ out_tid,
+    int32_t *__restrict__ out_i32, double *__restrict__ stats, float *__restrict__ pair_t, const PlanEmit emit,
+    unsigned long long *ent, SelShared *sel, float *exact, int64_t *slots) {
+    const size_t row_bytes = (size_t)nvec * sizeof(Raw16);
+    auto pair_terms = [&]() {
+        if constexpr (DOT) {
+            __syncthreads();
+            fill_pair_terms(vectors, row_bytes, qrow, nvec * 4, slots, k, pair_t + (size_t)q * k);
+            if (emit.cnt) {
+                const int64_t l = (int)threadIdx.x < k ? slots[threadIdx.x] : -1;
+                __syncthreads();
+                if ((int)threadIdx.x < k) {
+                    if (l >= 0) atomicAdd(&emit.cnt[l], 1);
+                    slots[threadIdx.x] = l >= 0 ? emit.list_off[l + 1] - emit.list_off[l] : 0;
+                }
+                __syncthreads();
+                if ((int)threadIdx.x < k) {
+                    int64_t run = 0;
+                    for (int i = 0; i < (int)threadIdx.x; i++) run += slots[i];
+                    emit.probe_off[(size_t)q * k + threadIdx.x] = run;
+                    if ((int)threadIdx.x == k - 1) emit.seg_len[q] = run + slots[threadIdx.x];
+                }
+            }
+        }
+    };
+    if (widen && k <= kWide / 2) {
+        const int nw = (int)(m < kWide ? m : (int64_t)kWide);
+        block_topk([v](int64_t i) { return v[i]; }, m, nw, kWide, cap, ent, sel);
+        const int kk = nw < k ? nw : k;
+        unsigned band = 0u;
+        if (kk > 0) {
+            const float edge = key_to_float((unsigned)(ent[kk - 1] >> 32)) + 2.f * eps;
+            band = float_to_key(edge + g_ref * fabsf(edge + qn));
+        }
+        const int cnt = __syncthreads_count((int)threadIdx.x < nw && (unsigned)(ent[threadIdx.x] >> 32) <= band);
+        if (!(m > nw && cnt == nw)) {
+            const unsigned my_pos = (int)threadIdx.x < cnt ? (unsigned)(ent[threadIdx.x] & 0xffffffffu) : 0u;
+            const int64_t slot = (int)threadIdx.x < cnt ? slot_of((int64_t)my_pos) : -1;
+            if ((int)threadIdx.x < cnt) slots[threadIdx.x] = slot;
+            __syncthreads();
+            score_rows<T, 0, 0>([&](int64_t j) { return vectors + (size_t)slots[j] * row_bytes; }, 0, cnt, qrow, nvec, lg,
+                                exact);
+            __syncthreads();
+            if ((int)threadIdx.x < kWide)
+                ent[threadIdx.x] = (int)threadIdx.x < cnt
+                                       ? ((unsigned long long)float_to_key(exact[threadIdx.x]) << 32) | my_pos
+                                       : ~0ull;
+            __syncthreads();
+            const unsigned long long mine = ent[threadIdx.x];
+            int rank = 0;
+            for (int j = 0; j < cnt; j++) rank += ent[j] < mine ? 1 : 0;
+            const int have = (int)(m < k ? m : (int64_t)k);
+            if ((int)threadIdx.x < cnt && rank < k) {
+                const size_t o = (size_t)q * k + rank;
+                out_dist[o] = key_to_float((unsigned)(mine >> 32));
+                if (out_slot) out_slot[o] = slot;
+                if (out_i32) out_i32[o] = (int32_t)slot;
+                if (out_tid) out_tid[o] = tids ? tids[slot] : ~0ull;
+                slots[rank] = slot;
+            }
+            if ((int)threadIdx.x >= have && (int)threadIdx.x < k) {
+                const size_t o = (size_t)q * k + threadIdx.x;
+                out_dist[o] = INFINITY;
+                if (out_slot) out_slot[o] = -1;
+                if (out_i32) out_i32[o] = -1;
+                if (out_tid) out_tid[o] = ~0ull;
+                slots[threadIdx.x] = -1;
+            }
+            if (stats && threadIdx.x == 0) atomicAdd(&stats[7], 1.0);
+            pair_terms();
+            return;
+        }
+        __syncthreads();
+    }
+    if (stats && threadIdx.x == 0) atomicAdd(&stats[6], 1.0);
+    score_rows<T, 0, 0>([&](int64_t j) { return vectors + (size_t)slot_of(j) * row_bytes; }, 0, m, qrow, nvec, lg, v);
+    __threadfence();
+    __syncthreads();
+    block_topk([v](int64_t i) { return __hip_atomic_load(v + i, __ATOMIC_RELAXED, __HIP_MEMORY_SCOPE_AGENT); }, m, k, kp,
+               cap, ent, sel);
+    for (int i = threadIdx.x; i < k; i += kQThreads) {
+        const unsigned long long e = ent[i];
+        const bool have = e != ~0ull && (int64_t)i < (m < k ? m : (int64_t)k);
+        const int64_t slot = have ? slot_of((int64_t)(unsigned)(e & 0xffffffffu)) : -1;
+        out_dist[(size_t)q * k + i] = have ? key_to_float((unsigned)(e >> 32)) : INFINITY;
+        if (out_slot) out_slot[(size_t)q * k + i] = slot;
+        if (out_i32) out_i32[(size_t)q * k + i] = (int32_t)slot;
+        if (out_tid) out_tid[(size_t)q * k + i] = (have && tids) ? tids[slot] : ~0ull;
+        slots[i] = slot;
+    }
+    pair_terms();
+}
 
 template <typename T, bool DOT = false>
 __global__ __launch_bounds__(kQThreads) void batch_recheck_kernel(
     const char *__restrict__ vectors, const uint64_t *__restrict__ tids, int nvec, int lg,
-    const char *__restrict__ queries, int kprime, int k, const float *__restrict__ approx_val,
-    const int64_t *__restrict__ cand_pos, const int64_t *__restrict__ cand_slot,
+    const char *__restrict__ queries, const float *__restrict__ qnorm, int kprime, int k, int kp, int cap,
+    const float *__restrict__ approx_val, const int64_t *__restrict__ cand_pos,
     const int64_t *__restrict__ list_off, const int32_t *__restrict__ probe_lists,
     const int64_t *__restrict__ probe_off, int probes,
-    const int64_t *__restrict__ seg_start, int64_t fixed_len,
-    const unsigned *__restrict__ row_norm_max, ScanBound bound, const float *__restrict__ eps_add, int nq,
+    const int64_t *__restrict__ seg_start, int64_t fixed_len, float *seg_vals,
+    const unsigned *__restrict__ row_norm_max, ScanBound bound, const float *__restrict__ eps_add, int widen,
     float *__restrict__ out_dist, int64_t *__restrict__ out_slot, uint64_t *__restrict__ out_tid,
-    int32_t *__restrict__ out_i32, int32_t *__restrict__ flags, float *__restrict__ pair_t, PlanEmit emit) {
+    int32_t *__restrict__ out_i32, double *__restrict__ stats, float *__restrict__ pair_t, PlanEmit emit) {
     static_assert(!DOT || std::is_same<T, float>::value, "pair terms: fp32 rows");
+    static_assert(kRecheckCap == kQThreads, "one candidate per thread");
+    extern __shared__ __attribute__((aligned(16))) char smem[];
+    unsigned long long *ent = reinterpret_cast<unsigned long long *>(smem);
+    SelShared *sel = reinterpret_cast<SelShared *>(smem + (size_t)cap * 8);
     __shared__ float exact[kRecheckCap];
     __shared__ float dots[DOT ? kRecheckCap : 1];
-    __shared__ __attribute__((aligned(16))) unsigned long long ent[kRecheckCap];
+    __shared__ int64_t slots[kRecheckCap];
+    __shared__ float qn_part[kQWaves];
+    __shared__ SlotMap map;
     const int q = blockIdx.x;
     const size_t row_bytes = (size_t)nvec * sizeof(Raw16);
-    const int64_t m = seg_start ? seg_start[q + 1] - seg_start[q] : fixed_len;
+    const char *qrow = queries + (size_t)q * row_bytes;
+    const bool mine_in = (int)threadIdx.x < kprime;
+    const float my_av = mine_in ? approx_val[(size_t)q * kprime + threadIdx.x] : 0.f;
+    const int64_t my_pos = mine_in ? cand_pos[(size_t)q * kprime + threadIdx.x] : 0;
+    const bool map_lds = probe_lists && probes <= kSlotTab;
+    if (map_lds && (int)threadIdx.x < probes) {
+        map.off[threadIdx.x] = probe_off[(size_t)q * probes + threadIdx.x];
+        map.beg[threadIdx.x] = list_off[probe_lists[(size_t)q * probes + threadIdx.x]];
+    }
+    const int64_t base = seg_start ? seg_start[q] : (int64_t)q * fixed_len;
+    const int64_t m = seg_start ? seg_start[q + 1] - base : fixed_len;
+    const float rn = __uint_as_float(*row_norm_max);
+    const float add = eps_add ? eps_add[q] : 0.f;
     const int ncand = (int)(m < kprime ? m : (int64_t)kprime);
     const int kk = ncand < k ? ncand : k;
-    const float *av = approx_val + (size_t)q * kprime;
-    __shared__ float qn_part[kQWaves];
-    {
-        const char *qrow = queries + (size_t)q * row_bytes;
+    if (mine_in) exact[threadIdx.x] = my_av;
+    float qn = 0.f;
+    if (qnorm) {
+        qn = qnorm[q];
+    } else {
         float a = 0.f;
         for (int v = threadIdx.x; v < nvec; v += kQThreads) {
             const Raw16 x = load16(qrow + (size_t)v * sizeof(Raw16));
@@ -361,54 +512,43 @@
         if ((threadIdx.x & (kWave - 1)) == 0) qn_part[threadIdx.x >> 6] = a;
     }
     __syncthreads();
-    float qn = 0.f;
-    for (int w = 0; w < kQWaves; w++) qn += qn_part[w];
-    const float rn = __uint_as_float(*row_norm_max);
+    if (!qnorm)
+        for (int w = 0; w < kQWaves; w++) qn += qn_part[w];
     const float cross = 2.f * sqrtf(qn * rn);
-    const float eps = 1.001f * (bound.g_sq * (qn + rn + cross) + bound.g_dot * cross + bound.g_norm * rn +
-                                (eps_add ? eps_add[q] : 0.f));
+    const float eps = 1.001f * (bound.g_sq * (qn + rn + cross) + bound.g_dot * cross + bound.g_norm * rn + add);
     unsigned band = 0u;
     if (kk > 0) {
-        const float edge = av[kk - 1] + 2.f * eps;
+        const float edge = exact[kk - 1] + 2.f * eps;
         band = float_to_key(edge + bound.g_ref * fabsf(edge + qn));
     }
-    const int cnt = __syncthreads_count((int)threadIdx.x < ncand && float_to_key(av[threadIdx.x]) <= band);
-    __shared__ int64_t slots[kRecheckCap];
+    const int cnt = __syncthreads_count((int)threadIdx.x < ncand && float_to_key(my_av) <= band);
+    const SlotOf slot_of{map_lds ? &map : nullptr, probe_off + (size_t)q * probes, probe_lists + (size_t)q * probes,
+                         list_off, probes};
+    if (m > ncand && cnt == ncand) {
+        redo_query<T, DOT>(vectors, tids, nvec, lg, qrow, q, slot_of, m, seg_vals + base, k, kp, cap, eps, qn, bound.g_ref,
+                      widen, out_dist, out_slot, out_tid, out_i32, stats, pair_t, emit, ent, sel, exact, slots);
+        return;
+    }
+    int64_t my_slot = -1;
+    uint64_t my_tid = ~0ull;
     if ((int)threadIdx.x < cnt) {
-        const int64_t p = cand_pos[(size_t)q * kprime + threadIdx.x];
-        int64_t slot = p;
-        if (cand_slot) {
-            slot = cand_slot[(size_t)q * kprime + threadIdx.x];
-        } else {
-            const int64_t *off = probe_off + (size_t)q * probes;
-            int lo = 0, hi = probes - 1;
-            while (lo < hi) {
-                const int mid = (lo + hi + 1) >> 1;
-                if (off[mid] <= p)
-                    lo = mid;
-                else
-                    hi = mid - 1;
-            }
-            slot = list_off[probe_lists[(size_t)q * probes + lo]] + (p - off[lo]);
-        }
-        slots[threadIdx.x] = slot;
+        my_slot = slot_of(my_pos);
+        slots[threadIdx.x] = my_slot;
+        if (out_tid && tids) my_tid = tids[my_slot];
     }
     __syncthreads();
     if constexpr (DOT)
         score_rows_dot([&](int64_t j) { return vectors + (size_t)slots[j] * row_bytes; }, 0, cnt,
-                       queries + (size_t)q * row_bytes, nvec, lg, exact, dots);
+                       qrow, nvec, lg, exact, dots);
     else
-        score_rows<T, 0, 0>([&](int64_t j) { return vectors + (size_t)slots[j] * row_bytes; }, 0, cnt,
-                            queries + (size_t)q * row_bytes, nvec, lg, exact);
+        score_rows<T, 0, 0>([&](int64_t j) { return vectors + (size_t)slots[j] * row_bytes; }, 0, cnt, qrow, nvec, lg,
+                            exact);
     __syncthreads();
-    if ((int)threadIdx.x < kRecheckCap)
-        ent[threadIdx.x] = (int)threadIdx.x < cnt
-                               ? ((unsigned long long)float_to_key(exact[threadIdx.x]) << 32) |
-                                     (unsigned)cand_pos[(size_t)q * kprime + threadIdx.x]
-                               : ~0ull;
+    ent[threadIdx.x] = (int)threadIdx.x < cnt
+                           ? ((unsigned long long)float_to_key(exact[threadIdx.x]) << 32) | (unsigned)my_pos
+                           : ~0ull;
     __syncthreads();
     const unsigned long long mine = ent[threadIdx.x];
-    const int64_t my_slot = (int)threadIdx.x < cnt ? slots[threadIdx.x] : -1;
     int rank = 0;
     {
         const ulonglong2 *e2 = reinterpret_cast<const ulonglong2 *>(ent);
@@ -425,7 +565,7 @@
         out_dist[o] = key_to_float((unsigned)(mine >> 32));
         if (out_slot) out_slot[o] = my_slot;
         if (out_i32) out_i32[o] = (int32_t)my_slot;
-        if (out_tid) out_tid[o] = tids ? tids[my_slot] : ~0ull;
+        if (out_tid) out_tid[o] = my_tid;
         if constexpr (DOT) pair_t[o] = -2.f * dots[threadIdx.x];
     }
     if ((int)threadIdx.x >= kk && (int)threadIdx.x < k) {
@@ -452,169 +592,6 @@
                 if ((int)threadIdx.x == k - 1) emit.seg_len[q] = run + slots[threadIdx.x];
             }
         }
-    }
-    if (threadIdx.x == 0) {
-        const int32_t flag = (m > ncand && cnt == ncand) ? 1 : 0;
-        flags[q] = flag;
-        if (flag) flags[nq + 1 + atomicAdd(&flags[nq], 1)] = q;
-    }
-}
-
-constexpr int kWide = kRecheckCap;
-
-template <typename T>
-__global__ __launch_bounds__(kQThreads) void batch_fix_kernel(
-    const char *__restrict__ vectors, const int64_t *__restrict__ list_off, const uint64_t *__restrict__ tids, int nvec,
-    int lg, const char *__restrict__ queries, const int32_t *__restrict__ probe_lists,
-    const int64_t *__restrict__ probe_off, int probes, const int64_t *__restrict__ seg_start, int64_t fixed_len,
-    const int32_t *__restrict__ flags, int nq, float *__restrict__ seg_vals, int k, int kp, int cap,
-    const unsigned *__restrict__ row_norm_max, ScanBound bound, const float *__restrict__ eps_add, int widen,
-    float *__restrict__ out_dist, int64_t *__restrict__ out_slot, uint64_t *__restrict__ out_tid,
-    int32_t *__restrict__ out_i32, double *__restrict__ stats, float *__restrict__ pair_t, PlanEmit emit) {
-    extern __shared__ __attribute__((aligned(16))) char smem[];
-    unsigned long long *ent = reinterpret_cast<unsigned long long *>(smem);
-    SelShared *sel = reinterpret_cast<SelShared *>(smem + (size_t)cap * 8);
-    __shared__ float exact[kWide];
-    __shared__ int64_t slots[kWide];
-    __shared__ float qn_part[kQWaves];
-    const int nflag = flags[nq];
-    const size_t row_bytes = (size_t)nvec * sizeof(Raw16);
-    for (int f = blockIdx.x; f < nflag; f += gridDim.x) {
-        const int q = flags[nq + 1 + f];
-        const int64_t base = probe_lists ? seg_start[q] : (int64_t)q * fixed_len;
-        const int64_t m = probe_lists ? seg_start[q + 1] - base : fixed_len;
-        const int64_t *off = probe_off + (size_t)q * probes;
-        const int32_t *pl = probe_lists + (size_t)q * probes;
-        auto slot_of = [&](int64_t j) -> int64_t {
-            if (!probe_lists) return j;
-            int lo = 0, hi = probes - 1;
-            while (lo < hi) {
-                const int mid = (lo + hi + 1) >> 1;
-                if (off[mid] <= j)
-                    lo = mid;
-                else
-                    hi = mid - 1;
-            }
-            return list_off[pl[lo]] + (j - off[lo]);
-        };
-        float *v = seg_vals + base;
-        const char *qrow = queries + (size_t)q * row_bytes;
-        auto pair_terms = [&]() {
-            if constexpr (std::is_same<T, float>::value) {
-                if (pair_t) {
-                    __threadfence();
-                    __syncthreads();
-                    fill_pair_terms(vectors, row_bytes, qrow, nvec * 4, out_i32 ? out_i32 + (size_t)q * k : nullptr,
-                                    out_slot ? out_slot + (size_t)q * k : nullptr, k, pair_t + (size_t)q * k);
-                    if (emit.cnt) {
-                        if ((int)threadIdx.x < k) {
-                            const int l = __hip_atomic_load(out_i32 + (size_t)q * k + threadIdx.x, __ATOMIC_RELAXED,
-                                                            __HIP_MEMORY_SCOPE_AGENT);
-                            if (l >= 0) atomicAdd(&emit.cnt[l], 1);
-                            slots[threadIdx.x] = l >= 0 ? emit.list_off[l + 1] - emit.list_off[l] : 0;
-                        }
-                        __syncthreads();
-                        if ((int)threadIdx.x < k) {
-                            int64_t run = 0;
-                            for (int i = 0; i < (int)threadIdx.x; i++) run += slots[i];
-                            emit.probe_off[(size_t)q * k + threadIdx.x] = run;
-                            if ((int)threadIdx.x == k - 1) emit.seg_len[q] = run + slots[threadIdx.x];
-                        }
-                    }
-                }
-            }
-        };
-        if constexpr (std::is_same<T, float>::value) {
-            if (pair_t && emit.cnt) {
-                if ((int)threadIdx.x < k) {
-                    const int l = out_i32[(size_t)q * k + threadIdx.x];
-                    if (l >= 0) atomicSub(&emit.cnt[l], 1);
-                }
-                __syncthreads();
-            }
-        }
-        bool settled = false;
-        if (widen && k <= kWide / 2) {
-            const int nw = (int)(m < kWide ? m : (int64_t)kWide);
-            block_topk([v](int64_t i) { return v[i]; }, m, nw, kWide, cap, ent, sel);
-            {
-                float a = 0.f;
-                for (int x = threadIdx.x; x < nvec; x += kQThreads) {
-                    const Raw16 e = load16(qrow + (size_t)x * sizeof(Raw16));
-                    a = accum_slice<T, 1>(a, e, e);
-                }
-                for (int m2 = 32; m2 > 0; m2 >>= 1) a += __shfl_xor(a, m2);
-                if ((threadIdx.x & (kWave - 1)) == 0) qn_part[threadIdx.x >> 6] = a;
-            }
-            __syncthreads();
-            float qn = 0.f;
-            for (int w = 0; w < kQWaves; w++) qn += qn_part[w];
-            const float rn = __uint_as_float(*row_norm_max);
-            const float cross = 2.f * sqrtf(qn * rn);
-            const float eps = 1.001f * (bound.g_sq * (qn + rn + cross) + bound.g_dot * cross + bound.g_norm * rn +
-                                        (eps_add ? eps_add[q] : 0.f));
-            const int kk = nw < k ? nw : k;
-            unsigned band = 0u;
-            if (kk > 0) {
-                const float edge = key_to_float((unsigned)(ent[kk - 1] >> 32)) + 2.f * eps;
-                band = float_to_key(edge + bound.g_ref * fabsf(edge + qn));
-            }
-            const int cnt = __syncthreads_count((int)threadIdx.x < nw && (unsigned)(ent[threadIdx.x] >> 32) <= band);
-            settled = !(m > nw && cnt == nw);
-            if (settled) {
-                const unsigned my_pos = (int)threadIdx.x < cnt ? (unsigned)(ent[threadIdx.x] & 0xffffffffu) : 0u;
-                if ((int)threadIdx.x < cnt) slots[threadIdx.x] = slot_of((int64_t)my_pos);
-                __syncthreads();
-                score_rows<T, 0, 0>([&](int64_t j) { return vectors + (size_t)slots[j] * row_bytes; }, 0, cnt, qrow, nvec, lg,
-                                    exact);
-                __syncthreads();
-                if ((int)threadIdx.x < kWide)
-                    ent[threadIdx.x] = (int)threadIdx.x < cnt
-                                           ? ((unsigned long long)float_to_key(exact[threadIdx.x]) << 32) | my_pos
-                                           : ~0ull;
-                __syncthreads();
-                const unsigned long long mine = ent[threadIdx.x];
-                int rank = 0;
-                for (int j = 0; j < cnt; j++) rank += ent[j] < mine ? 1 : 0;
-                const int have = (int)(m < k ? m : (int64_t)k);
-                if ((int)threadIdx.x < cnt && rank < k) {
-                    const size_t o = (size_t)q * k + rank;
-                    const int64_t slot = slots[threadIdx.x];
-                    out_dist[o] = key_to_float((unsigned)(mine >> 32));
-                    if (out_slot) out_slot[o] = slot;
-                    if (out_i32) out_i32[o] = (int32_t)slot;
-                    if (out_tid) out_tid[o] = tids ? tids[slot] : ~0ull;
-                }
-                if ((int)threadIdx.x >= have && (int)threadIdx.x < k) {
-                    const size_t o = (size_t)q * k + threadIdx.x;
-                    out_dist[o] = INFINITY;
-                    if (out_slot) out_slot[o] = -1;
-                    if (out_i32) out_i32[o] = -1;
-                    if (out_tid) out_tid[o] = ~0ull;
-                }
-                if (stats && threadIdx.x == 0) atomicAdd(&stats[7], 1.0);
-                pair_terms();
-            }
-            __syncthreads();
-        }
-        if (settled) continue;
-        if (stats && threadIdx.x == 0) atomicAdd(&stats[6], 1.0);
-        score_rows<T, 0, 0>([&](int64_t j) { return vectors + (size_t)slot_of(j) * row_bytes; }, 0, m, qrow, nvec, lg, v);
-        __threadfence();
-        __syncthreads();
-        block_topk([v](int64_t i) { return __hip_atomic_load(v + i, __ATOMIC_RELAXED, __HIP_MEMORY_SCOPE_AGENT); }, m, k, kp,
-                   cap, ent, sel);
-        for (int i = threadIdx.x; i < k; i += kQThreads) {
-            const unsigned long long e = ent[i];
-            const bool have = e != ~0ull && (int64_t)i < (m < k ? m : (int64_t)k);
-            const int64_t slot = have ? slot_of((int64_t)(unsigned)(e & 0xffffffffu)) : -1;
-            out_dist[(size_t)q * k + i] = have ? key_to_float((unsigned)(e >> 32)) : INFINITY;
-            if (out_slot) out_slot[(size_t)q * k + i] = slot;
-            if (out_i32) out_i32[(size_t)q * k + i] = (int32_t)slot;
-            if (out_tid) out_tid[(size_t)q * k + i] = (have && tids) ? tids[slot] : ~0ull;
-        }
-        pair_terms();
-        __syncthreads();
     }
 }
 
@@ -801,14 +778,12 @@
 struct ApproxScratch {
     float *cand_val = nullptr;
     int64_t *cand_pos = nullptr;
-    int32_t *flags = nullptr;
     int carve(DBuf &buf, int nq, int kprime) {
         const size_t nk = (size_t)nq * kprime;
-        const size_t a1 = (sizeof(float) * nk + 15) & ~(size_t)15, a2 = a1 + sizeof(int64_t) * nk;
-        PGV_TRY(buf.ensure(a2 + sizeof(int32_t) * (2 * (size_t)nq + 1)));
+        const size_t a1 = (sizeof(float) * nk + 15) & ~(size_t)15;
+        PGV_TRY(buf.ensure(a1 + sizeof(int64_t) * nk));
         cand_val = buf.as<float>();
         cand_pos = reinterpret_cast<int64_t *>(buf.as<char>() + a1);
-        flags = reinterpret_cast<int32_t *>(buf.as<char>() + a2);
         return PGV_OK;
     }
 };
@@ -824,24 +799,27 @@
     if (t.kprime > kRecheckCap || t.k > t.kprime)
         PGV_FAIL(PGV_ERR_ARG, "exact tail: k' = %d outside k..%d", t.kprime, kRecheckCap);
     if (t.pair_t && xr.dtype != PGV_F32) PGV_FAIL(PGV_ERR_ARG, "exact tail: pair terms are for fp32 rows");
-    static_assert(kWide >= kRecheckCap, "k <= k' <= kWide: batch_fix_kernel's emit");
+    static_assert(kWide >= kRecheckCap && kWide <= kQThreads, "k <= k' <= kWide: redo_query's row through slots[]");
     if (t.emit.cnt && !(dense && t.pair_t && t.out_i32 && t.emit.probe_off && t.emit.seg_len && t.emit.list_off))
         PGV_FAIL(PGV_ERR_ARG, "exact tail: the plan is counted where the pair terms are written");
     ApproxScratch sc;
     PGV_TRY(sc.carve(scratch, t.nq, t.kprime));
-    const int64_t *cand_slot = dense ? sc.cand_pos : nullptr;
     const int64_t *seg_start = dense ? nullptr : t.seg_start;
     const int64_t fixed_len = dense ? t.fixed_len : 0;
-    PGV_TRY(launch_topk_segments(ctx, t.approx, seg_start, t.nq, fixed_len, t.kprime, sc.cand_val, sc.cand_pos,
-                                 sc.flags + t.nq, t.emit.cnt, t.emit.cnt ? 2 * (int)fixed_len : 0,
-                                 dense ? 0 : t.seg_bound));
+    PGV_TRY(launch_topk_segments(ctx, t.approx, seg_start, t.nq, fixed_len, t.kprime, sc.cand_val, sc.cand_pos, nullptr,
+                                 t.emit.cnt, t.emit.cnt ? 2 * (int)fixed_len : 0, dense ? 0 : t.seg_bound));
+    double *stats = (ctx->profiling && ctx->stats_dev.p) ? ctx->stats_dev.as<double>() : nullptr;
+    int kp = 2;
+    while (kp < t.k) kp <<= 1;
+    const int cap = kp > kFastCap ? kp : kFastCap;
+    const size_t lds = (size_t)cap * 8 + sizeof(SelShared);
 #define PGV_RECHECK(T, DOT)                                                                                          \
-    hipLaunchKernelGGL((batch_recheck_kernel<T, DOT>), dim3(t.nq), dim3(kQThreads), 0, ctx->stream,                   \
+    hipLaunchKernelGGL((batch_recheck_kernel<T, DOT>), dim3(t.nq), dim3(kQThreads), lds, ctx->stream,                 \
                        static_cast<const char *>(xr.vectors), xr.tids, xr.geom.nvec, xr.geom.lpr_log2,                \
-                       static_cast<const char *>(t.queries), t.kprime, t.k, sc.cand_val, sc.cand_pos, cand_slot,      \
-                       xr.list_offsets, t.probe_lists, t.probe_off, t.probes, seg_start, fixed_len, xr.norm_max,      \
-                       t.bound, t.eps_add, t.nq, t.out_dist, t.out_slot, t.out_tid, t.out_i32, sc.flags, t.pair_t,    \
-                       t.emit)
+                       static_cast<const char *>(t.queries), t.qnorm, t.kprime, t.k, kp, cap, sc.cand_val,            \
+                       sc.cand_pos, xr.list_offsets, t.probe_lists, t.probe_off, t.probes, seg_start, fixed_len,      \
+                       t.approx, xr.norm_max, t.bound, t.eps_add, ctx->no_widen ? 0 : 1, t.out_dist, t.out_slot,      \
+                       t.out_tid, t.out_i32, stats, t.pair_t, t.emit)
     if (t.pair_t)
         PGV_RECHECK(float, true);
     else if (xr.dtype == PGV_F32)
@@ -850,24 +828,6 @@
         PGV_RECHECK(__half, false);
 #undef PGV_RECHECK
     PGV_HIP(hipGetLastError());
-    double *stats = (ctx->profiling && ctx->stats_dev.p) ? ctx->stats_dev.as<double>() : nullptr;
-    int kp = 2;
-    while (kp < t.k) kp <<= 1;
-    const int cap = kp > kFastCap ? kp : kFastCap;
-    const size_t lds = (size_t)cap * 8 + sizeof(SelShared);
-    const int grid = t.nq < ctx->num_cus ? t.nq : ctx->num_cus;
-#define PGV_FIX(T)                                                                                                    \
-    hipLaunchKernelGGL(batch_fix_kernel<T>, dim3(grid), dim3(kQThreads), lds, ctx->stream,                            \
-                       static_cast<const char *>(xr.vectors), xr.list_offsets, xr.tids, xr.geom.nvec,                 \
-                       xr.geom.lpr_log2, static_cast<const char *>(t.queries), t.probe_lists, t.probe_off, t.probes,  \
-                       seg_start, fixed_len, sc.flags, t.nq, t.approx, t.k, kp, cap, xr.norm_max, t.bound, t.eps_add, \
-                       ctx->no_widen ? 0 : 1, t.out_dist, t.out_slot, t.out_tid, t.out_i32, stats, t.pair_t, t.emit)
-    if (xr.dtype == PGV_F32)
-        PGV_FIX(float);
-    else
-        PGV_FIX(__half);
-#undef PGV_FIX
-    PGV_HIP(hipGetLastError());
     return PGV_OK;
 }
 
diff --git a/pgvector_amd/csrc/kernels_shadow.hip b/pgvector_amd/csrc/kernels_shadow.hip
--- a/pgvector_amd/csrc/kernels_shadow.hip
+++ b/pgvector_amd/csrc/kernels_shadow.hip
@@ -143,7 +143,7 @@
                                                            const float *__restrict__ row_norm_max,
                                                            __half *__restrict__ qcast, float *__restrict__ qscale,
                                                            float *__restrict__ qeps, float *__restrict__ cscale,
-                                                           float *__restrict__ ceps) {
+                                                           float *__restrict__ ceps, float *__restrict__ qnorm) {
     const int q = (int)(blockIdx.x * 4 + (threadIdx.x >> 6));
     if (q >= nq) return;
     const int lane = threadIdx.x & (kWave - 1);
@@ -189,6 +189,7 @@
         hh += __shfl_xor(hh, o);
     }
     const double u = 5.9604644775390625e-8;
+    if (lane == 0 && qnorm) qnorm[q] = __double2float_ru(qq * (1.0 + 1.0 / 1073741824.0));
     if (lane == 0 && ceps) {
         const int e = 1 + rt.s + sq;
         const double qn = sqrt(qq), dq = sqrt(dd), qh = sqrt(hh);
@@ -266,11 +267,12 @@
 
 int launch_shadow_query(pgv_ctx *ctx, const RowGeom &g32, const RowGeom &g16, const void *queries, int nq,
                         const ShadowTerms &st, const RankShadowTerms &rt, const float *center_norm_max,
-                        const float *row_norm_max, void *qcast, float *qscale, float *qeps, float *cscale, float *ceps) {
+                        const float *row_norm_max, void *qcast, float *qscale, float *qeps, float *cscale, float *ceps,
+                        float *qnorm) {
     if (nq <= 0) return PGV_OK;
     hipLaunchKernelGGL(shadow_query_kernel, dim3((unsigned)((nq + 3) / 4)), dim3(256), 0, ctx->stream,
                        static_cast<const float *>(queries), nq, g32.ld, g16.ld, st, rt, center_norm_max, row_norm_max,
-                       static_cast<__half *>(qcast), qscale, qeps, cscale, ceps);
+                       static_cast<__half *>(qcast), qscale, qeps, cscale, ceps, qnorm);
     PGV_HIP(hipGetLastError());
     return PGV_OK;
 }
diff --git a/pgvector_amd/csrc/pgv_abi_ivf.hip b/pgvector_amd/csrc/pgv_abi_ivf.hip
--- a/pgvector_amd/csrc/pgv_abi_ivf.hip
+++ b/pgvector_amd/csrc/pgv_abi_ivf.hip
@@ -124,6 +124,7 @@
     void *qcast = nullptr;
     float *qscale = nullptr, *qeps = nullptr;
     float *cscale = nullptr, *ceps = nullptr;
+    float *qnorm = nullptr;
     float *pair_t = nullptr;
     bool scan_follows = false;
     bool cast_for_scan = false;
@@ -134,13 +135,14 @@
     pgv_ctx *ctx = ix->ctx;
     const RowGeom &g16 = ix->shadow_geom;
     const size_t qb = ((size_t)nq * g16.ld * sizeof(uint16_t) + 255) & ~(size_t)255;
-    PGV_TRY(ctx->sh_q.ensure(qb + sizeof(float) * (size_t)nq * (4 + (size_t)probes)));
+    PGV_TRY(ctx->sh_q.ensure(qb + sizeof(float) * (size_t)nq * (5 + (size_t)probes)));
     sb->qcast = ctx->sh_q.p;
     sb->qscale = reinterpret_cast<float *>(ctx->sh_q.as<char>() + qb);
     sb->qeps = sb->qscale + nq;
     sb->cscale = sb->qeps + nq;
     sb->ceps = sb->cscale + nq;
-    sb->pair_t = sb->ceps + nq;
+    sb->qnorm = sb->ceps + nq;
+    sb->pair_t = sb->qnorm + nq;
     constexpr double u = 5.9604644775390625e-8;
     ShadowTerms st{};
     st.s = ix->shadow_s;
@@ -158,7 +160,7 @@
     PGV_TRY(launch_shadow_query(ctx, ix->geom, g16, q_dev, nq, st, rt, ix->center_norms + ix->nlists,
                                 ix->row_norms + ix->nrows, sb->qcast, for_scan ? sb->qscale : nullptr,
                                 for_scan ? sb->qeps : nullptr, for_rank ? sb->cscale : nullptr,
-                                for_rank ? sb->ceps : nullptr));
+                                for_rank ? sb->ceps : nullptr, sb->qnorm));
     sb->cast_for_scan = for_scan;
     return PGV_OK;
 }
@@ -842,6 +844,7 @@
         tail.bound = scan_bound_chain(ctx, ix->geom.ld, scan_chain_length(ix->geom, ix->dtype, false));
         if (rank_sh) tail.bound = shadow_band(ix->geom.ld, tail.bound.g_ref);
         tail.eps_add = rank_sh ? sb->ceps : nullptr;
+        tail.qnorm = rank_sh ? sb->qnorm : nullptr;
         tail.out_dist = dist;
         tail.out_i32 = out_lists_dev;
         PGV_TRY(launch_exact_tail(ctx, tail, ctx->ms_b));
@@ -1018,6 +1021,7 @@
         tail.bound = scan_bound_chain(ctx, ix->geom.ld, scan_chain_length(ix->geom, ix->dtype, path.wide));
         if (path.shadow) tail.bound = shadow_band(ix->geom.ld, tail.bound.g_ref);
         tail.eps_add = path.shadow ? sb->qeps : nullptr;
+        tail.qnorm = path.shadow ? sb->qnorm : nullptr;
         tail.out_dist = od.as<float>();
         tail.out_slot = os.as<int64_t>();
         tail.out_tid = ot.as<uint64_t>();
diff --git a/pgvector_amd/csrc/pgv_internal.h b/pgvector_amd/csrc/pgv_internal.h
--- a/pgvector_amd/csrc/pgv_internal.h
+++ b/pgvector_amd/csrc/pgv_internal.h
@@ -466,7 +466,8 @@
 int scan_chain_length(const RowGeom &g, pgv_dtype dtype, bool wide);
 int launch_shadow_query(pgv_ctx *ctx, const RowGeom &g32, const RowGeom &g16, const void *queries, int nq,
                         const ShadowTerms &st, const RankShadowTerms &rt, const float *center_norm_max,
-                        const float *row_norm_max, void *qcast, float *qscale, float *qeps, float *cscale, float *ceps);
+                        const float *row_norm_max, void *qcast, float *qscale, float *qeps, float *cscale, float *ceps,
+                        float *qnorm);
 int launch_shadow_pairs(pgv_ctx *ctx, const RowGeom &g32, const void *queries, const void *centers,
                         const int64_t *pair_start, int nlists, int64_t npairs, ScanPair *pairs);
 int mfma_scan_queries_per_task_wide();
@@ -536,6 +537,7 @@
     int64_t fixed_len = 0;
     ScanBound bound{};
     const float *eps_add = nullptr;
+    const float *qnorm = nullptr;
     float *out_dist = nullptr;
     int64_t *out_slot = nullptr;
     uint64_t *out_tid = nullptr;
```

Result: no change. 1.521 million (median of 6 runs) (+1.0%).
